# AOS55/exorl

Hardware: AMD Instinct MI355X
Metric: gradient-steps/sec TD3+BC walker_walk batch=1024 (higher is better)
Workload: dtype bf16x3

## Files before the change

exorl_amd/_lib.py:

```python
import ctypes as C
from pathlib import Path

HERE = Path(__file__).resolve().parent
LIB_PATH = HERE / 'libexorl_hip.so'

c_void_p, c_int32, c_int64, c_float, c_size_t, c_uint64, c_uint32 = (
    C.c_void_p, C.c_int32, C.c_int64, C.c_float, C.c_size_t, C.c_uint64, C.c_uint32)
P = C.POINTER

SAMPLER_MT19937, SAMPLER_PHILOX, SAMPLER_GIVEN = 0, 1, 2
WEIGHT_EPISODES, WEIGHT_TRANSITIONS = 0, 1
AGENT_TD3_BC, AGENT_TD3, AGENT_BC, AGENT_DDPG, AGENT_CRR, AGENT_CQL, AGENT_APS = 0, 1, 2, 3, 4, 5, 6
M_CRITIC_CQL, M_CRITIC_CQL_LOGSUM, M_ACTOR_ALPHA, M_ACTOR_ALPHA_LOSS, M_ACTOR_ENT = 10, 11, 12, 13, 14
CRR_WEIGHT = {'identity': 0, 'indicator': 1, 'exp': 2}
PREC_F32, PREC_BF16, PREC_BF16X3, PREC_BF16X6 = 0, 1, 2, 3
NET_ACTOR, NET_CRITIC, NET_CRITIC_TARGET = 0, 1, 2
T_PARAM, T_GRAD, T_ADAM_M, T_ADAM_V = 0, 1, 2, 3
M_BATCH_REWARD, M_CRITIC_TARGET_Q, M_CRITIC_Q1, M_CRITIC_Q2, M_CRITIC_LOSS, M_ACTOR_LOSS, M_ACTOR_LOGPROB = range(7)
N_METRICS = 16
INTR_RND, INTR_ICM, INTR_ICM_APT, INTR_DISAGREEMENT, INTR_DIAYN, INTR_PROTO, INTR_APS, INTR_SMM = 0, 1, 2, 3, 4, 5, 6, 7
IM_LOSS, IM_INTR_REWARD, IM_EXTR_REWARD, IM_RMS_MEAN, IM_RMS_STD, IM_ACC, IM_ENT_REWARD, IM_SF_REWARD = range(8)
N_INTR_METRICS = 8
INTR_XCHG_GRAD, INTR_XCHG_REP, INTR_XCHG_MOMENTS, INTR_XCHG_BN = 0, 1, 2, 3
XCHG_F32, XCHG_F64 = 0, 1
# ... 67 lines not shown
    'exorl_pixel_agent_state': (C.c_int, [c_void_p, c_void_p, c_void_p]),
    'exorl_pixel_agent_set_state': (C.c_int, [c_void_p, c_void_p, c_void_p]),
    'exorl_pixel_agent_encoder_opt2': (C.c_int, [c_void_p, c_void_p, c_void_p, c_void_p]),
    'exorl_pixel_agent_update_phase': (C.c_int, [c_void_p, c_int32, c_float, c_void_p, c_void_p, c_void_p, c_void_p, c_void_p]),
    'exorl_pixel_agent_grad_buffer': (C.c_int, [c_void_p, c_int32, P(c_void_p), P(c_int64)]),
    'exorl_pixel_agent_set_comm': (C.c_int, [c_void_p, c_void_p]),
    'exorl_pixel_agent_encoder_step_phase': (C.c_int, [c_void_p, c_int32, c_void_p, c_int32, c_int32, c_void_p]),
    'exorl_pixel_agent_rnd_features_phase': (C.c_int, [c_void_p, c_int32, c_void_p, c_float, c_void_p, c_void_p, c_void_p]),
    'exorl_pixel_agent_bn_partials': (C.c_int, [c_void_p, P(c_void_p), P(c_int64)]),
    'exorl_pixel_agent_metrics': (C.c_int, [c_void_p, c_void_p, c_void_p]),
    'exorl_pixel_agent_act': (C.c_int, [c_void_p, c_void_p, c_void_p, c_float, c_int32, c_void_p, c_void_p, c_void_p]),
    'exorl_aug_shift': (C.c_int, [c_void_p, c_int32, c_int32, c_int32, c_int32, c_void_p, c_uint64, c_uint64, c_void_p, c_void_p]),
    'exorl_encoder_param_floats': (c_int64, [c_int32, c_int32]),
    'exorl_encoder_out_dim': (c_int64, [c_int32]),
    'exorl_encoder_workspace_floats': (c_int64, [c_int32, c_int32, c_int32]),
    'exorl_encoder_forward': (C.c_int, [c_void_p, c_int32, c_int32, c_void_p, c_int32, c_void_p, P(c_void_p), c_void_p]),
    'exorl_encoder_backward': (C.c_int, [c_void_p, c_int32, c_int32, c_void_p, c_int32, c_void_p, c_void_p, c_void_p, c_void_p]),
    'exorl_encoder_forward_prec': (C.c_int, [c_void_p, c_int32, c_int32, c_void_p, c_int32, c_void_p, P(c_void_p), c_int32, c_void_p]),
    'exorl_encoder_backward_prec': (C.c_int, [c_void_p, c_int32, c_int32, c_void_p, c_int32, c_void_p, c_void_p, c_void_p, c_int32, c_void_p]),
    'exorl_intr_workspace_bytes': (c_size_t, [P(IntrCfg)]),
    'exorl_intr_create': (C.c_int, [P(IntrCfg), c_void_p, c_size_t, P(c_void_p)]),
    'exorl_intr_destroy': (C.c_int, [c_void_p]),
    'exorl_intr_num_tensors': (C.c_int, [c_void_p, P(c_int32)]),
    'exorl_intr_tensor': (C.c_int, [c_void_p, c_int32, c_int32, P(c_void_p), P(c_int64), P(c_int64)]),
    'exorl_intr_flat': (C.c_int, [c_void_p, c_int32, P(c_void_p), P(c_int64)]),
    'exorl_intr_state': (C.c_int, [c_void_p, P(c_void_p), P(c_void_p), P(c_int64)]),
    'exorl_intr_queue': (C.c_int, [c_void_p, P(c_void_p), P(c_int64), P(c_int64), P(c_int64), c_int32]),
    'exorl_intr_update': (C.c_int, [c_void_p, P(IntrBatch), c_int32, c_void_p]),
    'exorl_intr_update_phase': (C.c_int, [c_void_p, P(IntrBatch), c_int32, c_int32, P(c_int32), c_void_p]),
    'exorl_intr_exchange': (C.c_int, [c_void_p, c_int32, P(c_void_p), P(c_int64), P(c_int32), P(c_int32)]),
    'exorl_intr_metrics': (C.c_int, [c_void_p, c_void_p, c_void_p]),
    'exorl_intr_opt_steps': (C.c_int, [c_void_p, P(c_int64), c_int32]),
    'exorl_intr_counter': (C.c_int, [c_void_p, c_void_p, c_int32]),
    'exorl_last_error': (C.c_char_p, []),
    'exorl_abi_version': (C.c_int, []),
    'exorl_device_info': (C.c_int, [C.c_char_p, C.c_int, P(C.c_int), P(c_int64)]),
    'exorl_replay_create': (C.c_int, [P(ReplayCfg), P(c_void_p)]),
    'exorl_replay_destroy': (C.c_int, [c_void_p]),
    'exorl_replay_append_episode': (C.c_int, [c_void_p, c_void_p, c_void_p, c_void_p, c_void_p, c_void_p, c_int32, P(c_int32)]),
    'exorl_replay_evict': (C.c_int, [c_void_p, c_int32]),
    'exorl_replay_set_order': (C.c_int, [c_void_p, c_void_p, c_int32]),
    'exorl_replay_set_weights': (C.c_int, [c_void_p, c_int32, c_void_p, c_int32]),
    'exorl_replay_num_rows': (C.c_int, [c_void_p, P(c_int64), P(c_int64)]),
    'exorl_replay_seed_mt': (C.c_int, [c_void_p, c_void_p, c_int32, c_void_p, c_int32]),
    'exorl_replay_seed_mt_ints': (C.c_int, [c_void_p, c_uint64, c_uint32]),
    'exorl_replay_get_mt': (C.c_int, [c_void_p, c_void_p, P(c_int32), c_void_p, P(c_int32)]),
    'exorl_replay_seed_philox': (C.c_int, [c_void_p, c_uint64]),
    'exorl_replay_sample': (C.c_int, [c_void_p, c_int32, c_int32, c_float, c_int32, c_void_p, P(BatchOut), c_void_p, c_void_p]),
    'exorl_replay_last_pairs': (C.c_int, [c_void_p, c_int32, c_void_p, c_void_p]),
    'exorl_comm_unique_id': (C.c_int, [c_void_p]),
    'exorl_comm_init': (C.c_int, [c_int32, c_int32, c_void_p, P(c_void_p)]),
    'exorl_comm_destroy': (C.c_int, [c_void_p]),
    'exorl_comm_allreduce': (C.c_int, [c_void_p, c_void_p, c_int64, c_void_p]),
    'exorl_agent_set_comm': (C.c_int, [c_void_p, c_void_p]),
    'exorl_agent_workspace_bytes': (c_size_t, [P(AgentCfg)]),
    'exorl_agent_create': (C.c_int, [P(AgentCfg), c_void_p, c_size_t, P(c_void_p)]),
    'exorl_agent_destroy': (C.c_int, [c_void_p]),
    'exorl_agent_num_tensors': (C.c_int, [c_void_p, c_int32, P(c_int32)]),
    'exorl_agent_tensor': (C.c_int, [c_void_p, c_int32, c_int32, c_int32, P(c_void_p), P(c_int64), P(c_int64)]),
    'exorl_agent_flat': (C.c_int, [c_void_p, c_int32, c_int32, P(c_void_p), P(c_int64)]),
    'exorl_agent_params_changed': (C.c_int, [c_void_p, c_int32, c_void_p]),
    'exorl_agent_batch_slots': (C.c_int, [c_void_p, P(BatchOut)]),
    'exorl_agent_set_batch': (C.c_int, [c_void_p, c_void_p, c_void_p, c_void_p, c_void_p, c_void_p, c_void_p]),
    'exorl_agent_update': (C.c_int, [c_void_p, c_float, c_void_p, c_void_p, c_void_p]),
    'exorl_agent_update_phase': (C.c_int, [c_void_p, c_int32, c_float, c_void_p, c_void_p, c_void_p]),
    'exorl_agent_stats_buffer': (C.c_int, [c_void_p, P(c_void_p), P(c_int64)]),
    'exorl_agent_cql_alpha': (C.c_int, [c_void_p, c_void_p, c_int32]),
    'exorl_agent_act': (C.c_int, [c_void_p, c_void_p, c_int32, c_float, c_int32, c_void_p, c_void_p, c_void_p]),
    'exorl_agent_act_host': (C.c_int, [c_void_p, c_void_p, c_int32, c_float, c_int32, c_void_p, c_void_p, c_void_p]),
    'exorl_agent_metrics': (C.c_int, [c_void_p, c_void_p, c_void_p]),
    'exorl_agent_set_metrics': (C.c_int, [c_void_p, c_int32]),
    'exorl_agent_metric_window_bytes': (c_size_t, [P(AgentCfg)]),
    'exorl_agent_set_metric_window': (C.c_int, [c_void_p, c_void_p, c_size_t]),
    'exorl_agent_metric_window_read': (C.c_int, [c_void_p, c_void_p, c_void_p, c_int32, c_void_p]),
    'exorl_agent_set_parallel_branches': (C.c_int, [c_void_p, c_int32]),
    'exorl_agent_opt_steps': (C.c_int, [c_void_p, P(c_int64), P(c_int64)]),
    'exorl_agent_set_opt_steps': (C.c_int, [c_void_p, c_int64, c_int64]),
    'exorl_agent_enable_graph': (C.c_int, [c_void_p, c_void_p, c_int32, c_float, c_float, c_void_p]),
    'exorl_agent_enable_graph_intr': (C.c_int, [c_void_p, c_void_p, P(IntrBatch), c_int32, c_void_p, c_int32, c_float, c_float, c_void_p]),
    'exorl_agent_step_graph': (C.c_int, [c_void_p, c_float, c_void_p]),
    'exorl_agent_noise_counter': (C.c_int, [c_void_p, P(c_uint64), c_void_p]),
    'exorl_debug_philox_normal': (C.c_int, [c_uint64, c_uint64, c_int64, c_void_p, c_void_p]),
    'exorl_debug_agent_poison_scratch': (C.c_int, [c_void_p, c_void_p]),
    'exorl_debug_agent_weight_images': (C.c_int, [c_void_p, c_int32, P(WeightImages)]),
    'exorl_agent_disable_graph': (C.c_int, [c_void_p]),
    'exorl_gemm': (C.c_int, [c_int32, c_int32, c_int32, c_int32, c_int32, c_int32, c_void_p, c_int64, c_void_p, c_int64,
                             c_void_p, c_int64, c_void_p, c_int32, c_int32, c_void_p]),
    'exorl_gemm_bf16': (C.c_int, [c_int32, c_int32, c_int32, c_int32, c_int32, c_void_p, c_int64, c_void_p, c_int64, c_void_p, c_int64,
                                  c_void_p, c_int32, c_int32, c_void_p]),
    'exorl_gemm_planes': (C.c_int, [c_int32, c_void_p, c_int32, c_int32, c_int32, c_int32, c_void_p, c_void_p, c_int64, c_void_p, c_void_p, c_int64,
                                    c_void_p, c_int64, c_int32, c_void_p]),
    'exorl_gemm_planes3': (C.c_int, [c_int32, c_void_p, c_int32, c_int32, c_int32, c_int32, c_void_p, c_void_p, c_void_p, c_int64, c_void_p, c_void_p, c_void_p,
                                     c_int64, c_void_p, c_int64, c_int32, c_void_p]),
    'exorl_gemm_tune': (C.c_int, [c_int32]),
    'exorl_debug_precision_override': (C.c_int, [c_int32]),
    'exorl_profile_gemm': (C.c_int, [c_int32]),
    'exorl_profile_gemm_read': (C.c_int, [c_void_p, c_void_p, c_int32, P(c_int32)]),
    'exorl_profile_event_overhead': (C.c_int, [c_void_p, c_void_p]),
    'exorl_adam_step': (C.c_int, [c_void_p, c_void_p, c_void_p, c_void_p, c_int64, c_float, c_float, c_float, c_float,
                                  c_int64, c_void_p, c_float, c_void_p]),
    'exorl_soft_update': (C.c_int, [c_void_p, c_void_p, c_int64, c_float, c_void_p]),
    'exorl_ln_tanh_fwd': (C.c_int, [c_void_p, c_void_p, c_void_p, c_void_p, c_void_p, c_void_p, c_int32, c_int32, c_void_p]),
    'exorl_knn_topk': (C.c_int, [c_void_p, c_int32, c_void_p, c_int32, c_int32, c_int32, c_void_p, c_void_p]),
}


class ExorlError(RuntimeError):
    pass


_lib = None


def load():
    global _lib
    if _lib is not None:
        return _lib
    if not LIB_PATH.exists():
        raise ExorlError(f'{LIB_PATH} is missing: build it with `python exorl_amd/build.py` '
                         '(hipcc --offload-arch=gfx950). There is no CPU fallback.')
    lib = C.CDLL(str(LIB_PATH))
    for name, (res, args) in PROTOTYPES.items():
        fn = getattr(lib, name)
        fn.restype = res
        fn.argtypes = args
    _lib = lib
    return lib


def check(rc):
    if rc != 0:
        raise ExorlError(load().exorl_last_error().decode())


def ptr(t):
    if t is None:
        return None
    if hasattr(t, 'data_ptr'):
        return t.data_ptr()
    return t.ctypes.data


def current_stream():
    import torch
    return torch.cuda.current_stream().cuda_stream
```

exorl_amd/csrc/agent.hip:

```cpp
#include <cmath>
#include <vector>

#include "kernels.h"

namespace exorl {

struct NetDesc {
    int in_dim = 0, out_dim = 0, H = 0, n_trunks = 0, n_heads = 0;
    int64_t W0 = 0, b0 = 0, g = 0, beta = 0, trunk_stride = 0;
    int64_t W1 = 0, b1 = 0, W2 = 0, b2 = 0, head_stride = 0;
    int64_t total = 0;
    std::vector<TensorDesc> tensors;
};

static int64_t pad4(int64_t n) { return round_up(n, 4); }

static NetDesc make_net(int in_dim, int out_dim, int H, int n_trunks, int n_heads) {
    NetDesc d;
    d.in_dim = in_dim; d.out_dim = out_dim; d.H = H; d.n_trunks = n_trunks; d.n_heads = n_heads;
    int64_t off = 0;
    auto add = [&](int64_t rows, int64_t cols) { const int64_t o = off; d.tensors.push_back({o, rows, cols}); off += pad4(rows * cols); return o; };
    auto add_trunk = [&](bool first) {
        const int64_t w = add(H, in_dim), b = add(H, 1), gg = add(H, 1), be = add(H, 1);
        if (first) { d.W0 = w; d.b0 = b; d.g = gg; d.beta = be; }
// ... 29 lines not shown
    hipStream_t aux = nullptr;
    hipEvent_t ev_fork = nullptr, ev_join = nullptr;
    bool on = false;
    int fork(hipStream_t s) const {
        if (!on) return 0;
        EXORL_CHECK_HIP(hipEventRecord(ev_fork, s));
        EXORL_CHECK_HIP(hipStreamWaitEvent(aux, ev_fork, 0));
        return 0;
    }
    int join(hipStream_t s) const {
        if (!on) return 0;
        EXORL_CHECK_HIP(hipEventRecord(ev_join, aux));
        EXORL_CHECK_HIP(hipStreamWaitEvent(s, ev_join, 0));
        return 0;
    }
    hipStream_t side(hipStream_t s) const { return on ? aux : s; }
};

struct FwdBufs {
    float *h1, *xhat, *rstd, *h2, *out;
    Planes h1q, xhatq;
    FwdBufs rows_from(int64_t row0, int64_t H, int64_t out_cols) const {
        return FwdBufs{h1 + row0 * H, xhat + row0 * H, rstd + row0, h2 + row0 * H, out + row0 * out_cols, h1q.at(row0 * H), xhatq.at(row0 * H)};
    }
};
struct BwdBufs { float *dz2, *dh1; Planes dz2q; };
struct NetShadow { float* w0t; Planes w1q, w0q; };

enum class Route {
    F32,
    Planes,
    Planes3,
};
static Route route_of(int prec, const Planes& act, const Planes& w1, int rows) {
    if (prec == EXORL_PREC_BF16 || (prec == EXORL_PREC_BF16X3 && w1.lo)) return Route::Planes;
    if (prec == EXORL_PREC_BF16X6 && act && w1 && rows % 128 == 0) return Route::Planes3;
    return Route::F32;
}
struct Operand {
    const float* f; Planes q;
    Operand() : f(nullptr) {}
    Operand(const float* f32, int64_t foff, const Planes& planes, int64_t qoff) : f(f32 ? f32 + foff : nullptr), q(planes.at(qoff)) {}
};
struct Product { Operand A, B; float* C; const float* bias; int M, N, K; };
static Gemm16Problem g16(const Planes& A, const Planes& B, float* C, const float* bias, int M, int N, int K, int64_t ld) {
    Gemm16Problem p{A.hi, B.hi, C, bias, M, N, K, ld, ld, ld};
    if (A.mid && B.mid) { p.A_mid = A.mid; p.B_mid = B.mid; }
    if (A.lo && B.lo) { p.A_lo = A.lo; p.B_lo = B.lo; }
    return p;
}
static Gemm16Problem g16(const Product& p, int64_t ld) { return g16(p.A.q, p.B.q, p.C, p.bias, p.M, p.N, p.K, ld); }
static int products(Route rt, int prec, int a_layout, int b_layout, const Product* p, int count, int64_t ld, bool relu, bool accumulate, hipStream_t s) {
    if (rt == Route::F32) {
        GemmProblem g[4];
        for (int i = 0; i < count; ++i) g[i] = GemmProblem{p[i].A.f, p[i].B.f, p[i].C, p[i].bias, p[i].M, p[i].N, p[i].K, ld, ld, ld};
        return gemm_grouped(prec, a_layout, b_layout, g, count, relu, accumulate, s);
    }
    Gemm16Problem q[4];
    for (int i = 0; i < count; ++i) q[i] = g16(p[i], ld);
    return gemm16_grouped(a_layout, b_layout, q, count, relu, accumulate, s);
}
static int refresh_w1_planes(const NetDesc& d, const float* P, const NetShadow& sh, hipStream_t s) {
    if (!sh.w1q.mid) return 0;
    return to_planes3(P + d.W1, d.H, d.H, d.H, sh.w1q.hi, sh.w1q.mid, sh.w1q.lo, d.H, d.H, d.n_heads, d.head_stride, (int64_t)d.H * d.H, s);
}
struct Partials { float *Ph, *Pt, *Pw; };

static ShadowSpec shadow_spec(const NetDesc& d, const NetShadow& sh, const NetShadow* target) {
    ShadowSpec s{};
    s.n_trunks = d.n_trunks; s.n_heads = d.n_heads; s.in_dim = d.in_dim; s.H = d.H;
    for (int t = 0; t < d.n_trunks; ++t) s.w0_off[t] = d.W0 + t * d.trunk_stride;
    for (int i = 0; i < d.n_heads; ++i) s.w1_off[i] = d.W1 + i * d.head_stride;
    const NetShadow none{};
    const NetShadow& t = target ? *target : none;
    const bool own = !sh.w1q.mid;
    s.w0t = sh.w0t; s.t_w0t = t.w0t;
    if (own) { s.w1b = sh.w1q.hi; s.w1l = sh.w1q.lo; s.t_w1b = t.w1q.hi; s.t_w1l = t.w1q.lo; }
    s.w0b = sh.w0q.hi; s.w0l = sh.w0q.lo; s.t_w0b = t.w0q.hi; s.t_w0l = t.w0q.lo;
    return s;
}

static int net_forward(const NetDesc& d, const float* P, const NetShadow& sh, const float* x, int64_t ldx, int rows,
                       const FwdBufs& f, bool save, bool tanh_out, int prec, hipStream_t s, const SampleSpec* sample = nullptr,
                       bool no_head = false) {
    const int H = d.H;
    const int64_t act = (int64_t)rows * H;
    const Route rt = route_of(prec, f.h1q, sh.w1q, rows);
    const bool bf = rt == Route::Planes;
    if (bf && sh.w0q && trunk_fwd16_supported(H))
        EXORL_TRY(trunk_fwd16(x, ldx, sh.w0q, P + d.b0, P + d.g, P + d.beta, save ? f.rstd : nullptr, f.h1q, save ? f.xhatq : Planes{}, rows,
                              d.in_dim, H, d.n_trunks, act, d.trunk_stride, s));
    else
        EXORL_TRY(trunk_fwd(x, ldx, sh.w0t, P + d.b0, P + d.g, P + d.beta, bf ? nullptr : f.h1, (save && !bf) ? f.xhat : nullptr,
                            save ? f.rstd : nullptr, bf ? f.h1q.hi : nullptr, (bf && save) ? f.xhatq.hi : nullptr, rows, d.in_dim, H,
                            d.n_trunks, act, d.trunk_stride, (int64_t)d.in_dim * H, s));
    if (rt == Route::Planes3) EXORL_TRY(to_planes3(f.h1, H, d.n_trunks * rows, H, f.h1q.hi, f.h1q.mid, f.h1q.lo, d.n_trunks * rows, H, 1, 0, 0, s));
    Product p[2];
    for (int i = 0; i < d.n_heads; ++i) {
        const int64_t t = (d.n_trunks == d.n_heads ? i : 0) * act;
        p[i] = Product{Operand(f.h1, t, f.h1q, t), Operand(P + d.W1, i * d.head_stride, sh.w1q, (int64_t)i * H * H), f.h2 + i * act,
                       P + d.b1 + i * d.head_stride, rows, H, H};
    }
    EXORL_TRY(products(rt, prec, 0, 0, p, d.n_heads, H, true, false, s));
    if (no_head) return 0;
    if (H % 4 == 0)
        EXORL_TRY(head_fwd4(f.h2, P + d.W2, P + d.b2, f.out, rows, H, d.out_dim, tanh_out ? 1 : 0, d.n_heads, act, d.head_stride,
                            (int64_t)rows * d.out_dim, s, sample));
    else
        EXORL_TRY(head_fwd(f.h2, P + d.W2, P + d.b2, f.out, rows, H, d.out_dim, tanh_out ? 1 : 0, d.n_heads, act, d.head_stride,
                           (int64_t)rows * d.out_dim, s));
    return 0;
}

static bool forward2_supported(const NetDesc& d, int prec, const NetShadow& sa, const FwdBufs& fa, const NetShadow& sb, const FwdBufs& fb, int rows) {
    const bool planes = route_of(prec, fa.h1q, sa.w1q, rows) == Route::Planes && route_of(prec, fb.h1q, sb.w1q, rows) == Route::Planes;
    return planes && sa.w0q && sb.w0q && trunk_fwd16_supported(d.H) && d.out_dim == 1 && d.n_heads == 2 && d.H % 4 == 0;
}
static int net_forward2(const NetDesc& d, const float* Pa, const NetShadow& sa, const float* xa, const FwdBufs& fa, bool save_a,
                        const float* Pb, const NetShadow& sb, const float* xb, const FwdBufs& fb, bool save_b, int64_t ldx, int rows,
                        hipStream_t s, bool no_head = false, bool fold_a = false, int* slots_a = nullptr) {
    const int H = d.H;
    const int64_t act = (int64_t)rows * H, wst = (int64_t)H * round_up(d.in_dim, 32);
    const float* P[2] = {Pa, Pb};
    const NetShadow* sh[2] = {&sa, &sb};
    const float* x[2] = {xa, xb};
    const FwdBufs* f[2] = {&fa, &fb};
    const bool save[2] = {save_a, save_b};
    TrunkBatch tb{};
    int nt = 0;
    for (int k = 0; k < 2; ++k)
        for (int t = 0; t < d.n_trunks; ++t) {
            const Planes w = sh[k]->w0q.at(t * wst), h = f[k]->h1q.at(t * act), xh = save[k] ? f[k]->xhatq.at(t * act) : Planes{};
            tb.it[nt++] = TrunkItem{x[k], w.hi, P[k] + d.b0 + t * d.trunk_stride, P[k] + d.g + t * d.trunk_stride, P[k] + d.beta + t * d.trunk_stride,
                                    save[k] ? f[k]->rstd + (int64_t)t * rows : nullptr, h.hi, xh.hi, w.lo, h.lo, xh.lo};
        }
    EXORL_TRY(trunk_fwd16_batch(tb, nt, ldx, rows, d.in_dim, H, s));
    Gemm16Problem q[4];
    HeadBatch hb{};
    int nq = 0;
    for (int k = 0; k < 2; ++k)
        for (int i = 0; i < d.n_heads; ++i) {
            q[nq] = g16(f[k]->h1q.at((d.n_trunks == d.n_heads ? i : 0) * act), sh[k]->w1q.at((int64_t)i * H * H), f[k]->h2 + i * act,
                        P[k] + d.b1 + i * d.head_stride, rows, H, H, H);
            hb.it[nq] = HeadItem{f[k]->h2 + i * act, P[k] + d.W2 + i * d.head_stride, P[k] + d.b2 + i * d.head_stride, f[k]->out + (int64_t)i * rows};
            ++nq;
        }
    if (slots_a) *slots_a = 0;
    if (no_head && fold_a && slots_a) {
        const int slots = gemm16_head_slots(q, nq);
        if (slots > 0 && (int64_t)slots <= H) {
            for (int i = 0; i < d.n_heads; ++i) {
                q[i].head_w = P[0] + d.W2 + i * d.head_stride;
                q[i].head_part = f[0]->h2 + i * act;
            }
            *slots_a = slots;
        }
    }
    EXORL_TRY(gemm16_grouped(0, 0, q, nq, true, false, s));
    if (no_head) return 0;
    return head_fwd1_batch(hb, nq, rows, H, s);
}

static int net_backward(const NetDesc& d, const float* P, const NetShadow& sh, float* G, const Partials& pt, const float* x,
                        int64_t ldx, int rows, const FwdBufs& f, const DoutSpec& dout, const BwdBufs& b, float* dx, int dx_col0,
                        int dx_cols, int prec, hipStream_t s, const Fork& fk, FinalizeArgs* defer = nullptr, bool have_dz2 = false) {
    const int H = d.H;
    const int64_t act = (int64_t)rows * H;
    const bool paired = d.n_trunks == d.n_heads;
    Route rt = route_of(prec, f.h1q, sh.w1q, rows);
    if (rt == Route::Planes3 && !b.dz2q) rt = Route::F32;
    const bool bf = rt == Route::Planes;
    const Planes none{};
    const Planes &dz2q = bf ? b.dz2q : none, &h1q = bf ? f.h1q : none, &xhatq = bf ? f.xhatq : none;
    if (have_dz2) {
    } else if (d.out_dim > 16) {
        EXORL_REQUIRE(d.n_heads == 1, "net_backward: wide heads are single-net only");
        EXORL_TRY(head_bwd_wide(dout, P + d.W2, f.h2, bf ? nullptr : b.dz2, dz2q, G ? pt.Ph : nullptr, rows, H, d.out_dim, act, d.head_stride,
                                G ? 1 : 0, s));
    } else {
        EXORL_TRY(head_bwd(dout, P + d.W2, f.h2, bf ? nullptr : b.dz2, dz2q, G ? pt.Ph : nullptr, rows, H, d.out_dim, d.n_heads, act,
                           d.head_stride, G ? 1 : 0, s, dout.mode == EXORL_DOUT_ACTOR_MU && dout.bc_part));
    }
    if (rt == Route::Planes3) EXORL_TRY(to_planes3(b.dz2, H, d.n_heads * rows, H, b.dz2q.hi, b.dz2q.mid, b.dz2q.lo, d.n_heads * rows, H, 1, 0, 0, s));
    auto trunk_of = [&](int i) { return (paired ? i : 0) * act; };
    auto wgrad = [&](int i, int r0, int kr) {
        const int64_t o = (int64_t)r0 * H;
        return Product{Operand(b.dz2, i * act + o, b.dz2q, i * act + o), Operand(f.h1, trunk_of(i) + o, f.h1q, trunk_of(i) + o),
                       G + d.W1 + i * d.head_stride, nullptr, H, H, kr};
    };
    auto dgrad = [&](int i) {
        return Product{Operand(b.dz2, i * act, b.dz2q, i * act), Operand(P + d.W1, i * d.head_stride, sh.w1q, (int64_t)i * H * H),
                       b.dh1 + trunk_of(i), nullptr, rows, H, H};
    };
    Product p[2];
    int dgrads_done = 0;
    if (bf && G && !fk.on) {
        Gemm16Problem q[4];
        int at[4], nq = 0;
        for (int i = 0; i < d.n_heads; ++i) { at[nq] = 1; q[nq++] = g16(wgrad(i, 0, rows), H); }
        dgrads_done = paired ? d.n_heads : 1;
        for (int i = 0; i < dgrads_done; ++i) { at[nq] = 0; q[nq++] = g16(dgrad(i), H); }
        EXORL_TRY(gemm16_grouped_mixed(at, q, nq, s));
    } else if (G) {
        EXORL_TRY(fk.fork(s));
        const int slab = (!bf && rows >= 8192) ? 1024 : rows;
        for (int r0 = 0; r0 < rows; r0 += slab) {
            for (int i = 0; i < d.n_heads; ++i) p[i] = wgrad(i, r0, rows - r0 < slab ? rows - r0 : slab);
            EXORL_TRY(products(rt, prec, 1, 1, p, d.n_heads, H, false, r0 > 0, fk.side(s)));
        }
    }
    for (int i = 0; i < d.n_heads; ++i) p[i] = dgrad(i);
    if (!paired) {
        for (int i = dgrads_done; i < d.n_heads; ++i) EXORL_TRY(products(rt, prec, 0, 1, p + i, 1, H, false, i > 0, s));
    } else if (dgrads_done == 0) {
        EXORL_TRY(products(rt, prec, 0, 1, p, d.n_heads, H, false, false, s));
    }
    const bool dx_fused = dx && !G;
    EXORL_TRY(ln_bwd(b.dh1, f.h1, f.xhat, h1q, xhatq, f.rstd, P + d.g, pt.Pt, rows, H, d.n_trunks, act, d.trunk_stride, G ? 1 : 0, s,
                     dx_fused ? sh.w0t + (int64_t)dx_col0 * H : nullptr, (int64_t)d.in_dim * H, dx_fused ? dx : nullptr, dx_cols,
                     (bf && trunk_fwd16_supported(H)) ? P + d.beta : nullptr));
    if (dx && !dx_fused)
        EXORL_TRY(head_fwd4(b.dh1, sh.w0t + (int64_t)dx_col0 * H, nullptr, dx, rows, H, dx_cols, 0, d.n_trunks, act,
                            (int64_t)d.in_dim * H, (int64_t)rows * dx_cols, s));
    if (G) {
        EXORL_TRY(outer_reduce(x, ldx, d.in_dim, b.dh1, pt.Pw, rows, H, d.n_trunks, act, s));
        EXORL_TRY(fk.join(s));
        FinalizeArgs fa{};
        fa.Ph = pt.Ph; fa.head_chunks = have_dz2 ? qhead_chunks(rows) : head_chunks(rows); fa.n_heads = d.n_heads; fa.head_stride = d.head_stride;
        fa.gW2 = d.W2; fa.gb1 = d.b1; fa.gb2 = d.b2;
        fa.Pt = pt.Pt; fa.trunk_chunks = trunk_chunks(rows); fa.n_trunks = d.n_trunks; fa.trunk_stride = d.trunk_stride;
        fa.Pw = pt.Pw; fa.w_chunks = outer_chunks(rows);
        fa.gW0 = d.W0; fa.gb0 = d.b0; fa.gg = d.g; fa.gbeta = d.beta;
        fa.H = H; fa.nout = d.out_dim; fa.in_dim = d.in_dim; fa.G = G;
        if (defer) *defer = fa;
        else EXORL_TRY(finalize_grads(fa, s));
    }
    return 0;
}

struct Carver : SimpleCarver {
    bool scratch = false;
    std::vector<std::pair<int64_t, int64_t>>* fill = nullptr;
    using SimpleCarver::SimpleCarver;
    float* take(int64_t n) {
        if (fill) {
            const int64_t padded = round_up(n, 64), o = scratch ? off : off + n, len = scratch ? padded : padded - n;
            if (len > 0) {
                if (!fill->empty() && fill->back().first + fill->back().second == o) fill->back().second += len;
                else fill->push_back({o, len});
            }
        }
        return SimpleCarver::take(n);
    }
};

constexpr int ACT_ROWS = 64;

}

using namespace exorl;

struct exorl_agent {
    exorl_agent_cfg cfg;
    NetDesc actor, critic;
    bool has_critic = false;
    bool owns_ws = false;
    float* ws = nullptr;
    size_t ws_bytes = 0;
    float* flat[3][4] = {{nullptr}};
    float *obs = nullptr, *action = nullptr, *reward = nullptr, *discount = nullptr, *next_obs = nullptr;
    float *xa = nullptr, *xc_cur = nullptr, *xc_next = nullptr, *xc_pi = nullptr;
    FwdBufs fa{}, ft{}, fc{};
    BwdBufs bc{}, ba{};
    float *dq = nullptr, *da = nullptr, *dpre = nullptr, *abs_part = nullptr;
    float *sfq = nullptr, *sftq = nullptr;
    float *x_all = nullptr, *dq_all = nullptr;
    CqlScalars* cql = nullptr;
    float *xc_rep = nullptr, *crr_w = nullptr;
    FwdBufs fr{};
    NetShadow sh_actor{}, sh_critic{}, sh_target{};
    ShadowSpec spec_actor{}, spec_critic{};
    Partials pa{}, pc{};
    float *stats = nullptr, *metrics = nullptr;
    float *act_x = nullptr, *act_noise = nullptr;
    float* act_part = nullptr; unsigned int* act_ticket = nullptr;
    FwdBufs fact{};
    StepState* state = nullptr;
    const float *noise_c = nullptr, *noise_a = nullptr;
    int64_t actor_t = 0, critic_t = 0;
    uint64_t act_noise_counter = 0;
    float inv_bg = 0.f;
    float dev_stddev = -1.f;
    hipGraphExec_t graph_exec = nullptr;
    hipGraph_t graph = nullptr;
    hipStream_t capture_stream = nullptr;
    exorl_replay* graph_replay = nullptr;
    uint64_t graph_weights_epoch = 0;
    uint64_t graph_replay_ctr = 0;
    exorl_intr* graph_intr = nullptr;
    bool capturing = false;
    Fork fk{};
    bool parallel_branches = false;
    bool fuse_opt = false;
    bool whole_step = false;
    exorl_comm* comm = nullptr;
    hipStream_t comm_stream = nullptr;
    hipEvent_t ev_stats_ready = nullptr, ev_stats_done = nullptr;
    FinalizeArgs pend_c{}, pend_a{};
    bool staged_by_sampler = false;
    bool want_metrics = true;
    int tq_slots = 0;
    double* win_sums = nullptr; long long* win_steps = nullptr;
    float *win_crit = nullptr, *win_bc = nullptr;
};

namespace exorl {

static bool planes_ok(const exorl_agent_cfg& cfg) {
    return cfg.precision == EXORL_PREC_BF16X3 && cfg.hidden_dim % 64 == 0 && cfg.batch % 64 == 0 && trunk_fwd16_supported(cfg.hidden_dim);
}

static bool planes3_ok(const exorl_agent_cfg& cfg) {
    return cfg.precision == EXORL_PREC_BF16X6 && cfg.hidden_dim % 128 == 0 && cfg.batch % 128 == 0;
}

static void carve(exorl_agent* a, Carver& c) {
    const auto& cfg = a->cfg;
    const int64_t B = cfg.batch, O = cfg.obs_dim, A = cfg.act_dim, H = cfg.hidden_dim, W = O + A;
    const int64_t AO = a->actor.out_dim;
    const int64_t RC = cfg.kind == EXORL_AGENT_CQL ? (3 * cfg.n_samples + 1) * B : B;
    for (int w = 0; w < 4; ++w) a->flat[EXORL_NET_ACTOR][w] = c.take(a->actor.total);
    if (a->has_critic) {
        for (int w = 0; w < 4; ++w) a->flat[EXORL_NET_CRITIC][w] = c.take(a->critic.total);
        a->flat[EXORL_NET_CRITIC_TARGET][EXORL_T_PARAM] = c.take(a->critic.total);
    }
    a->obs = c.take(B * O); a->action = c.take(B * A); a->reward = c.take(B); a->discount = c.take(B); a->next_obs = c.take(B * O);
    const int np = cfg.precision == EXORL_PREC_BF16 ? 1 : planes_ok(cfg) ? 2 : planes3_ok(cfg) ? 3 : 0;
    const int nb = np == 3 ? 0 : np;
    auto take_u16 = [&](int64_t n) { return reinterpret_cast<unsigned short*>(c.take((n + 1) / 2)); };
    auto take_hi_lo = [&](Planes& x, int64_t nx, Planes* y, int64_t ny, int planes) {
        if (planes >= 1) { x.hi = take_u16(nx); if (y) y->hi = take_u16(ny); }
        if (planes >= 2) { x.lo = take_u16(nx); if (y) y->lo = take_u16(ny); }
    };
    auto three_planes = [&](Planes& x, int64_t n) { if (np == 3) { x.hi = take_u16(n); x.mid = take_u16(n); x.lo = take_u16(n); } };
    auto take_fwd = [&](int64_t trunk_rows, int64_t head_rows, int64_t out_cols, bool saved, bool f32_h1, int planes) {
        FwdBufs f{};
        if (f32_h1) f.h1 = c.take(trunk_rows * H);
        if (saved) { f.xhat = c.take(trunk_rows * H); f.rstd = c.take(trunk_rows); }
        f.h2 = c.take(head_rows * H); f.out = c.take(head_rows * out_cols);
        take_hi_lo(f.h1q, trunk_rows * H, saved ? &f.xhatq : nullptr, trunk_rows * H, planes);
        return f;
    };
    auto take_bwd = [&](int64_t head_rows, int64_t trunk_rows) {
        BwdBufs b{c.take(head_rows * H), c.take(trunk_rows * H), {}};
        take_hi_lo(b.dz2q, head_rows * H, nullptr, 0, nb);
        return b;
    };
    auto take_shadow = [&](int64_t n_trunks, int64_t n_heads, int64_t in_dim) {
        NetShadow sh{c.take(n_trunks * in_dim * H), {}, {}};
        take_hi_lo(sh.w1q, n_heads * H * H, &sh.w0q, n_trunks * H * round_up(in_dim, 32), nb);
        return sh;
    };
    c.scratch = true;
    a->xa = c.take(2 * B * O);
    a->fa = take_fwd(2 * B, 2 * B, AO, true, true, nb);
    a->ba = take_bwd(B, B);
    three_planes(a->fa.h1q, 2 * B * H);
    three_planes(a->ba.dz2q, B * H);
    c.scratch = false;
    a->sh_actor = take_shadow(1, 1, O);
    three_planes(a->sh_actor.w1q, H * H);
    c.scratch = true;
    a->pa = Partials{c.take((int64_t)head_chunks(B) * ((AO + 1) * H + 32)), c.take((int64_t)trunk_chunks(B) * 3 * H),
                     c.take((int64_t)outer_chunks(B) * O * H)};
    a->dpre = c.take(B * AO);
    c.scratch = false;
    a->stats = c.take(4 + EXORL_N_METRICS);
    a->metrics = a->stats ? a->stats + 4 : nullptr;
    a->state = reinterpret_cast<StepState*>(c.take((sizeof(StepState) + 3) / 4));
    a->act_x = c.take(ACT_ROWS * O);
    a->act_noise = c.take(ACT_ROWS * A);
    a->act_part = c.take((int64_t)cdiv(H, 4) * ACT_FAST_ROWS * 16);
    a->act_ticket = reinterpret_cast<unsigned int*>(c.take(4));
    a->fact = take_fwd(ACT_ROWS, ACT_ROWS, AO, false, true, nb ? 1 : 0);
    if (a->has_critic) {
        const int64_t nt = a->critic.n_trunks;
        c.scratch = true;
        a->xc_cur = c.take(B * W); a->xc_next = c.take(B * W); a->xc_pi = c.take(B * W);
        const int64_t od = a->critic.out_dim;
        a->ft = take_fwd(nt * B, 2 * B, od, false, true, nb);
        a->fc = take_fwd(nt * RC, 2 * RC, od, true, true, nb);
        a->bc = take_bwd(2 * RC, nt * RC);
        three_planes(a->ft.h1q, nt * B * H);
        three_planes(a->fc.h1q, nt * RC * H);
// ... 32 lines not shown
    EXORL_REQUIRE(cfg, "agent: null cfg");
    EXORL_REQUIRE(cfg->kind >= EXORL_AGENT_TD3_BC && cfg->kind <= EXORL_AGENT_APS, "agent: unknown kind %d", cfg->kind);
    EXORL_REQUIRE(cfg->kind != EXORL_AGENT_APS || (cfg->sf_dim >= 1 && cfg->sf_dim <= 16 && cfg->sf_dim < cfg->obs_dim),
                  "agent: APS needs 1 <= sf_dim <= 16 and obs_dim = observation + sf_dim (got sf_dim=%d obs_dim=%d)", cfg->sf_dim, cfg->obs_dim);
    EXORL_REQUIRE(cfg->kind != EXORL_AGENT_CQL || (cfg->n_samples >= 1 && cfg->n_samples <= 16 && cfg->act_dim <= 16),
                  "agent: CQL needs 1 <= n_samples <= 16 and action_dim <= 16 (got %d, %d)", cfg->n_samples, cfg->act_dim);
    EXORL_REQUIRE(!cfg->use_critic_lagrange || cfg->kind == EXORL_AGENT_CQL, "agent: use_critic_lagrange is a CQL option");
    EXORL_REQUIRE(cfg->kind != EXORL_AGENT_CRR || (cfg->num_value_samples >= 1 && cfg->num_value_samples <= 64 &&
                  cfg->weight_func >= EXORL_CRR_IDENTITY && cfg->weight_func <= EXORL_CRR_EXP),
                  "agent: CRR needs 1 <= num_value_samples <= 64 and a valid weight_func (got %d, %d)", cfg->num_value_samples, cfg->weight_func);
    EXORL_REQUIRE(cfg->obs_dim > 0 && cfg->act_dim > 0 && cfg->act_dim <= 16 && cfg->hidden_dim >= 4 && cfg->hidden_dim <= 1024 && cfg->hidden_dim % 4 == 0 &&
                  cfg->obs_dim + cfg->act_dim <= 256 &&
                  cfg->batch > 0, "agent: unsupported dims O=%d A=%d (<=16) H=%d (multiple of 4, <=1024) B=%d; O+A <= 256", cfg->obs_dim, cfg->act_dim,
                  cfg->hidden_dim, cfg->batch);
    EXORL_REQUIRE(cfg->precision == EXORL_PREC_F32 || cfg->precision == EXORL_PREC_BF16 || cfg->precision == EXORL_PREC_BF16X3 ||
                  cfg->precision == EXORL_PREC_BF16X6, "agent: unknown precision %d", cfg->precision);
    EXORL_REQUIRE(cfg->world_size >= 1, "agent: world_size must be >= 1");
    EXORL_REQUIRE(cfg->precision != EXORL_PREC_BF16 || (cfg->hidden_dim % 8 == 0 && cfg->batch % 8 == 0),
                  "agent: bf16 precision needs hidden_dim and batch to be multiples of 8 (got H=%d B=%d)", cfg->hidden_dim, cfg->batch);
    a->cfg = *cfg;
    a->has_critic = cfg->kind != EXORL_AGENT_BC;
    a->actor = make_net(cfg->obs_dim, cfg->kind == EXORL_AGENT_CQL ? 2 * cfg->act_dim : cfg->act_dim, cfg->hidden_dim, 1, 1);
    if (a->has_critic)
        a->critic = make_net(cfg->obs_dim + cfg->act_dim, cfg->kind == EXORL_AGENT_APS ? cfg->sf_dim : 1, cfg->hidden_dim,
                             (cfg->kind == EXORL_AGENT_DDPG || cfg->kind == EXORL_AGENT_APS) ? 1 : 2, 2);
    a->inv_bg = 1.0f / ((float)cfg->batch * (float)cfg->world_size);
    return 0;
}

static NoiseSpec noise_spec(exorl_agent* a, const float* buf, int which) {
    return NoiseSpec{buf, a->cfg.seed, (uint64_t)which, buf ? nullptr : &a->state->noise_counter};
}
static NoiseSpec act_noise_spec(exorl_agent* a, const float* buf) {
    NoiseSpec n{buf, a->cfg.seed, 0, nullptr};
    if (!buf) n.counter = (1ull << 63) | a->act_noise_counter++;
    return n;
}

static int push_opt_steps(exorl_agent* a) {
    long long t[2] = {a->actor_t, a->critic_t};
    EXORL_CHECK_HIP(hipMemcpy(&a->state->t_actor, t, sizeof(t), hipMemcpyHostToDevice));
    auto prod = [](double b, long long t) { double r = 1.0; for (long long i = 0; i < t; ++i) r *= b; return r; };
    const double p[4] = {prod(0.9, a->actor_t), 0.0, prod(0.9, a->critic_t), prod(0.999, a->critic_t)};
    const double p2 = prod(0.999, a->actor_t);
    EXORL_CHECK_HIP(hipMemcpy(&a->state->b1t, p, sizeof(p), hipMemcpyHostToDevice));
    EXORL_CHECK_HIP(hipMemcpy(&a->state->b2t, &p2, sizeof(p2), hipMemcpyHostToDevice));
    return 0;
}

static FusedAdamArgs fused_adam_args(exorl_agent* a, int net, const NetDesc& d, const AdamConst* c, float* target, uint64_t* bump) {
    float** f = a->flat[net];
    return FusedAdamArgs{f[EXORL_T_PARAM], f[EXORL_T_GRAD], f[EXORL_T_ADAM_M], f[EXORL_T_ADAM_V], target, c, d.n_heads,
                         {d.W1, d.W1 + d.head_stride}, reinterpret_cast<unsigned long long*>(bump)};
}
static int opt_step(exorl_agent* a, int net, const NetDesc& d, const FinalizeArgs& pend, const AdamConst* c, float* target, const ShadowSpec& spec,
                    uint64_t* bump, hipStream_t s) {
    float** f = a->flat[net];
    if (a->fuse_opt) EXORL_TRY(finalize_adam(pend, fused_adam_args(a, net, d, c, target, bump), spec, s));
    else EXORL_TRY(adam_step_dev(f[EXORL_T_PARAM], f[EXORL_T_GRAD], f[EXORL_T_ADAM_M], f[EXORL_T_ADAM_V], d.total, c, target, &spec, s, bump));
    EXORL_TRY(refresh_w1_planes(d, f[EXORL_T_PARAM], net == EXORL_NET_ACTOR ? a->sh_actor : a->sh_critic, s));
    if (target) EXORL_TRY(refresh_w1_planes(d, target, a->sh_target, s));
    return 0;
}
static int opt_step_critic(exorl_agent* a, hipStream_t s) {
    return opt_step(a, EXORL_NET_CRITIC, a->critic, a->pend_c, &a->state->critic, a->flat[EXORL_NET_CRITIC_TARGET][EXORL_T_PARAM], a->spec_critic,
                    nullptr, s);
}

static bool qfuse(const exorl_agent* a) {
    return a->whole_step && !a->fk.on && (!a->want_metrics || a->win_sums) && a->has_critic && a->critic.n_heads == 2 && a->critic.out_dim == 1 && a->cfg.hidden_dim % 4 == 0 &&
           (a->cfg.kind == EXORL_AGENT_TD3_BC || a->cfg.kind == EXORL_AGENT_TD3 || a->cfg.kind == EXORL_AGENT_DDPG);
}
static bool step_metrics(const exorl_agent* a) { return a->win_sums ? !qfuse(a) : a->want_metrics; }
constexpr size_t WIN_HEAD_BYTES = 256;
static_assert(EXORL_N_METRICS * sizeof(double) + sizeof(long long) <= WIN_HEAD_BYTES, "the window's sums and step count fit its head");
static size_t window_bytes(const exorl_agent_cfg& cfg) {
    return WIN_HEAD_BYTES + sizeof(float) * (size_t)round_up(6 * (int64_t)qhead_chunks(cfg.batch) + head_chunks(cfg.batch), 64);
}
static int run_metrics_window(exorl_agent* a, hipStream_t s) {
    const int B = a->cfg.batch;
    MetricsWindowArgs w{};
    w.fused = qfuse(a) ? 1 : 0;
    w.crit_part = a->win_crit; w.abs_part = a->abs_part; w.bc_part = a->win_bc;
    w.q_chunks = qhead_chunks(B); w.bc_chunks = a->cfg.kind == EXORL_AGENT_TD3_BC ? head_chunks(B) : 0;
    w.kind = a->cfg.kind; w.act_dim = a->cfg.act_dim; w.ent_from_std = a->cfg.kind != EXORL_AGENT_CQL;
    w.inv_bg = a->inv_bg; w.alpha = a->cfg.alpha; w.stddev = &a->state->stddev;
    w.metrics = a->metrics; w.sums = a->win_sums; w.steps = a->win_steps;
    return metrics_window(w, s);
}
static int run_qhead(exorl_agent* a, int mode, hipStream_t s) {
    const NetDesc& d = a->critic;
    const int B = a->cfg.batch, H = d.H;
    const int64_t act = (int64_t)B * H;
    const float* Pc = a->flat[EXORL_NET_CRITIC][EXORL_T_PARAM];
    const float* Pt = a->flat[EXORL_NET_CRITIC_TARGET][EXORL_T_PARAM];
    const bool bf = route_of(a->cfg.precision, a->fc.h1q, a->sh_critic.w1q, B) == Route::Planes;
    QHeadArgs q{};
    for (int i = 0; i < 2; ++i) {
        q.a[i] = a->fc.h2 + i * act; q.W[i] = Pc + d.W2 + i * d.head_stride; q.b[i] = Pc + d.b2 + i * d.head_stride;
        q.a[2 + i] = a->ft.h2 + i * act; q.W[2 + i] = Pt + d.W2 + i * d.head_stride; q.b[2 + i] = Pt + d.b2 + i * d.head_stride;
    }
    q.q = a->fc.out; q.tq = a->ft.out; q.reward = a->reward; q.discount = a->discount;
    q.tpart[0] = q.tpart[1] = nullptr; q.tslots = 0;
    if (mode == 0 && a->tq_slots > 0) {
        q.tpart[0] = a->ft.h2; q.tpart[1] = a->ft.h2 + act; q.tslots = a->tq_slots;
    }
    q.dz = bf ? nullptr : a->bc.dz2; q.dzb = bf ? a->bc.dz2q.hi : nullptr; q.dzl = bf ? a->bc.dz2q.lo : nullptr; q.act = act;
    q.P = mode == 0 ? a->pc.Ph : nullptr;
    const bool met = mode == 0 && a->win_sums;
    q.abs_part = met ? a->win_crit : a->abs_part;
    q.rows = B; q.H = H; q.mode = mode; q.inv_bg = a->inv_bg;
    return qhead(q, s, met);
}

static int phase0(exorl_agent* a, float stddev, const float* noise_c, hipStream_t s) {
    const auto& cfg = a->cfg;
    const int B = cfg.batch, O = cfg.obs_dim, A = cfg.act_dim, W = O + A, prec = cfg.precision;
    if (!a->staged_by_sampler)
        EXORL_TRY(prepare_inputs(a->obs, a->action, a->next_obs, a->xa, a->xc_cur, a->xc_next, a->xc_pi, B, O, A, a->has_critic, a->state,
                                 a->capturing ? 1 : 0, s));
    a->actor_t += 1;
    if (a->has_critic) a->critic_t += 1;
    if (!a->has_critic) return 0;
    const float* Pa = a->flat[EXORL_NET_ACTOR][EXORL_T_PARAM];
    const float* Pc = a->flat[EXORL_NET_CRITIC][EXORL_T_PARAM];
    const float* Pt = a->flat[EXORL_NET_CRITIC_TARGET][EXORL_T_PARAM];
    a->noise_c = noise_c;
    const bool fused_sample = cfg.hidden_dim % 4 == 0 && A > 1;
    SampleSpec sp{&a->state->stddev, noise_c, cfg.kind == EXORL_AGENT_CRR ? nullptr : a->noise_a, cfg.seed, &a->state->noise_counter, stddev, cfg.stddev_clip,
                  a->xc_next + O, a->xc_pi + O, W, B};
    EXORL_TRY(net_forward(a->actor, Pa, a->sh_actor, a->xa, O, 2 * B, a->fa, true, true, prec, s, fused_sample ? &sp : nullptr));
    if (!fused_sample)
        EXORL_TRY(sample_actions2(a->fa.out, noise_c, cfg.kind == EXORL_AGENT_CRR ? nullptr : a->noise_a, cfg.seed,
                                  &a->state->noise_counter, stddev, cfg.stddev_clip, a->xc_next + O, a->xc_pi + O, W, B, A, s, &a->state->stddev));
    const bool qf = qfuse(a);
    a->tq_slots = 0;
    if (!a->fk.on && forward2_supported(a->critic, prec, a->sh_target, a->ft, a->sh_critic, a->fc, B)) {
        EXORL_TRY(net_forward2(a->critic, Pt, a->sh_target, a->xc_next, a->ft, false, Pc, a->sh_critic, a->xc_cur, a->fc, true, W, B, s, qf, qf,
                               &a->tq_slots));
    } else {
        EXORL_TRY(a->fk.fork(s));
        EXORL_TRY(net_forward(a->critic, Pt, a->sh_target, a->xc_next, W, B, a->ft, false, false, prec, a->fk.side(s), nullptr, qf));
        EXORL_TRY(net_forward(a->critic, Pc, a->sh_critic, a->xc_cur, W, B, a->fc, true, false, prec, s, nullptr, qf));
        EXORL_TRY(a->fk.join(s));
    }
    if (qf) EXORL_TRY(run_qhead(a, 0, s));
    const bool aps = cfg.kind == EXORL_AGENT_APS;
    const float* task = aps ? a->obs + (O - cfg.sf_dim) : nullptr;
    const float *qv = a->fc.out, *tqv = a->ft.out;
    if (aps) {
        EXORL_TRY(sf_q(a->ft.out, task, O, a->sftq, B, cfg.sf_dim, 2, s));
        EXORL_TRY(sf_q(a->fc.out, task, O, a->sfq, B, cfg.sf_dim, 2, s));
        qv = a->sfq; tqv = a->sftq;
    }
    if (step_metrics(a))
        EXORL_TRY(critic_loss(qv, tqv, a->reward, a->discount, a->dq, a->metrics, B, a->inv_bg, s));
    DoutSpec td{};
    td.mode = EXORL_DOUT_TD; td.q = qv; td.tq = tqv; td.reward = a->reward; td.discount = a->discount; td.inv_bg = a->inv_bg;
    td.task = task; td.task_ld = O;
    EXORL_TRY(net_backward(a->critic, Pc, a->sh_critic, a->flat[EXORL_NET_CRITIC][EXORL_T_GRAD], a->pc, a->xc_cur, W, B, a->fc, td,
                           a->bc, nullptr, 0, 0, prec, s, a->fk, a->fuse_opt ? &a->pend_c : nullptr, qf));
    return 0;
}

static int phase1(exorl_agent* a, float stddev, const float* noise_a, hipStream_t s) {
    if (!a->has_critic) return 0;
    const auto& cfg = a->cfg;
    const int B = cfg.batch, O = cfg.obs_dim, A = cfg.act_dim, W = O + A, prec = cfg.precision;
    EXORL_TRY(opt_step_critic(a, s));
    if (cfg.kind == EXORL_AGENT_CRR) {
        const int n = cfg.num_value_samples;
        const float* Pc = a->flat[EXORL_NET_CRITIC][EXORL_T_PARAM];
        EXORL_TRY(repeat_sample(a->obs, a->fa.out + (int64_t)B * A, noise_a, cfg.seed, noise_a ? nullptr : &a->state->noise_counter, 1,
                                stddev, cfg.stddev_clip, a->xc_rep, B, O, A, n, s, &a->state->stddev));
        EXORL_TRY(net_forward(a->critic, Pc, a->sh_critic, a->xc_rep, W, B * n, a->fr, false, false, prec, s));
        EXORL_TRY(net_forward(a->critic, Pc, a->sh_critic, a->xc_cur, W, B, a->fc, false, false, prec, s));
        EXORL_TRY(crr_weights(a->fr.out, a->fc.out, a->crr_w, B, n, cfg.weight_func, s));
        return 0;
    }
    if ((cfg.kind == EXORL_AGENT_DDPG || cfg.kind == EXORL_AGENT_APS) && (a->want_metrics || a->win_sums))
        EXORL_TRY(sample_action(a->fa.out + (int64_t)B * A, noise_spec(a, noise_a, 1), stddev, cfg.stddev_clip, 1, a->xc_pi + O, W, B, A,
                                a->metrics + EXORL_M_ACTOR_LOGPROB, s, &a->state->stddev, cfg.world_size));
    const bool qf = qfuse(a);
    EXORL_TRY(net_forward(a->critic, a->flat[EXORL_NET_CRITIC][EXORL_T_PARAM], a->sh_critic, a->xc_pi, W, B, a->fc, true, false, prec, s,
                          nullptr, qf));
    if (cfg.kind == EXORL_AGENT_APS) {
        EXORL_TRY(sf_q(a->fc.out, a->obs + (O - cfg.sf_dim), O, a->sfq, B, cfg.sf_dim, 2, s));
        EXORL_TRY(actor_stats(a->sfq, a->stats, B, s));
    } else if (!qf) {
        EXORL_TRY(actor_stats(a->fc.out, a->stats, B, s));
    }
    return 0;
}

static int phase2(exorl_agent* a, float stddev, hipStream_t s) {
    const auto& cfg = a->cfg;
    const int B = cfg.batch, O = cfg.obs_dim, A = cfg.act_dim, W = O + A, H = cfg.hidden_dim, prec = cfg.precision;
    const float* Pa = a->flat[EXORL_NET_ACTOR][EXORL_T_PARAM];
    if (a->has_critic && cfg.kind != EXORL_AGENT_CRR) {
        DoutSpec dq{};
        dq.mode = EXORL_DOUT_ACTOR_Q; dq.q = a->fc.out; dq.stats = a->stats; dq.inv_bg = a->inv_bg; dq.alpha = cfg.alpha;
        if (cfg.kind == EXORL_AGENT_APS) { dq.q = a->sfq; dq.task = a->obs + (O - cfg.sf_dim); dq.task_ld = O; }
        dq.use_lambda = cfg.kind == EXORL_AGENT_TD3_BC;
        const bool qf = qfuse(a);
        if (qf) EXORL_TRY(run_qhead(a, 1, s));
        if (qf && a->comm && dq.use_lambda) {
            EXORL_TRY(reduce_pairs(a->abs_part, qhead_chunks(B), a->stats, s));
            EXORL_CHECK_HIP(hipEventRecord(a->ev_stats_ready, s));
            EXORL_CHECK_HIP(hipStreamWaitEvent(a->comm_stream, a->ev_stats_ready, 0));
            EXORL_TRY(comm_allreduce_sum(a->comm, a->stats, 4, a->comm_stream));
            EXORL_CHECK_HIP(hipEventRecord(a->ev_stats_done, a->comm_stream));
        }
        EXORL_TRY(net_backward(a->critic, a->flat[EXORL_NET_CRITIC][EXORL_T_PARAM], a->sh_critic, nullptr, a->pc, a->xc_pi, W, B, a->fc,
                               dq, a->bc, a->da, O, A, prec, s, a->fk, nullptr, qf));
    }
    const FwdBufs f = a->fa.rows_from(B, H, A);
    if (!a->has_critic)
        EXORL_TRY(net_forward(a->actor, Pa, a->sh_actor, a->xa + (int64_t)B * O, O, B, f, true, true, prec, s));
    if (step_metrics(a))
        EXORL_TRY(actor_dmu(a->da, A, a->has_critic ? a->critic.n_trunks : 0, (int64_t)B * A, f.out, a->action,
                            a->has_critic ? nullptr : a->reward, a->crr_w, a->dpre, a->stats, a->metrics, B, A, a->inv_bg, cfg.alpha,
                            cfg.kind, stddev, s, &a->state->stddev));
    DoutSpec dm{};
    dm.mode = EXORL_DOUT_ACTOR_MU; dm.da = a->da; dm.da_nets = a->has_critic ? a->critic.n_trunks : 0; dm.mu = f.out; dm.a_data = a->action;
    dm.kind = cfg.kind; dm.inv_bg = a->inv_bg; dm.stddev = stddev; dm.stddev_ptr = &a->state->stddev; dm.w = a->crr_w;
    if (qfuse(a)) {
        dm.lam_parts = a->abs_part; dm.lam_chunks = qhead_chunks(B); dm.use_lambda = cfg.kind == EXORL_AGENT_TD3_BC; dm.alpha = cfg.alpha;
        if (a->comm && dm.use_lambda) {
            EXORL_CHECK_HIP(hipStreamWaitEvent(s, a->ev_stats_done, 0));
            dm.lam_parts = a->stats; dm.lam_chunks = 1;
        }
        if (a->win_sums && cfg.kind == EXORL_AGENT_TD3_BC) dm.bc_part = a->win_bc;
    }
    EXORL_TRY(net_backward(a->actor, Pa, a->sh_actor, a->flat[EXORL_NET_ACTOR][EXORL_T_GRAD], a->pa, a->xa + (int64_t)B * O, O, B, f,
                           dm, a->ba, nullptr, 0, 0, prec, s, a->fk, a->fuse_opt ? &a->pend_a : nullptr));
    return 0;
}

static int phase3(exorl_agent* a, hipStream_t s) {
    return opt_step(a, EXORL_NET_ACTOR, a->actor, a->pend_a, &a->state->actor, nullptr, a->spec_actor,
                    a->staged_by_sampler ? &a->state->replay_counter : nullptr, s);
}

static CqlNoise cql_noise(exorl_agent* a) {
    const int64_t BA = (int64_t)a->cfg.batch * a->cfg.act_dim, n = a->cfg.n_samples;
    const float* nc = a->noise_c;
    CqlNoise z{};
    z.z_next = nc; z.u_rand = nc ? nc + BA : nullptr; z.z_cur = nc ? nc + (1 + n) * BA : nullptr;
    z.z_nxt = nc ? nc + (1 + 2 * n) * BA : nullptr; z.z_actor = a->noise_a;
    z.seed = a->cfg.seed; z.counter_ptr = &a->state->noise_counter;
    return z;
}

static int cql_phase0a(exorl_agent* a, hipStream_t s, bool split) {
    const auto& cfg = a->cfg;
    const int B = cfg.batch, O = cfg.obs_dim, A = cfg.act_dim, W = O + A, n = cfg.n_samples, prec = cfg.precision;
    const int R = (3 * n + 1) * B;
    if (!a->staged_by_sampler)
        EXORL_TRY(prepare_inputs(a->obs, a->action, a->next_obs, a->xa, a->xc_cur, a->xc_next, a->xc_pi, B, O, A, 1, a->state,
                                 a->capturing ? 1 : 0, s));
    a->actor_t += 1;
    a->critic_t += 1;
    const float* Pa = a->flat[EXORL_NET_ACTOR][EXORL_T_PARAM];
    const float* Pc = a->flat[EXORL_NET_CRITIC][EXORL_T_PARAM];
    EXORL_TRY(net_forward(a->actor, Pa, a->sh_actor, a->xa, O, 2 * B, a->fa, true, false, prec, s));
    EXORL_TRY(cql_build_inputs(a->obs, a->action, a->fa.out, cql_noise(a), a->xc_next, a->x_all, B, O, A, n, s));
    EXORL_TRY(net_forward(a->critic, a->flat[EXORL_NET_CRITIC_TARGET][EXORL_T_PARAM], a->sh_target, a->xc_next, W, B, a->ft, false, false,
                          prec, s));
    EXORL_TRY(net_forward(a->critic, Pc, a->sh_critic, a->x_all, W, R, a->fc, true, false, prec, s));
    if (split)
        EXORL_TRY(cql_critic_dq(a->fc.out, a->ft.out, a->reward, a->discount, a->dq_all, a->metrics, B, n, cfg.alpha, a->inv_bg, s,
                                a->cql + 1, &a->state->critic, cfg.target_cql_penalty, 1, a->stats + 2));
    return 0;
}

static int cql_phase0b(exorl_agent* a, hipStream_t s, bool split) {
    const auto& cfg = a->cfg;
    const int B = cfg.batch, O = cfg.obs_dim, A = cfg.act_dim, W = O + A, n = cfg.n_samples, prec = cfg.precision;
    const int R = (3 * n + 1) * B;
    const float* Pc = a->flat[EXORL_NET_CRITIC][EXORL_T_PARAM];
    EXORL_TRY(cql_critic_dq(a->fc.out, a->ft.out, a->reward, a->discount, a->dq_all, a->metrics, B, n, cfg.alpha, a->inv_bg, s,
                            cfg.use_critic_lagrange ? a->cql + 1 : nullptr, &a->state->critic, cfg.target_cql_penalty, split ? 2 : 0, a->stats + 2));
    DoutSpec d{};
    d.mode = EXORL_DOUT_BUFFER; d.buf = a->dq_all;
    EXORL_TRY(net_backward(a->critic, Pc, a->sh_critic, a->flat[EXORL_NET_CRITIC][EXORL_T_GRAD], a->pc, a->x_all, W, R, a->fc, d, a->bc,
                           nullptr, 0, 0, prec, s, a->fk, a->fuse_opt ? &a->pend_c : nullptr));
    return 0;
}

static int cql_phase0(exorl_agent* a, hipStream_t s) {
    EXORL_REQUIRE(!(a->cfg.use_critic_lagrange && a->cfg.world_size > 1), "agent_update_phase: CQL with use_critic_lagrange under data parallelism "
                  "runs phase 0 as phases 4 and 5 with a sum-all-reduce of exorl_agent_stats in between");
    EXORL_TRY(cql_phase0a(a, s, false));
    return cql_phase0b(a, s, false);
}

static int cql_phase1(exorl_agent* a, hipStream_t s) {
    const auto& cfg = a->cfg;
    const int B = cfg.batch, O = cfg.obs_dim, A = cfg.act_dim, W = O + A, prec = cfg.precision;
    EXORL_TRY(opt_step_critic(a, s));
    EXORL_TRY(cql_actor_sample(a->fa.out + (int64_t)B * 2 * A, cql_noise(a), a->xc_pi, W, a->stats, B, O, A, s));
    EXORL_TRY(net_forward(a->critic, a->flat[EXORL_NET_CRITIC][EXORL_T_PARAM], a->sh_critic, a->xc_pi, W, B, a->fc, true, false, prec, s));
    return 0;
}

static int cql_phase2(exorl_agent* a, hipStream_t s) {
    const auto& cfg = a->cfg;
    const int B = cfg.batch, O = cfg.obs_dim, A = cfg.act_dim, W = O + A, H = cfg.hidden_dim, prec = cfg.precision;
    EXORL_TRY(cql_alpha_step(a->cql, a->stats, &a->state->actor, a->metrics, B, A, a->inv_bg, a->fc.out, s));
    DoutSpec dq{};
// ... 319 lines not shown
    EXORL_TRY(release_graph(a));
    if (!a->capture_stream) EXORL_CHECK_HIP(hipStreamCreateWithFlags(&a->capture_stream, hipStreamNonBlocking));
    exorl_batch_out slots;
    EXORL_TRY(exorl_agent_batch_slots(a, &slots));
    const int O_raw = a->cfg.obs_dim - meta_dim;
    if (meta_dim > 0) {
        int r_act = 0, r_meta = 0;
        replay_dims(r, &r_act, &r_meta);
        EXORL_REQUIRE(O_raw > 0 && replay_obs_bytes(r) == O_raw * 4 && r_act == a->cfg.act_dim && r_meta == meta_dim,
                      "agent_enable_graph_intr: the replay's rows (%d obs bytes, %d action, %d meta columns) do not fill [obs | meta] rows of "
                      "%d + %d floats and %d actions", replay_obs_bytes(r), r_act, r_meta, O_raw, meta_dim, a->cfg.act_dim);
        slots.meta = a->obs + O_raw;
        slots.meta_stride = a->cfg.obs_dim;
    }
    if (it) {
        EXORL_REQUIRE(ib && ib->reward_out == a->reward && (!ib->extr_reward || ib->extr_reward == a->reward),
                      "agent_enable_graph_intr: the module writes its reward into the agent's reward slot");
        EXORL_TRY(intr_graph_prepare(it, ib, a->capture_stream));
    }
    EXORL_TRY(replay_prepare(r, a->cfg.batch, nstep, a->capture_stream));
    const uint64_t ctr = replay_philox_counter(r);
    EXORL_CHECK_HIP(hipMemcpyAsync(&a->state->replay_counter, &ctr, sizeof(ctr), hipMemcpyHostToDevice, a->capture_stream));
    EXORL_TRY(set_device_float(&a->state->stddev, stddev, a->capture_stream));
    a->dev_stddev = stddev;
    EXORL_CHECK_HIP(hipStreamSynchronize(a->capture_stream));
    const int64_t t_a = a->actor_t, t_c = a->critic_t;
    if (!a->fk.aux) {
        EXORL_CHECK_HIP(hipStreamCreateWithFlags(&a->fk.aux, hipStreamNonBlocking));
        EXORL_CHECK_HIP(hipEventCreateWithFlags(&a->fk.ev_fork, hipEventDisableTiming));
        EXORL_CHECK_HIP(hipEventCreateWithFlags(&a->fk.ev_join, hipEventDisableTiming));
    }
    EXORL_CHECK_HIP(hipStreamBeginCapture(a->capture_stream, hipStreamCaptureModeThreadLocal));
    a->capturing = true;
    a->fk.on = a->parallel_branches;
    StageOut stage{a->xa, a->xc_cur, a->xc_next, a->xc_pi, a->cfg.obs_dim, a->cfg.act_dim, a->cfg.batch, a->has_critic ? 1 : 0, a->state};
    a->staged_by_sampler = replay_obs_bytes(r) == a->cfg.obs_dim * 4;
    int rc = replay_sample_impl(r, a->cfg.batch, nstep, gamma, EXORL_SAMPLER_PHILOX, nullptr, &slots, nullptr, a->capture_stream,
                                &a->state->replay_counter, a->staged_by_sampler ? &stage : nullptr);
    if (rc == 0 && meta_dim > 0) rc = copy_meta_columns(a->obs, a->next_obs, a->cfg.obs_dim, a->cfg.batch, O_raw, meta_dim, a->capture_stream);
    if (rc == 0 && it) rc = intr_graph_capture(it, ib, a->capture_stream);
    a->fuse_opt = !a->comm && !a->fk.on;
    a->whole_step = true;
    if (rc == 0) rc = whole_step_body(a, stddev, nullptr, nullptr, a->capture_stream);
    a->fuse_opt = false;
    a->whole_step = false;
    a->staged_by_sampler = false;
    a->capturing = false;
    a->fk.on = false;
    hipGraph_t g = nullptr;
    hipError_t e = hipStreamEndCapture(a->capture_stream, &g);
    a->actor_t = t_a; a->critic_t = t_c;
    replay_advance_philox(r, (uint64_t)-1);
    if (rc != 0) { if (g) (void)hipGraphDestroy(g); return rc; }
    if (e != hipSuccess) { set_error("agent_enable_graph: hipStreamEndCapture -> %s", hipGetErrorString(e)); return 1; }
    a->graph = g;
    EXORL_CHECK_HIP(hipGraphInstantiate(&a->graph_exec, g, nullptr, nullptr, 0));
    a->graph_replay = r;
    a->graph_weights_epoch = replay_weights_epoch(r);
    a->graph_replay_ctr = ctr;
    a->graph_intr = it;
    return 0;
}

int exorl_agent_enable_graph(exorl_agent_t* a, exorl_replay_t* r, int32_t nstep, float gamma, float stddev, void* stream) {
    return enable_graph_impl(a, nullptr, nullptr, 0, r, nstep, gamma, stddev, stream);
}

int exorl_agent_enable_graph_intr(exorl_agent_t* a, exorl_intr_t* intr, const exorl_intr_batch* batch, int32_t meta_dim, exorl_replay_t* r,
                                  int32_t nstep, float gamma, float stddev, void* stream) {
    EXORL_REQUIRE(a, "agent_enable_graph_intr: null argument");
    EXORL_REQUIRE(meta_dim >= 0 && meta_dim < a->cfg.obs_dim, "agent_enable_graph_intr: meta_dim=%d out of range", meta_dim);
    EXORL_REQUIRE(!intr || a->cfg.world_size == 1, "agent_enable_graph_intr: the joint graph is the one-process step");
    return enable_graph_impl(a, intr, batch, meta_dim, r, nstep, gamma, stddev, stream);
}

int exorl_agent_noise_counter(exorl_agent_t* a, uint64_t* counter_out, void* stream) {
    EXORL_REQUIRE(a && counter_out, "agent_noise_counter: null argument");
    hipStream_t s = as_stream(stream);
    EXORL_CHECK_HIP(hipMemcpyAsync(counter_out, &a->state->noise_counter, sizeof(uint64_t), hipMemcpyDeviceToHost, s));
    EXORL_CHECK_HIP(hipStreamSynchronize(s));
    return 0;
}

int exorl_debug_agent_poison_scratch(exorl_agent_t* a, void* stream) {
    EXORL_REQUIRE(a, "debug_agent_poison_scratch: null handle");
    hipStream_t s = as_stream(stream);
    exorl_agent layout;
    layout.cfg = a->cfg; layout.actor = a->actor; layout.critic = a->critic; layout.has_critic = a->has_critic;
    std::vector<std::pair<int64_t, int64_t>> runs;
    Carver c(nullptr);
    c.fill = &runs;
    carve(&layout, c);
    EXORL_REQUIRE((size_t)c.off * sizeof(float) == a->ws_bytes, "debug_agent_poison_scratch: layout mismatch");
    for (const auto& r : runs) EXORL_CHECK_HIP(hipMemsetAsync(a->ws + r.first, 0xFF, (size_t)r.second * sizeof(float), s));
    return 0;
}

int exorl_debug_agent_weight_images(exorl_agent_t* a, int32_t net, exorl_weight_images* out) {
    EXORL_REQUIRE(a && out, "debug_agent_weight_images: null argument");
    const NetDesc* d = net_of(a, net);
    EXORL_REQUIRE(d, "debug_agent_weight_images: agent has no net %d", net);
    const NetShadow& sh = net == EXORL_NET_ACTOR ? a->sh_actor : net == EXORL_NET_CRITIC ? a->sh_critic : a->sh_target;
    *out = exorl_weight_images{d->n_trunks, d->n_heads, d->in_dim, d->H, sh.w0t, sh.w0q.hi, sh.w0q.lo, sh.w1q.hi, sh.w1q.mid, sh.w1q.lo};
    return 0;
}

int exorl_agent_cql_alpha(exorl_agent_t* a, float* host, int32_t set) {
    EXORL_REQUIRE(a && host && a->cql, "agent_cql_alpha: not a CQL agent / null argument");
    const int nsc = a->cfg.use_critic_lagrange ? 2 : 1;
    for (int i = 0; i < nsc; ++i) {
        float* h = host + 3 * i;
        if (set) {
            CqlScalars sc{h[0], h[1], h[2], expf(h[0])};
            EXORL_CHECK_HIP(hipMemcpy(a->cql + i, &sc, sizeof(sc), hipMemcpyHostToDevice));
        } else {
            CqlScalars sc;
            EXORL_CHECK_HIP(hipMemcpy(&sc, a->cql + i, sizeof(sc), hipMemcpyDeviceToHost));
            h[0] = sc.log_alpha; h[1] = sc.m; h[2] = sc.v;
        }
    }
    return 0;
}

int exorl_agent_set_parallel_branches(exorl_agent_t* a, int32_t enable) {
    EXORL_REQUIRE(a, "agent_set_parallel_branches: null handle");
    EXORL_REQUIRE(!a->graph_exec, "agent_set_parallel_branches: disable the captured graph first");
    a->parallel_branches = enable != 0;
    return 0;
}

int exorl_agent_set_metrics(exorl_agent_t* a, int32_t enable) {
    EXORL_REQUIRE(a, "agent_set_metrics: null handle");
    EXORL_REQUIRE(!a->graph_exec, "agent_set_metrics: disable the captured graph first");
    a->want_metrics = enable != 0;
    return 0;
}

size_t exorl_agent_metric_window_bytes(const exorl_agent_cfg* cfg) {
    exorl_agent tmp;
    if (describe(&tmp, cfg) != 0) return 0;
    return window_bytes(*cfg);
}

int exorl_agent_set_metric_window(exorl_agent_t* a, void* buf_dev, size_t bytes) {
    EXORL_REQUIRE(a, "agent_set_metric_window: null handle");
    EXORL_REQUIRE(!a->graph_exec, "agent_set_metric_window: disable the captured graph first");
    if (!buf_dev) {
        a->win_sums = nullptr; a->win_steps = nullptr; a->win_crit = a->win_bc = nullptr;
        return 0;
    }
    EXORL_REQUIRE(a->cfg.world_size == 1, "agent_set_metric_window: the metric window belongs to the one-process step; this agent was built for "
                  "world_size=%d (its metrics are partial means that the caller all-reduces)", a->cfg.world_size);
    const size_t need = window_bytes(a->cfg);
    EXORL_REQUIRE(bytes >= need && (uintptr_t)buf_dev % 256 == 0, "agent_set_metric_window: buffer %zu B (need %zu B, 256-byte aligned)", bytes, need);
    EXORL_CHECK_HIP(hipMemset(buf_dev, 0, WIN_HEAD_BYTES));
    a->win_sums = static_cast<double*>(buf_dev);
    a->win_steps = reinterpret_cast<long long*>(a->win_sums + EXORL_N_METRICS);
    a->win_crit = reinterpret_cast<float*>(static_cast<char*>(buf_dev) + WIN_HEAD_BYTES);
    a->win_bc = a->win_crit + 6 * (int64_t)qhead_chunks(a->cfg.batch);
    return 0;
}

int exorl_agent_metric_window_read(exorl_agent_t* a, double* sums_host, int64_t* steps_host, int32_t reset, void* stream) {
    EXORL_REQUIRE(a && sums_host && steps_host, "agent_metric_window_read: null argument");
    EXORL_REQUIRE(a->win_sums, "agent_metric_window_read: no metric window (exorl_agent_set_metric_window)");
    hipStream_t s = as_stream(stream);
// ... 38 lines not shown
```

exorl_amd/csrc/fused.hip:

```cpp
#include "kernels.h"

namespace exorl {

constexpr int MAX_IN = 256;
constexpr float LN_EPS2 = 1e-5f;
typedef __bf16 bf16_t;

__device__ __forceinline__ unsigned short f2bf(float x) {
    bf16_t b = (bf16_t)x;
    return __builtin_bit_cast(unsigned short, b);
}
__device__ __forceinline__ unsigned short f2bf_lo(float x) { return f2bf(x - __uint_as_float((unsigned)f2bf(x) << 16)); }
__device__ __forceinline__ ushort4 f4_to_bf4(const float4& v) { ushort4 q; q.x = f2bf(v.x); q.y = f2bf(v.y); q.z = f2bf(v.z); q.w = f2bf(v.w); return q; }
__device__ __forceinline__ ushort4 f4_to_bf4_lo(const float4& v) { ushort4 q; q.x = f2bf_lo(v.x); q.y = f2bf_lo(v.y); q.z = f2bf_lo(v.z); q.w = f2bf_lo(v.w); return q; }

constexpr int TF_ROWS = 8;
constexpr int TF_LDS_FLOATS = 35 * 1024;

__device__ __forceinline__ float tanh_fast(float x) {
    const float e = __expf(2.0f * x);
    return 1.0f - 2.0f * __frcp_rn(1.0f + e);
}

template <bool FAST>
// ... 410 lines not shown
        return 0;
    }
#define EXORL_TF16(T) do { if (x3) hipLaunchKernelGGL((trunk_fwd16_kernel<T, true>), grid, dim3(512), 0, s, tb, ldx, rows, in_dim, Kp); \
                           else hipLaunchKernelGGL((trunk_fwd16_kernel<T, false>), grid, dim3(512), 0, s, tb, ldx, rows, in_dim, Kp); } while (0)
    switch (H / 128) {
        case 1: EXORL_TF16(1); break;
        case 2: EXORL_TF16(2); break;
        case 3: EXORL_TF16(3); break;
        case 4: EXORL_TF16(4); break;
        case 5: EXORL_TF16(5); break;
        case 6: EXORL_TF16(6); break;
        case 7: EXORL_TF16(7); break;
        default: EXORL_TF16(8); break;
    }
#undef EXORL_TF16
    EXORL_LAUNCH_CHECK();
    return 0;
}

int trunk_fwd16(const float* x, int64_t ldx, const Planes& W0q, const float* b0, const float* gain, const float* beta, float* rstd,
                const Planes& hq, const Planes& xhatq, int rows, int in_dim, int H, int nets, int64_t astride, int64_t pstride, hipStream_t s) {
    EXORL_REQUIRE(W0q && hq && nets >= 1 && nets <= 4, "trunk_fwd16: bad arguments");
    TrunkBatch tb{};
    const int64_t wstride = (int64_t)H * round_up(in_dim, 32);
    for (int n = 0; n < nets; ++n) {
        const Planes w = W0q.at(n * wstride), h = hq.at(n * astride), xh = xhatq.at(n * astride);
        tb.it[n] = TrunkItem{x, w.hi, b0 + n * pstride, gain + n * pstride, beta + n * pstride, rstd ? rstd + (int64_t)n * rows : nullptr,
                             h.hi, xh.hi, w.lo, h.lo, xh.lo};
    }
    return trunk_fwd16_batch(tb, nets, ldx, rows, in_dim, H, s);
}

int trunk_fwd(const float* x, int64_t ldx, const float* W0T, const float* b0, const float* gain, const float* beta,
              float* h, float* xhat, float* rstd, unsigned short* h_bf16, unsigned short* xhat_bf16, int rows, int in_dim,
              int H, int nets, int64_t astride, int64_t pstride, int64_t tstride, hipStream_t s) {
    EXORL_REQUIRE(H >= 4 && H <= 1024 && H % 4 == 0 && in_dim >= 1 && in_dim <= MAX_IN, "trunk_fwd: unsupported H=%d in=%d", H, in_dim);
    int kc = TF_LDS_FLOATS / H;
    if (kc > in_dim) kc = in_dim;
    const size_t lds = ((size_t)kc * H + TF_ROWS * MAX_IN) * sizeof(float);
    const dim3 grid(cdiv(rows, TF_ROWS), nets);
    static bool attr_set = false;
    if (!attr_set) {
        EXORL_CHECK_HIP(hipFuncSetAttribute((const void*)trunk_fwd_kernel<true>, hipFuncAttributeMaxDynamicSharedMemorySize, 160 * 1024));
        EXORL_CHECK_HIP(hipFuncSetAttribute((const void*)trunk_fwd_kernel<false>, hipFuncAttributeMaxDynamicSharedMemorySize, 160 * 1024));
        attr_set = true;
    }
    if (h_bf16) hipLaunchKernelGGL((trunk_fwd_kernel<true>), grid, dim3(512), lds, s, x, ldx, W0T, b0, gain, beta, h, xhat, rstd, h_bf16,
                                   xhat_bf16, rows, in_dim, H, astride, pstride, tstride, kc);
    else        hipLaunchKernelGGL((trunk_fwd_kernel<false>), grid, dim3(512), lds, s, x, ldx, W0T, b0, gain, beta, h, xhat, rstd, h_bf16,
                                   xhat_bf16, rows, in_dim, H, astride, pstride, tstride, kc);
    EXORL_LAUNCH_CHECK();
    return 0;
}

constexpr int TB_ROWS = 8;
static int tb_iters(int rows) { return rows >= 8192 ? 4 : 1; }
static int or_iters(int rows) { return rows >= 8192 ? 4 : 1; }
__device__ __forceinline__ float4 bf4_to_f4(ushort4 q) {
    return make_float4(__uint_as_float((unsigned)q.x << 16), __uint_as_float((unsigned)q.y << 16),
                       __uint_as_float((unsigned)q.z << 16), __uint_as_float((unsigned)q.w << 16));
}

__device__ __forceinline__ float wave_sum8(const float (&v)[8], int lane) {
    float a[4], b[2];
#pragma unroll
    for (int j = 0; j < 4; ++j) {
        const float keep = (lane & 1) ? v[2 * j + 1] : v[2 * j];
        const float send = (lane & 1) ? v[2 * j] : v[2 * j + 1];
        a[j] = keep + __shfl_xor(send, 1, 64);
    }
#pragma unroll
    for (int j = 0; j < 2; ++j) {
        const float keep = (lane & 2) ? a[2 * j + 1] : a[2 * j];
        const float send = (lane & 2) ? a[2 * j] : a[2 * j + 1];
        b[j] = keep + __shfl_xor(send, 2, 64);
    }
    float r = ((lane & 4) ? b[1] : b[0]) + __shfl_xor((lane & 4) ? b[0] : b[1], 4, 64);
    r += __shfl_xor(r, 8, 64);
    r += __shfl_xor(r, 16, 64);
    r += __shfl_xor(r, 32, 64);
    return r;
}

template <bool PARAMS, bool B16, bool LO, bool RECOMP>
__global__ __launch_bounds__(512) void ln_bwd_kernel(float* dh, const float* __restrict__ h, const float* __restrict__ xhat,
                                                     const unsigned short* __restrict__ hb, const unsigned short* __restrict__ xhb,
                                                     const float* __restrict__ rstd, const float* __restrict__ gain,
                                                     float* __restrict__ P, int rows, int H, int64_t astride,
                                                     int64_t pstride, const float* __restrict__ w0t, int64_t tstride,
                                                     float* __restrict__ dx, int dx_cols, const unsigned short* __restrict__ hl,
                                                     const unsigned short* __restrict__ xhl, int iters, const float* __restrict__ beta) {
    __shared__ __attribute__((aligned(16))) float red[PARAMS ? 3 * 8 * 1024 : 4];
    const int net = blockIdx.y;
    const int tid = threadIdx.x, lane = tid & 63, wave = tid >> 6;
    const int H4 = H >> 2;
    float4 g[4], be[4], pg[4], pb[4], pb0[4];
#pragma unroll
    for (int i = 0; i < 4; ++i) {
        const int c4 = lane + 64 * i;
        g[i] = c4 < H4 ? reinterpret_cast<const float4*>(gain + net * pstride)[c4] : make_float4(0.f, 0.f, 0.f, 0.f);
        be[i] = (RECOMP && c4 < H4) ? reinterpret_cast<const float4*>(beta + net * pstride)[c4] : make_float4(0.f, 0.f, 0.f, 0.f);
        pg[i] = pb[i] = pb0[i] = make_float4(0.f, 0.f, 0.f, 0.f);
    }
    for (int it = 0; it < iters; ++it) {
        const int row = blockIdx.x * TB_ROWS * iters + it * 8 + wave;
        if (row >= rows) continue;
        const int64_t o = net * astride + (int64_t)row * H;
        float4 d[4], xh[4];
        float s1 = 0.f, s2 = 0.f;
        float4 dvs[4], hvs[4];
        ushort4 xb[4], xl[4], hbv[4], hlv[4];
#pragma unroll
        for (int i = 0; i < 4; ++i) {
            const int cc = lane + 64 * i < H4 ? lane + 64 * i : 0;
            dvs[i] = reinterpret_cast<const float4*>(dh + o)[cc];
            if constexpr (B16) {
                xb[i] = reinterpret_cast<const ushort4*>(xhb + o)[cc];
                if constexpr (LO) xl[i] = reinterpret_cast<const ushort4*>(xhl + o)[cc];
                if constexpr (!RECOMP) {
                    hbv[i] = reinterpret_cast<const ushort4*>(hb + o)[cc];
                    if constexpr (LO) hlv[i] = reinterpret_cast<const ushort4*>(hl + o)[cc];
                }
            } else {
                hvs[i] = reinterpret_cast<const float4*>(h + o)[cc];
                xh[i] = reinterpret_cast<const float4*>(xhat + o)[cc];
            }
        }
#pragma unroll
        for (int i = 0; i < 4; ++i) {
            const int c4 = lane + 64 * i;
            d[i] = make_float4(0.f, 0.f, 0.f, 0.f);
            if (c4 >= H4) { xh[i] = make_float4(0.f, 0.f, 0.f, 0.f); }
            if (c4 < H4) {
                float4 hv;
                if constexpr (B16) {
                    xh[i] = bf4_to_f4(xb[i]);
                    if constexpr (LO) {
                        const float4 l2 = bf4_to_f4(xl[i]);
                        xh[i].x += l2.x; xh[i].y += l2.y; xh[i].z += l2.z; xh[i].w += l2.w;
                    }
                    if constexpr (RECOMP) {
                        hv.x = tanh_fast(xh[i].x * g[i].x + be[i].x); hv.y = tanh_fast(xh[i].y * g[i].y + be[i].y);
                        hv.z = tanh_fast(xh[i].z * g[i].z + be[i].z); hv.w = tanh_fast(xh[i].w * g[i].w + be[i].w);
                    } else {
                        hv = bf4_to_f4(hbv[i]);
                        if constexpr (LO) {
                            const float4 l1 = bf4_to_f4(hlv[i]);
                            hv.x += l1.x; hv.y += l1.y; hv.z += l1.z; hv.w += l1.w;
                        }
                    }
                } else {
                    hv = hvs[i];
                }
                const float4 dv = dvs[i];
                float4 dy;
                dy.x = dv.x * (1.0f - hv.x * hv.x); dy.y = dv.y * (1.0f - hv.y * hv.y);
                dy.z = dv.z * (1.0f - hv.z * hv.z); dy.w = dv.w * (1.0f - hv.w * hv.w);
                if constexpr (PARAMS) {
                    pg[i].x += dy.x * xh[i].x; pg[i].y += dy.y * xh[i].y; pg[i].z += dy.z * xh[i].z; pg[i].w += dy.w * xh[i].w;
                    pb[i].x += dy.x; pb[i].y += dy.y; pb[i].z += dy.z; pb[i].w += dy.w;
                }
                d[i].x = dy.x * g[i].x; d[i].y = dy.y * g[i].y; d[i].z = dy.z * g[i].z; d[i].w = dy.w * g[i].w;
                s1 += (d[i].x + d[i].y) + (d[i].z + d[i].w);
                s2 += (d[i].x * xh[i].x + d[i].y * xh[i].y) + (d[i].z * xh[i].z + d[i].w * xh[i].w);
            }
        }
        const float m1 = wave_sum(s1) / (float)H, m2 = wave_sum(s2) / (float)H;
        const float rs = rstd[net * (int64_t)rows + row];
        float4 dzv[4];
#pragma unroll
        for (int i = 0; i < 4; ++i) {
            const int c4 = lane + 64 * i;
            dzv[i] = make_float4(0.f, 0.f, 0.f, 0.f);
            if (c4 < H4) {
                float4 v;
                v.x = rs * (d[i].x - m1 - xh[i].x * m2); v.y = rs * (d[i].y - m1 - xh[i].y * m2);
                v.z = rs * (d[i].z - m1 - xh[i].z * m2); v.w = rs * (d[i].w - m1 - xh[i].w * m2);
                if (PARAMS || !dx) reinterpret_cast<float4*>(dh + o)[c4] = v;
                dzv[i] = v;
                if constexpr (PARAMS) { pb0[i].x += v.x; pb0[i].y += v.y; pb0[i].z += v.z; pb0[i].w += v.w; }
            }
        }
        if constexpr (!PARAMS) {
            if (dx) {
                for (int j0 = 0; j0 < dx_cols; j0 += 8) {
                    float part[8];
#pragma unroll
                    for (int j = 0; j < 8; ++j) part[j] = 0.f;
#pragma unroll
                    for (int i = 0; i < 4; ++i) {
                        const int cc = lane + 64 * i < H4 ? lane + 64 * i : 0;
                        float4 wv[8];
#pragma unroll
                        for (int j = 0; j < 8; ++j)
                            wv[j] = reinterpret_cast<const float4*>(w0t + net * tstride + (int64_t)(j0 + j < dx_cols ? j0 + j : 0) * H)[cc];
#pragma unroll
                        for (int j = 0; j < 8; ++j) part[j] += dzv[i].x * wv[j].x + dzv[i].y * wv[j].y + dzv[i].z * wv[j].z + dzv[i].w * wv[j].w;
                    }
                    const float tot = wave_sum8(part, lane);
                    const int j = j0 + (lane & 7);
                    if (lane < 8 && j < dx_cols) dx[((int64_t)net * rows + row) * dx_cols + j] = tot;
                }
            }
        }
    }
    if constexpr (PARAMS) {
        float* Pn = P + ((int64_t)net * gridDim.x + blockIdx.x) * 3 * H;
#pragma unroll
        for (int i = 0; i < 4; ++i) {
            const int c4 = lane + 64 * i;
            if (c4 < H4) {
                reinterpret_cast<float4*>(red + wave * 1024)[c4] = pg[i];
                reinterpret_cast<float4*>(red + (8 + wave) * 1024)[c4] = pb[i];
                reinterpret_cast<float4*>(red + (16 + wave) * 1024)[c4] = pb0[i];
            }
        }
        __syncthreads();
        for (int c = tid; c < H; c += 512) {
#pragma unroll
            for (int q = 0; q < 3; ++q) {
                float sacc = 0.f;
#pragma unroll
                for (int w = 0; w < 8; ++w) sacc += red[(q * 8 + w) * 1024 + c];
                Pn[q * H + c] = sacc;
            }
        }
    }
}

int ln_bwd(float* dh, const float* h, const float* xhat, const Planes& hq, const Planes& xhatq, const float* rstd, const float* gain, float* P,
           int rows, int H, int nets, int64_t astride, int64_t pstride, int want_params, hipStream_t s, const float* w0t, int64_t tstride,
           float* dx, int dx_cols, const float* beta) {
    const unsigned short *h_bf16 = hq.hi, *xhat_bf16 = xhatq.hi, *h_lo = hq.lo, *xhat_lo = xhatq.lo;
    EXORL_REQUIRE(H >= 4 && H <= 1024 && H % 4 == 0, "ln_bwd: unsupported H=%d", H);
    EXORL_REQUIRE(!dx || (!want_params && w0t && dx_cols >= 1), "ln_bwd: the dx epilogue belongs to the dgrad-only pass");
    const dim3 grid(trunk_chunks(rows), nets);
    const bool b16 = h_bf16 && xhat_bf16;
    const int iters = tb_iters(rows);
    EXORL_REQUIRE((h_lo != nullptr) == (xhat_lo != nullptr) && (!h_lo || b16), "ln_bwd: lo planes come in pairs, with the bf16 hi planes");
    const bool lo = h_lo != nullptr, rc = b16 && beta != nullptr;
#define EXORL_LNB(PA, BB, LL, RR) hipLaunchKernelGGL((ln_bwd_kernel<PA, BB, LL, RR>), grid, dim3(512), 0, s, dh, h, xhat, h_bf16, xhat_bf16, rstd, gain, P, rows, H, astride, pstride, w0t, tstride, dx, dx_cols, h_lo, xhat_lo, iters, beta)
#define EXORL_LNB2(PA) do { if (!b16) EXORL_LNB(PA, false, false, false); \
                             else if (lo && rc) EXORL_LNB(PA, true, true, true); else if (lo) EXORL_LNB(PA, true, true, false); \
                             else if (rc) EXORL_LNB(PA, true, false, true); else EXORL_LNB(PA, true, false, false); } while (0)
    if (want_params) EXORL_LNB2(true); else EXORL_LNB2(false);
#undef EXORL_LNB2
#undef EXORL_LNB
    EXORL_LAUNCH_CHECK();
    return 0;
}
int trunk_chunks(int rows) { return cdiv(rows, TB_ROWS * tb_iters(rows)); }

constexpr int OR_ROWS = 32;
__global__ __launch_bounds__(256) void outer_reduce_kernel(const float* __restrict__ u, int64_t ldu, int J,
                                                           const float* __restrict__ v, float* __restrict__ P, int rows,
                                                           int H, int64_t vstride, int iters) {
    __shared__ __attribute__((aligned(16))) float us[OR_ROWS][32];
    const int net = blockIdx.z;
    const int c = blockIdx.x * 256 + threadIdx.x;
    float* Pn = P + ((int64_t)net * gridDim.y + blockIdx.y) * (int64_t)J * H;
    for (int j0 = 0; j0 < J; j0 += 32) {
        float acc[32];
#pragma unroll
        for (int j = 0; j < 32; ++j) acc[j] = 0.f;
        for (int sub = 0; sub < iters; ++sub) {
            const int row0 = (blockIdx.y * iters + sub) * OR_ROWS;
            const int nr = rows - row0 < OR_ROWS ? rows - row0 : OR_ROWS;
            const int rclamp = nr > 0 ? row0 : rows - 1;
            float vall[OR_ROWS];
            const int cc = c < H ? c : 0;
#pragma unroll
            for (int r = 0; r < OR_ROWS; ++r) vall[r] = v[net * vstride + (int64_t)(r < nr ? row0 + r : rclamp) * H + cc];
            float ust[OR_ROWS * 32 / 256];
#pragma unroll
            for (int q = 0; q < OR_ROWS * 32 / 256; ++q) {
                const int i = threadIdx.x + 256 * q, r = i >> 5, j = i & 31;
                ust[q] = u[(int64_t)(r < nr ? row0 + r : rclamp) * ldu + (j0 + j < J ? j0 + j : 0)];
            }
            __syncthreads();
#pragma unroll
            for (int q = 0; q < OR_ROWS * 32 / 256; ++q) {
                const int i = threadIdx.x + 256 * q, r = i >> 5, j = i & 31;
                us[r][j] = (r < nr && j0 + j < J) ? ust[q] : 0.f;
            }
            __syncthreads();
            if (c < H) {
#pragma unroll 1
                for (int rb = 0; rb < OR_ROWS; rb += 8) {
#pragma unroll
                    for (int r = 0; r < 8; ++r) {
                        const float vr = vall[rb + r];
#pragma unroll
                        for (int j4 = 0; j4 < 8; ++j4) {
                            const float4 uu = *reinterpret_cast<const float4*>(&us[rb + r][4 * j4]);
                            acc[4 * j4] += uu.x * vr; acc[4 * j4 + 1] += uu.y * vr; acc[4 * j4 + 2] += uu.z * vr; acc[4 * j4 + 3] += uu.w * vr;
                        }
                        __builtin_amdgcn_sched_barrier(0);
                    }
                }
            }
        }
        if (c < H) {
#pragma unroll
            for (int j = 0; j < 32; ++j)
                if (j0 + j < J) Pn[(int64_t)(j0 + j) * H + c] = acc[j];
        }
    }
}

int outer_reduce(const float* u, int64_t ldu, int J, const float* v, float* P, int rows, int H, int nets, int64_t vstride,
                 hipStream_t s) {
    hipLaunchKernelGGL(outer_reduce_kernel, dim3(cdiv(H, 256), outer_chunks(rows), nets), dim3(256), 0, s, u, ldu, J, v, P, rows,
                       H, vstride, or_iters(rows));
    EXORL_LAUNCH_CHECK();
    return 0;
}
int outer_chunks(int rows) { return cdiv(rows, OR_ROWS * or_iters(rows)); }

__device__ __forceinline__ float philox_normal_f(uint64_t seed, uint64_t counter, uint32_t elem) {
    uint32_t c[4] = {elem, 0u, (uint32_t)counter, (uint32_t)(counter >> 32)};
    Philox::gen(c, seed);
    const float u1 = ((float)c[0] + 1.0f) * 2.3283064365386963e-10f;
    const float u2 = (float)c[1] * 2.3283064365386963e-10f;
    return sqrtf(-2.0f * __logf(u1)) * __cosf(6.283185307179586f * u2);
// ... 99 lines not shown
    return 0;
}

constexpr int HB_ROWS = 8;
__device__ __forceinline__ float dout_value(const DoutSpec& d, int net, int m, int j, int rows, int nout, float lam = 1.0f) {
    if (d.mode == EXORL_DOUT_BUFFER) return d.buf[((int64_t)net * rows + m) * nout + j];
    if (d.mode == EXORL_DOUT_CQL_ACTOR) {
        const int A = nout >> 1, jj = j < A ? j : j - A;
        const float* rr = d.raw + (int64_t)m * nout;
        const float mu = tanhf(rr[jj]);
        const float ls = rr[A + jj];
        const float sd = expf(fminf(fmaxf(ls, -10.0f), 2.0f));
        const int e = m * A + jj;
        const float z = d.z ? d.z[e] : philox_normal_f(d.seed, (d.counter_ptr ? *d.counter_ptr : 0ull) * 8 + d.counter, (uint32_t)e);
        const float y = tanhf(mu + sd * z);
        float dy = 0.f;
        for (int t = 0; t < d.da_nets; ++t) dy += d.da[((int64_t)t * rows + m) * A + jj];
        const float g = dy * (1.0f - y * y);
        const float c = *d.alpha_ptr * d.inv_bg / (float)A;
        if (j < A) return (g + 2.0f * c * y) * (1.0f - mu * mu);
        const float inside = (ls >= -10.0f && ls <= 2.0f) ? 1.0f : 0.0f;
        return (g * z + c * (-1.0f / sd + 2.0f * y * z)) * sd * inside;
    }
    if (d.mode == EXORL_DOUT_TD) {
        const float y = d.reward[m] + d.discount[m] * fminf(d.tq[m], d.tq[rows + m]);
        const float g = 2.0f * (d.q[net * rows + m] - y) * d.inv_bg;
        return d.task ? g * d.task[(int64_t)m * d.task_ld + j] : g;
    }
    if (d.mode == EXORL_DOUT_ACTOR_Q) {
        const float lambda = d.use_lambda ? d.alpha / (d.stats[0] * d.inv_bg) : 1.0f;
        const float q1 = d.q[m], q2 = d.q[rows + m];
        const float w1 = q1 < q2 ? 1.0f : (q1 == q2 ? 0.5f : 0.0f);
        const float g = -lambda * d.inv_bg * (net == 0 ? w1 : 1.0f - w1);
        return d.task ? g * d.task[(int64_t)m * d.task_ld + j] : g;
    }
    const int i = m * nout + j;
    const float mv = d.mu[i];
    float dmu;
    if (d.kind == EXORL_AGENT_BC) {
        const float sd = d.stddev_ptr ? *d.stddev_ptr : d.stddev;
        dmu = -(d.a_data[i] - mv) / (sd * sd) * d.inv_bg;
    } else if (d.kind == EXORL_AGENT_CRR) {
        const float sd = d.stddev_ptr ? *d.stddev_ptr : d.stddev;
        dmu = -d.w[m] * (d.a_data[i] - mv) / (sd * sd) * d.inv_bg;
    } else {
        dmu = 0.f;
        for (int t = 0; t < d.da_nets; ++t) dmu += d.da[((int64_t)t * rows + m) * nout + j];
        dmu *= lam;
        if (d.kind == EXORL_AGENT_TD3_BC) dmu += 2.0f * d.inv_bg / (float)nout * (mv - d.a_data[i]);
    }
    return dmu * (1.0f - mv * mv);
}

template <int NO, bool MET = false>
__global__ __launch_bounds__(256) void head_bwd_kernel(const DoutSpec dspec, const float* __restrict__ W,
                                                       const float* __restrict__ a, float* __restrict__ dz,
                                                       unsigned short* __restrict__ dzb, float* __restrict__ P, int rows,
                                                       int H, int nout, int64_t astride, int64_t pstride, int want_params,
                                                       unsigned short* __restrict__ dzl) {
    __shared__ float ds[HB_ROWS * 16];
    __shared__ float lam_s[5];
    const int net = blockIdx.y;
    const int row0 = blockIdx.x * HB_ROWS;
    const int c4 = threadIdx.x;
    const int H4 = H >> 2;
    const int c4c = c4 < H4 ? c4 : 0;
    const int nr = rows - row0 < HB_ROWS ? rows - row0 : HB_ROWS;
    float4 w[NO], pw[NO], avs[HB_ROWS];
#pragma unroll
    for (int j = 0; j < NO; ++j) {
        w[j] = reinterpret_cast<const float4*>(W + net * pstride + (int64_t)(j < nout ? j : 0) * H)[c4c];
        pw[j] = make_float4(0.f, 0.f, 0.f, 0.f);
    }
#pragma unroll
    for (int r = 0; r < HB_ROWS; ++r)
        avs[r] = reinterpret_cast<const float4*>(a + net * astride + (int64_t)(row0 + (r < nr ? r : 0)) * H)[c4c];
    const bool mu_path = dspec.mode == EXORL_DOUT_ACTOR_MU && dspec.kind != EXORL_AGENT_BC && dspec.kind != EXORL_AGENT_CRR;
    const int dr = (threadIdx.x >> 4) & (HB_ROWS - 1), dj = threadIdx.x & 15;
    const bool dlive = threadIdx.x < HB_ROWS * 16 && row0 + dr < rows && dj < nout;
    float mu_v = 0.f, da_v = 0.f, ad_v = 0.f;
    if (mu_path) {
        const int i = (dlive ? row0 + dr : 0) * nout + (dlive ? dj : 0);
        mu_v = dspec.mu[i];
        for (int t = 0; t < dspec.da_nets; ++t) da_v += dspec.da[(int64_t)t * rows * nout + i];
        if (dspec.kind == EXORL_AGENT_TD3_BC) ad_v = dspec.a_data[i];
    }
    float lam = 1.0f;
    if (dspec.mode == EXORL_DOUT_ACTOR_MU && dspec.lam_parts && dspec.use_lambda) {
        float sabs = 0.f;
        for (int i = threadIdx.x; i < dspec.lam_chunks; i += blockDim.x) sabs += dspec.lam_parts[2 * i];
        sabs = wave_sum(sabs);
        if ((threadIdx.x & 63) == 0) lam_s[threadIdx.x >> 6] = sabs;
        __syncthreads();
        if (threadIdx.x == 0) lam_s[4] = dspec.alpha / (((lam_s[0] + lam_s[1]) + (lam_s[2] + lam_s[3])) * dspec.inv_bg);
        __syncthreads();
        lam = lam_s[4];
    }
    if (threadIdx.x < HB_ROWS * 16) {
        float dv = 0.f;
        if (mu_path) {
            float dmu = da_v * lam;
            if (dspec.kind == EXORL_AGENT_TD3_BC) dmu += 2.0f * dspec.inv_bg / (float)nout * (mu_v - ad_v);
            dv = dlive ? dmu * (1.0f - mu_v * mu_v) : 0.f;
        } else if (dlive) {
            dv = dout_value(dspec, net, row0 + dr, dj, rows, nout, lam);
        }
        ds[threadIdx.x] = dv;
    }
    if constexpr (MET) {
        __shared__ float bc_s[2];
        if (threadIdx.x < HB_ROWS * 16) {
            const float d = dlive ? mu_v - ad_v : 0.f;
            const float sq = wave_sum(d * d);
            if ((threadIdx.x & 63) == 0) bc_s[threadIdx.x >> 6] = sq;
        }
        __syncthreads();
        if (threadIdx.x == 0) dspec.bc_part[blockIdx.x] = bc_s[0] + bc_s[1];
    }
    __syncthreads();
    const int64_t nh = (int64_t)(nout + 1) * H + 16;
    float* Pn = P ? P + ((int64_t)net * gridDim.x + blockIdx.x) * nh : nullptr;
    if (want_params && threadIdx.x < nout) {
        float sj = 0.f;
        for (int r = 0; r < HB_ROWS; ++r) sj += ds[r * 16 + threadIdx.x];
        Pn[(int64_t)(nout + 1) * H + threadIdx.x] = sj;
    }
    if (c4 >= H4) return;
    float4 pb = make_float4(0.f, 0.f, 0.f, 0.f);
#pragma unroll
    for (int r = 0; r < HB_ROWS; ++r) {
        if (r >= nr) break;
        const int64_t o = net * astride + (int64_t)(row0 + r) * H;
        const float4 av = avs[r];
        float4 sacc = make_float4(0.f, 0.f, 0.f, 0.f);
#pragma unroll
        for (int j = 0; j < NO; ++j) {
            const float d = ds[r * 16 + j];
            sacc.x += d * w[j].x; sacc.y += d * w[j].y; sacc.z += d * w[j].z; sacc.w += d * w[j].w;
            pw[j].x += d * av.x; pw[j].y += d * av.y; pw[j].z += d * av.z; pw[j].w += d * av.w;
        }
        float4 v;
        v.x = av.x > 0.f ? sacc.x : 0.f; v.y = av.y > 0.f ? sacc.y : 0.f;
        v.z = av.z > 0.f ? sacc.z : 0.f; v.w = av.w > 0.f ? sacc.w : 0.f;
        if (dz) reinterpret_cast<float4*>(dz + o)[c4] = v;
        if (dzb) reinterpret_cast<ushort4*>(dzb + o)[c4] = f4_to_bf4(v);
        if (dzl) reinterpret_cast<ushort4*>(dzl + o)[c4] = f4_to_bf4_lo(v);
        pb.x += v.x; pb.y += v.y; pb.z += v.z; pb.w += v.w;
    }
    if (want_params) {
#pragma unroll
        for (int j = 0; j < NO; ++j)
            if (j < nout) reinterpret_cast<float4*>(Pn + (int64_t)j * H)[c4] = pw[j];
        reinterpret_cast<float4*>(Pn + (int64_t)nout * H)[c4] = pb;
    }
}

int head_bwd(const DoutSpec& dspec, const float* W, const float* a, float* dz, const Planes& dzq, float* P, int rows,
             int H, int nout, int nets, int64_t astride, int64_t pstride, int want_params, hipStream_t s, bool metrics) {
    unsigned short *dz_bf16 = dzq.hi, *dz_lo = dzq.lo;
    EXORL_REQUIRE(nout >= 1 && nout <= 16 && H % 4 == 0 && H <= 1024, "head_bwd: nout=%d H=%d unsupported", nout, H);
    dim3 grid(cdiv(rows, HB_ROWS), nets);
    if (metrics) {
        EXORL_REQUIRE(dspec.mode == EXORL_DOUT_ACTOR_MU && dspec.kind == EXORL_AGENT_TD3_BC && nets == 1 && dspec.bc_part,
                      "head_bwd: the metrics variant is TD3+BC's actor gradient on one net");
        if (nout == 1) hipLaunchKernelGGL((head_bwd_kernel<1, true>), grid, dim3(256), 0, s, dspec, W, a, dz, dz_bf16, P, rows, H, nout, astride, pstride, want_params, dz_lo);
        else if (nout <= 8) hipLaunchKernelGGL((head_bwd_kernel<8, true>), grid, dim3(256), 0, s, dspec, W, a, dz, dz_bf16, P, rows, H, nout, astride, pstride, want_params, dz_lo);
        else hipLaunchKernelGGL((head_bwd_kernel<16, true>), grid, dim3(256), 0, s, dspec, W, a, dz, dz_bf16, P, rows, H, nout, astride, pstride, want_params, dz_lo);
// ... 380 lines not shown
```

exorl_amd/csrc/gemm.hip:

```cpp
#include <algorithm>
#include <type_traits>
#include <vector>

#include "kernels.h"

namespace exorl {
static int g_tune_variant = 0;
static int g_prec_override = 0;
int tune_variant() { return g_tune_variant; }
int prec_override_mask() { return g_prec_override; }
}
extern "C" int exorl_gemm_tune(int32_t variant) {
    exorl::g_tune_variant = variant < 0 ? 0 : variant;
    return 0;
}
extern "C" int exorl_debug_precision_override(int32_t mask) {
    exorl::g_prec_override = mask;
    return 0;
}

namespace exorl {

struct GemmProfile {
    bool on = false;
// ... 779 lines not shown
        constexpr int pair = I / TERMS, term = I % TERMS, ua = pair / SB, ub = pair % SB;
        if constexpr (term == 0) acc[pair] = __builtin_amdgcn_mfma_f32_32x32x16_bf16(f.bh[ub].v, f.ah[ua].v, acc[pair], 0, 0, 0);
        else if constexpr (term == 1) accx[pair] = __builtin_amdgcn_mfma_f32_32x32x16_bf16(f.bl[ub].v, f.ah[ua].v, accx[pair], 0, 0, 0);
        else if constexpr (term == 2) accx[pair] = __builtin_amdgcn_mfma_f32_32x32x16_bf16(f.bh[ub].v, f.al[ua].v, accx[pair], 0, 0, 0);
        else if constexpr (term == 3) accy[pair] = __builtin_amdgcn_mfma_f32_32x32x16_bf16(f.bt[ub].v, f.ah[ua].v, accy[pair], 0, 0, 0);
        else if constexpr (term == 4) accy[pair] = __builtin_amdgcn_mfma_f32_32x32x16_bf16(f.bh[ub].v, f.at[ua].v, accy[pair], 0, 0, 0);
        else accy[pair] = __builtin_amdgcn_mfma_f32_32x32x16_bf16(f.bl[ub].v, f.al[ua].v, accy[pair], 0, 0, 0);
    };
    auto region = [&](Frags& cur, Frags& nxt, auto has_next, int nst_, auto nq, auto nfill, int fst, auto chunk) {
        constexpr bool HN = decltype(has_next)::value;
        constexpr int NFILL = decltype(nfill)::value;
        constexpr int F0 = decltype(chunk)::value * NP / 2, F1 = (decltype(chunk)::value + 1) * NP / 2;
        g16p_static_for<0, NM>([&](auto ic) {
            constexpr int I = decltype(ic)::value;
            mfma_one(cur, ic);
            __builtin_amdgcn_sched_barrier(0);
            if constexpr (HN) g16p_static_for<I * FPG, ((I + 1) * FPG < NF ? (I + 1) * FPG : NF)>([&](auto jc) { read_one(nxt, nst_, nq, jc); });
            constexpr int PPG = (F1 - F0 + NM - 1) / NM;
            if constexpr (NFILL > 0)
                g16p_static_for<F0 + I * PPG, (F0 + (I + 1) * PPG < F1 ? F0 + (I + 1) * PPG : F1)>([&](auto pc) { fill_one(fst, pc); });
            __builtin_amdgcn_sched_barrier(0);
        });
        if constexpr (HN) fence(nxt);
    };
    auto wait_landed = [&](auto younger) {
        constexpr int y = decltype(younger)::value;
        asm volatile("s_waitcnt vmcnt(%0)" :: "n"(y * NP) : "memory");
    };
    Frags fr[2];
    using T = std::true_type;
    using F = std::false_type;
    using NoFill = std::integral_constant<int, 0>;
    using Fill = std::integral_constant<int, NP>;
    using C0 = std::integral_constant<int, 0>;
    auto group = [&](auto first, auto last) {
        constexpr bool FIRST = decltype(first)::value, LAST = decltype(last)::value;
        g16p_static_for<0, NSTG>([&](auto sc) {
            constexpr int s = decltype(sc)::value;
            constexpr bool PENDING = s > 0 ? !LAST : !FIRST;
            g16p_static_for<0, NQ - 1>([&](auto qc) {
                constexpr int q = decltype(qc)::value;
                if constexpr (PENDING && q == 0)
                    region(fr[q & 1], fr[(q + 1) & 1], T{}, s, std::integral_constant<int, q + 1>{}, Fill{}, (s + NSTG - 1) % NSTG, std::integral_constant<int, 1>{});
                else
                    region(fr[q & 1], fr[(q + 1) & 1], T{}, s, std::integral_constant<int, q + 1>{}, NoFill{}, 0, C0{});
            });
            Frags& cur = fr[(NQ - 1) & 1];
            Frags& nxt = fr[NQ & 1];
            if constexpr (!LAST || s < NSTG - 1) {
                wait_landed(std::integral_constant<int, LAST ? NSTG - 2 - s : NSTG - 2>{});
                asm volatile("s_waitcnt lgkmcnt(0)" ::: "memory");
                __builtin_amdgcn_s_barrier();
                asm volatile("" ::: "memory");
                __builtin_amdgcn_sched_barrier(0);
                if constexpr (!LAST) region(cur, nxt, T{}, (s + 1) % NSTG, std::integral_constant<int, 0>{}, Fill{}, s, C0{});
                else region(cur, nxt, T{}, (s + 1) % NSTG, std::integral_constant<int, 0>{}, NoFill{}, 0, C0{});
            } else {
                region(cur, nxt, F{}, 0, std::integral_constant<int, 0>{}, NoFill{}, 0, C0{});
            }
        });
    };

    g16p_static_for<0, NSTG>([&](auto sc) { fill(decltype(sc)::value); });
    wait_landed(std::integral_constant<int, NSTG - 1>{});
    __builtin_amdgcn_s_barrier();
    asm volatile("" ::: "memory");
    g16p_static_for<0, NF>([&](auto jc) { read_one(fr[0], 0, std::integral_constant<int, 0>{}, jc); });
    fence(fr[0]);
    if (nst == NSTG) {
        group(T{}, T{});
    } else {
        group(T{}, F{});
        for (int t = NSTG; t + NSTG < nst; t += NSTG) group(F{}, F{});
        group(F{}, T{});
    }

    const bool relu = gb.relu != 0;
    auto total = [&](int pair, int i) {
        if constexpr (X6) return (accy[pair][i] + accx[pair][i]) + acc[pair][i];
        else if constexpr (X3) return accx[pair][i] + acc[pair][i];
        else return acc[pair][i];
    };
    if (P.head_part) {
#pragma unroll
        for (int ta = 0; ta < SA; ++ta) {
            float dot = 0.f;
#pragma unroll
            for (int tb = 0; tb < SB; ++tb) {
                const int nb = n0 + wn * WC + tb * 32 + 4 * h;
#pragma unroll
                for (int g4 = 0; g4 < 4; ++g4) {
                    const float4 bias = P.bias ? *reinterpret_cast<const float4*>(P.bias + nb + 8 * g4) : make_float4(0.f, 0.f, 0.f, 0.f);
                    const float4 w = *reinterpret_cast<const float4*>(P.head_w + nb + 8 * g4);
                    float4 v;
                    v.x = total(ta * SB + tb, 4 * g4 + 0) + bias.x;
                    v.y = total(ta * SB + tb, 4 * g4 + 1) + bias.y;
                    v.z = total(ta * SB + tb, 4 * g4 + 2) + bias.z;
                    v.w = total(ta * SB + tb, 4 * g4 + 3) + bias.w;
                    if (relu) { v.x = fmaxf(v.x, 0.f); v.y = fmaxf(v.y, 0.f); v.z = fmaxf(v.z, 0.f); v.w = fmaxf(v.w, 0.f); }
                    dot += (v.x * w.x + v.y * w.y) + (v.z * w.z + v.w * w.w);
                }
            }
            dot += __shfl_xor(dot, 32);
            if (h == 0) P.head_part[(int64_t)(m0 + wm * WR + ta * 32 + (lane & 31)) * (P.N / WC) + (n0 / WC + wn)] = dot;
        }
    } else {
#pragma unroll
    for (int ta = 0; ta < SA; ++ta)
#pragma unroll
        for (int tb = 0; tb < SB; ++tb) {
            const int nb = n0 + wn * WC + tb * 32 + 4 * h;
            float* crow = P.C + (int64_t)(m0 + wm * WR + ta * 32 + (lane & 31)) * P.ldc + nb;
#pragma unroll
            for (int g4 = 0; g4 < 4; ++g4) {
                if (P.n_store && nb + 8 * g4 >= P.n_store) continue;
                float4* dst = reinterpret_cast<float4*>(crow + 8 * g4);
                const float4 bias = P.bias ? *reinterpret_cast<const float4*>(P.bias + nb + 8 * g4) : make_float4(0.f, 0.f, 0.f, 0.f);
                float4 v;
                v.x = total(ta * SB + tb, 4 * g4 + 0) + bias.x;
                v.y = total(ta * SB + tb, 4 * g4 + 1) + bias.y;
                v.z = total(ta * SB + tb, 4 * g4 + 2) + bias.z;
                v.w = total(ta * SB + tb, 4 * g4 + 3) + bias.w;
                if (relu) { v.x = fmaxf(v.x, 0.f); v.y = fmaxf(v.y, 0.f); v.z = fmaxf(v.z, 0.f); v.w = fmaxf(v.w, 0.f); }
                if (gb.accumulate) { const float4 o = *dst; v.x += o.x; v.y += o.y; v.z += o.z; v.w += o.w; }
                *dst = v;
            }
        }
    }
}
template <int TN>
__device__ __forceinline__ bool g16p_tile(const Gemm16Batch& gb, int& pidx, int& m0, int& n0) {
    constexpr int SH = TN == 128 ? 7 : 6;
    if (gb.xcd_map) {
        const XcdTile xt = xcd_tile(blockIdx.x, gb.count, gb.p[0].M >> 7, gb.p[0].N >> SH);
        if (!xt.ok) return false;
        pidx = xt.p; m0 = xt.tm << 7; n0 = xt.tn << SH;
        return true;
    }
    pidx = blockIdx.z;
    const int tiles_n = gb.p[pidx].N >> SH, ntiles = tiles_n * (gb.p[pidx].M >> 7);
    if ((int)blockIdx.x >= ntiles) return false;
    m0 = ((int)blockIdx.x / tiles_n) << 7;
    n0 = ((int)blockIdx.x % tiles_n) << SH;
    return true;
}

template <bool AT, bool BT, int NPL, int TN, int KS = 32, int NSTG = 4>
__global__ __launch_bounds__(256) void gemm16p_kernel(const Gemm16Batch gb) {
    extern __shared__ __attribute__((aligned(16))) unsigned char smem_p[];
    int pidx, m0, n0;
    if (!g16p_tile<TN>(gb, pidx, m0, n0)) return;
    gemm16p_body<AT, BT, NPL, TN, KS, NSTG>(gb, smem_p, pidx, m0, n0);
}

template <int NPL, int TN>
__global__ __launch_bounds__(256) void gemm16p_mixed_kernel(const Gemm16Batch gb) {
    extern __shared__ __attribute__((aligned(16))) unsigned char smem_p[];
    int pidx, m0, n0;
    if (!g16p_tile<TN>(gb, pidx, m0, n0)) return;
    if (gb.a_t[pidx]) gemm16p_body<true, true, NPL, TN, 32, 4>(gb, smem_p, pidx, m0, n0);
    else gemm16p_body<false, true, NPL, TN, 32, 4>(gb, smem_p, pidx, m0, n0);
}
constexpr int g16p_lds(int npl, int tn, int ks = 32, int nstg = 4) { return nstg * npl * (2 + tn / 64) * 64 * 2 * ks; }
static_assert(g16p_lds(3, 64) == 147456, "three planes, 128 x 64 tile, four k32 stages");

static bool g16p_uniform(const Gemm16Batch& gb, int count, int tn) {
    if (!(count == 1 || count == 2 || count == 4)) return false;
    const int X = 8 / count, sm = X == 8 ? 4 : 2, sn = X == 2 ? 1 : 2;
    for (int i = 0; i < count; ++i) {
        if (gb.p[i].M != gb.p[0].M || gb.p[i].N != gb.p[0].N) return false;
        if ((gb.p[i].M / 128) % sm != 0 || (gb.p[i].N / tn) % sn != 0) return false;
    }
    return true;
}
template <typename K>
static int g16p_launch(K kernel, Gemm16Batch& gb, int count, int npl, int tn, hipStream_t s, int ks = 32, int nstg = 4) {
    const int lds = g16p_lds(npl, tn, ks, nstg);
    static std::vector<const void*> enabled;
    if (std::find(enabled.begin(), enabled.end(), (const void*)kernel) == enabled.end()) {
        EXORL_CHECK_HIP(hipFuncSetAttribute((const void*)kernel, hipFuncAttributeMaxDynamicSharedMemorySize, lds));
        enabled.push_back((const void*)kernel);
    }
    gb.count = count;
    gb.xcd_map = g16p_uniform(gb, count, tn) ? 1 : 0;
    int tmax = 0, ttot = 0;
    for (int i = 0; i < count; ++i) { const int t = (gb.p[i].M >> 7) * (gb.p[i].N / tn); tmax = t > tmax ? t : tmax; ttot += t; }
    hipLaunchKernelGGL(kernel, gb.xcd_map ? dim3(ttot, 1, 1) : dim3(tmax, 1, count), dim3(256), lds, s, gb);
// ... 80 lines not shown
    if constexpr (NPL == 3 && (F == Form::mixed || TN != 64)) { set_error("gemm16: no three-plane kernel of this form"); return 2; }
    else if constexpr (F == Form::mixed) return g16p_launch(gemm16p_mixed_kernel<NPL, TN>, gb, count, NPL, TN, s);
    else if constexpr (F == Form::row_row && X3) return g16p_launch(gemm16p_kernel<false, false, 2, TN, 64, 2>, gb, count, 2, TN, s, 64, 2);
    else return g16p_launch(gemm16p_kernel<F == Form::k_k, F != Form::row_row, NPL, TN>, gb, count, NPL, TN, s);
}

template <Form F>
static int launch16(Gemm16Batch& gb, int count, const Facts16& f, Pick16 pk, hipStream_t s) {
    constexpr bool MIXED = F == Form::mixed;
    constexpr int AL = F == Form::k_k, BL = F != Form::row_row;
    gb.swizzle = 1;
    const dim3 grid64(f.t64, 1, count), grid128(f.t128x64, 1, count), block(256);
    ProfBracket prof;
    EXORL_TRY(prof.begin(s, f.flops));
    switch (pk.family) {
    case Family::p:
        if (f.has_mid) EXORL_TRY((launch16p<F, 3, 64>(gb, count, s)));
        else if (f.has_lo) EXORL_TRY((pk.tn == 128 ? launch16p<F, 2, 128>(gb, count, s) : launch16p<F, 2, 64>(gb, count, s)));
        else EXORL_TRY((pk.tn == 128 ? launch16p<F, 1, 128>(gb, count, s) : launch16p<F, 1, 64>(gb, count, s)));
        break;
    case Family::x3:
        if constexpr (MIXED) hipLaunchKernelGGL(gemm16x3_mixed_kernel, grid64, block, 0, s, gb);
        else hipLaunchKernelGGL((gemm16x3_kernel<AL != 0, BL != 0>), grid64, block, 0, s, gb);
        break;
    case Family::g:
        if constexpr (MIXED) hipLaunchKernelGGL(gemm16g_mixed_kernel, grid64, block, 0, s, gb);
        else hipLaunchKernelGGL((gemm16g_kernel<AL != 0, BL != 0>), grid64, block, 0, s, gb);
        break;
    case Family::reg:
        if constexpr (!MIXED) {
            const bool exact = f.m_div >= 128 && f.n_div >= 64 && f.k_div >= 64, big = f.t128x64 * count >= 256;
            if (exact && big) hipLaunchKernelGGL((gemm16_kernel<AL, BL, 128, 3, false>), grid128, block, 0, s, gb);
            else if (exact) hipLaunchKernelGGL((gemm16_kernel<AL, BL, 64, 3, false>), grid64, block, 0, s, gb);
            else if (big) hipLaunchKernelGGL((gemm16_kernel<AL, BL, 128, 2, true>), grid128, block, 0, s, gb);
            else hipLaunchKernelGGL((gemm16_kernel<AL, BL, 64, 2, true>), grid64, block, 0, s, gb);
        }
        break;
    case Family::none: break;
    }
    EXORL_LAUNCH_CHECK();
    return prof.end(s);
}

static bool pk3_has_mid(const Gemm16Problem* probs, int count) {
    for (int i = 0; i < count; ++i)
        if (probs[i].A_mid || probs[i].B_mid) return true;
    return false;
}
int gemm16_head_slots(const Gemm16Problem* probs, int count) {
    if (count < 1 || count > 4) return 0;
    Gemm16Batch gb;
    memset(&gb, 0, sizeof(gb));
    const Pick16 pk = pick16(gather16(probs, count, gb));
    if (pk.family != Family::p || pk3_has_mid(probs, count)) return 0;
    for (int i = 0; i < count; ++i)
        if (probs[i].N != probs[0].N) return 0;
    return probs[0].N / (pk.tn / 2);
}

int gemm16_grouped(int a_layout, int b_layout, const Gemm16Problem* probs, int count, bool relu, bool accumulate, hipStream_t s) {
    EXORL_REQUIRE(count >= 1 && count <= 4, "gemm16_grouped: count %d out of range", count);
    for (int i = 0; i < count; ++i) {
        const Gemm16Problem& p = probs[i];
        EXORL_REQUIRE(p.M > 0 && p.N > 0 && p.K > 0, "gemm16_grouped: empty problem %d", i);
        auto ok = [](const unsigned short* ptr, int64_t ld, int R, int K, int layout) {
            const uintptr_t a = reinterpret_cast<uintptr_t>(ptr);
            if (layout == 0) return (a % 16 == 0) && (ld % 8 == 0) && (K % 8 == 0);
            return (a % 4 == 0) && (ld % 2 == 0) && (R % 2 == 0);
        };
        EXORL_REQUIRE(ok(p.A, p.lda, p.M, p.K, a_layout) && ok(p.B, p.ldb, p.N, p.K, b_layout),
                      "gemm16_grouped: problem %d (M=%d N=%d K=%d lda=%lld ldb=%lld) violates the bf16 path's alignment rules "
                      "(hidden_dim and batch must be multiples of 8 in bf16 precision)", i, p.M, p.N, p.K, (long long)p.lda, (long long)p.ldb);
    }
    Gemm16Batch gb;
    memset(&gb, 0, sizeof(gb));
    const Facts16 f = gather16(probs, count, gb);
    const Pick16 pk = pick16(f);
    gb.relu = relu ? 1 : 0;
    gb.accumulate = accumulate ? 1 : 0;
    for (int i = 0; i < count; ++i)
        if (probs[i].head_part)
            EXORL_REQUIRE(probs[i].head_w && a_layout == 0 && b_layout == 0 && !accumulate && gemm16_head_slots(probs, count) > 0,
                          "gemm16_grouped: a folded head needs a forward launch on the 128 x TN kernels (ask gemm16_head_slots first)");
    EXORL_REQUIRE(!f.has_mid || pk.family == Family::p, "gemm16_grouped: three-plane operands need M %% 128 = 0, N %% 64 = 0, K %% 128 = 0 (K >= 128), 16-byte aligned "
                  "hi/mid/lo planes with pitches that are multiples of 8, 16-byte aligned C and bias, ldc %% 4 = 0 (problem 0: M=%d N=%d K=%d)",
                  probs[0].M, probs[0].N, probs[0].K);
    for (int i = 0; i < count; ++i)
        EXORL_REQUIRE(!f.has_mid || !probs[i].head_part, "gemm16_grouped: no folded head on three-plane operands");
    EXORL_REQUIRE(pk.family != Family::none, "gemm16_grouped: split-bf16 operands need M, N, K multiples of 64 and 16-byte aligned hi/lo planes");
    if (a_layout == 0 && b_layout == 0) return launch16<Form::row_row>(gb, count, f, pk, s);
    if (a_layout == 0 && b_layout == 1) return launch16<Form::row_k>(gb, count, f, pk, s);
    if (a_layout == 1 && b_layout == 1) return launch16<Form::k_k>(gb, count, f, pk, s);
    set_error("gemm16_grouped: unsupported layout combination %d %d", a_layout, b_layout);
    return 2;
}

int gemm16_grouped_mixed(const int* a_layouts, const Gemm16Problem* probs, int count, hipStream_t s) {
    EXORL_REQUIRE(count >= 1 && count <= 4, "gemm16_grouped_mixed: count %d out of range", count);
    Gemm16Batch gb;
    memset(&gb, 0, sizeof(gb));
    const Facts16 f = gather16(probs, count, gb);
    EXORL_REQUIRE(!f.has_mid, "gemm16_grouped_mixed: three-plane operands have no mixed wgrad + dgrad form");
    const Pick16 pk = pick16(f);
    bool ok = f.ab16 && f.m_div >= 64 && f.n_div >= 64 && f.k_div >= 256 && pk.family != Family::none;
    for (int i = 0; i < count; ++i) {
        gb.a_t[i] = a_layouts[i] != 0;
        ok = ok && probs[i].M > 0 && !probs[i].bias;
    }
    if (!ok) {
        for (int i = 0; i < count; ++i) EXORL_TRY(gemm16_grouped(a_layouts[i], 1, probs + i, 1, false, false, s));
        return 0;
    }
    EXORL_REQUIRE(pk.family != Family::reg, "gemm16_grouped_mixed: the register-staged kernel has no mixed form");
    return launch16<Form::mixed>(gb, count, f, pk, s);
}

template <int PREC, int AL, int BL>
static int launch_layout(const GemmBatch& gb, int count, int max_tiles, bool vec, hipStream_t s) {
    dim3 grid(max_tiles, 1, count), block(256);
    double flops = 0;
    for (int i = 0; i < count; ++i) flops += 2.0 * gb.p[i].M * (double)gb.p[i].N * gb.p[i].K;
    ProfBracket prof;
    EXORL_TRY(prof.begin(s, flops));
    constexpr size_t dyn = PREC == EXORL_PREC_BF16X6 ? 6 * TILEB : 0;
    if constexpr (PREC == EXORL_PREC_BF16X6) {
        static bool attr = false;
        if (!attr) {
            EXORL_CHECK_HIP(hipFuncSetAttribute((const void*)gemm_kernel<PREC, AL, BL, true>, hipFuncAttributeMaxDynamicSharedMemorySize, (int)dyn));
            EXORL_CHECK_HIP(hipFuncSetAttribute((const void*)gemm_kernel<PREC, AL, BL, false>, hipFuncAttributeMaxDynamicSharedMemorySize, (int)dyn));
            attr = true;
        }
    }
    if (vec) hipLaunchKernelGGL((gemm_kernel<PREC, AL, BL, true>), grid, block, dyn, s, gb);
    else     hipLaunchKernelGGL((gemm_kernel<PREC, AL, BL, false>), grid, block, dyn, s, gb);
    EXORL_LAUNCH_CHECK();
    return prof.end(s);
}

template <int PREC>
static int launch_prec(const GemmBatch& gb, int count, int al, int bl, int max_tiles, bool vec, hipStream_t s) {
    if (al == 0 && bl == 0) return launch_layout<PREC, 0, 0>(gb, count, max_tiles, vec, s);
    if (al == 0 && bl == 1) return launch_layout<PREC, 0, 1>(gb, count, max_tiles, vec, s);
    if (al == 1 && bl == 1) return launch_layout<PREC, 1, 1>(gb, count, max_tiles, vec, s);
    if (al == 1 && bl == 0) return launch_layout<PREC, 1, 0>(gb, count, max_tiles, vec, s);
    set_error("gemm: bad layout %d %d", al, bl);
    return 2;
}

static bool aligned_for_vec(const GemmProblem& p, int al, int bl) {
    auto ok = [](const float* ptr, int64_t ld, int R, int K, int layout) {
        const uintptr_t a = reinterpret_cast<uintptr_t>(ptr);
        if (layout == 0) return (a % 16 == 0) && (ld % 4 == 0) && (K % 4 == 0);
        return (a % 8 == 0) && (ld % 2 == 0) && (R % 2 == 0);
    };
    return ok(p.A, p.lda, p.M, p.K, al) && ok(p.B, p.ldb, p.N, p.K, bl);
}

struct PlaneArena { unsigned char* buf = nullptr; size_t bytes = 0; };
static PlaneArena g_plane_arena;
static bool g_plane_capture_ok = false, g_plane_captured = false;
static size_t* g_plane_probe = nullptr;

__global__ __launch_bounds__(256) void to_planes_kernel(const float* __restrict__ src, int64_t ld, int rows, int cols, unsigned short* __restrict__ hi,
                                                        unsigned short* __restrict__ lo, int rows_p, int cols_p) {
    const int64_t groups = (int64_t)rows_p * (cols_p / 8);
    const bool vec = (ld % 4 == 0) && (reinterpret_cast<uintptr_t>(src) % 16 == 0);
// ... 338 lines not shown
```

exorl_amd/csrc/kernels.h:

```cpp
#pragma once
#include <vector>

#include "common.h"

namespace exorl {

struct TensorDesc { int64_t off, rows, cols; };

struct SimpleCarver {
    float* base; int64_t off = 0;
    explicit SimpleCarver(float* b) : base(b) {}
    float* take(int64_t n) { float* p = base ? base + off : nullptr; off += round_up(n, 64); return p; }
};

struct Planes {
    unsigned short *hi = nullptr, *mid = nullptr, *lo = nullptr;
    Planes at(int64_t off) const { return Planes{hi ? hi + off : nullptr, mid ? mid + off : nullptr, lo ? lo + off : nullptr}; }
    explicit operator bool() const { return hi != nullptr; }
};

struct GemmProblem {
    const float* A;
    const float* B;
    float* C;
    const float* bias;
    int M, N, K;
    int64_t lda, ldb, ldc;
};
int gemm_grouped(int precision, int a_layout, int b_layout, const GemmProblem* probs, int count, bool relu,
                 bool accumulate, hipStream_t s);
void gemm_planes_capture(bool allow, size_t* probe);
int gemm_planes_reserve(size_t bytes);

struct Gemm16Problem {
    const unsigned short* A;
    const unsigned short* B;
    float* C;
    const float* bias;
    int M, N, K;
    int64_t lda, ldb, ldc;
    const unsigned short* A_lo = nullptr;
    const unsigned short* B_lo = nullptr;
    const float* head_w = nullptr;
    float* head_part = nullptr;
    int n_store = 0;
    const unsigned short* A_mid = nullptr;
    const unsigned short* B_mid = nullptr;
};
int to_planes3(const float* src, int64_t ld, int rows, int cols, unsigned short* hi, unsigned short* mid, unsigned short* lo, int rows_p, int cols_p,
               int nb, int64_t src_stride, int64_t dst_stride, hipStream_t s);
int gemm16_head_slots(const Gemm16Problem* probs, int count);
int gemm16_grouped(int a_layout, int b_layout, const Gemm16Problem* probs, int count, bool relu, bool accumulate, hipStream_t s);
int gemm16_grouped_mixed(const int* a_layouts, const Gemm16Problem* probs, int count, hipStream_t s);

int ln_tanh_fwd(const float* z, const float* gain, const float* beta, float* h, float* xhat, float* rstd,
                int rows, int H, int nets, int64_t astride, int64_t pstride, hipStream_t s);
int ln_tanh_bwd(const float* dh, const float* h, const float* xhat, const float* rstd, const float* gain, float* dz,
                int rows, int H, int nets, int64_t astride, int64_t pstride, hipStream_t s);
int ln_param_grad(const float* dh, const float* h, const float* xhat, float* dgain, float* dbeta,
                  int rows, int H, int nets, int64_t astride, int64_t pstride, hipStream_t s);
int colsum(const float* x, float* out, int rows, int cols, int nets, int64_t astride, int64_t pstride, hipStream_t s);
int relu_bwd_colsum(float* x, const float* act, float* out, int rows, int cols, hipStream_t s);
int linear_splitk(int prec, const float* x, int64_t ldx, const float* W, const float* b, float* out, int rows, int F, int K, float* scratch,
                  int splits, hipStream_t s);
int head_fwd(const float* a, const float* W, const float* b, float* out, int rows, int H, int nout, int tanh_out,
             int nets, int64_t astride, int64_t pstride, int64_t ostride, hipStream_t s);
int head_bwd_dx(const float* dout, const float* W, const float* a, float* dz, int rows, int H, int nout,
                int nets, int64_t astride, int64_t pstride, int64_t dstride, hipStream_t s);
int head_bwd_params(const float* dout, const float* a, const float* dz, float* dW, float* db_hidden, float* db_out,
                    int rows, int H, int nout, int nets, int64_t astride, int64_t pstride, int64_t dstride, hipStream_t s);

int trunk_fwd(const float* x, int64_t ldx, const float* W0T, const float* b0, const float* gain, const float* beta,
              float* h, float* xhat, float* rstd, unsigned short* h_bf16, unsigned short* xhat_bf16, int rows, int in_dim,
              int H, int nets, int64_t astride, int64_t pstride, int64_t tstride, hipStream_t s);
struct TrunkItem { const float* x; const unsigned short* W0b; const float *b0, *gain, *beta; float* rstd; unsigned short *hb, *xhb;
                   const unsigned short* W0l; unsigned short *hl, *xhl; };
struct TrunkBatch { TrunkItem it[4]; };
int trunk_fwd16_batch(const TrunkBatch& tb, int count, int64_t ldx, int rows, int in_dim, int H, hipStream_t s);
struct HeadItem { const float* a; const float* W; const float* b; float* out; };
struct HeadBatch { HeadItem it[4]; };
int head_fwd1_batch(const HeadBatch& hb, int count, int rows, int H, hipStream_t s);
bool trunk_fwd16_supported(int H);
int trunk_fwd16(const float* x, int64_t ldx, const Planes& W0q, const float* b0, const float* gain, const float* beta, float* rstd,
                const Planes& hq, const Planes& xhatq, int rows, int in_dim, int H, int nets, int64_t astride, int64_t pstride, hipStream_t s);
int ln_bwd(float* dh, const float* h, const float* xhat, const Planes& hq, const Planes& xhatq, const float* rstd, const float* gain, float* P,
           int rows, int H, int nets, int64_t astride, int64_t pstride, int want_params, hipStream_t s, const float* w0t, int64_t tstride,
           float* dx, int dx_cols, const float* beta);
int trunk_chunks(int rows);
int64_t knn_scratch_floats(int n_src, int n_tgt);
int knn_topk(const float* src, int n_src, const float* tgt, int n_tgt, int dim, int k, float* out, float* d2, hipStream_t s);
int outer_reduce(const float* u, int64_t ldu, int J, const float* v, float* P, int rows, int H, int nets, int64_t vstride,
                 hipStream_t s);
int outer_chunks(int rows);
struct SampleSpec {
    const float* stddev_ptr;
    const float *noise_c, *noise_a;
    uint64_t seed;
    const uint64_t* counter_ptr;
    float stddev, clip;
    float *dst_next, *dst_pi;
    int64_t dst_ld;
    int B;
};
int head_fwd4(const float* a, const float* W, const float* b, float* out, int rows, int H, int nout, int tanh_out,
              int nets, int64_t astride, int64_t pstride, int64_t ostride, hipStream_t s, const SampleSpec* sample = nullptr);
#define EXORL_DOUT_BUFFER   0
#define EXORL_DOUT_TD       1
#define EXORL_DOUT_ACTOR_Q  2
#define EXORL_DOUT_CQL_ACTOR 4
#define EXORL_DOUT_ACTOR_MU 3
struct DoutSpec {
    int mode;
    union {
        const float* buf;
        float* bc_part;
    };
    const float *q, *tq, *reward, *discount;
    const float* stats;
    const float *da, *mu, *a_data;
    const float* w;
    const float *raw, *z;
    const float* alpha_ptr;
    uint64_t seed, counter; const uint64_t* counter_ptr;
    const float* task;
    int64_t task_ld;
    const float* lam_parts;
    int lam_chunks;
    int da_nets;
    int kind;
    int use_lambda;
    float inv_bg, alpha, stddev;
    const float* stddev_ptr;
};
int head_bwd(const DoutSpec& dspec, const float* W, const float* a, float* dz, const Planes& dzq, float* P, int rows,
             int H, int nout, int nets, int64_t astride, int64_t pstride, int want_params, hipStream_t s, bool metrics = false);
int head_chunks(int rows);
int tune_variant();
constexpr int TUNE_CONV_WGRAD_TILE = 64;
constexpr int TUNE_ACT_GENERIC = 256;
constexpr int TUNE_CONV_PER_IMAGE = 8388608;
constexpr int TUNE_ADAPTER_PADDED = 134217728;
constexpr int TUNE_CONV_STRIP = 1073741824;
int prec_override_mask();
struct QHeadArgs {
    const float* a[4];
    const float* W[4];
    const float* b[4];
    float *q, *tq;
    const float *reward, *discount;
    float* dz; unsigned short* dzb; unsigned short* dzl; int64_t act;
    float* P;
    float* abs_part;
    const float* tpart[2];
    int tslots;
    int rows, H, mode;
    float inv_bg;
};
int qhead(const QHeadArgs& q, hipStream_t s, bool metrics = false);
int qhead_chunks(int rows);
__device__ __forceinline__ float chunk_sum(const float* __restrict__ p, int n, int64_t stride) {
    float acc = 0.f;
    int ch = 0;
    if (n > 1024) {
        for (; ch + 32 <= n; ch += 32) {
            float t[32], sub = 0.f;
#pragma unroll
            for (int q = 0; q < 32; ++q) t[q] = p[(int64_t)(ch + q) * stride];
#pragma unroll
            for (int q = 0; q < 32; ++q) sub += t[q];
            acc += sub;
        }
    }
    for (; ch + 32 <= n; ch += 32) {
        float t[32];
#pragma unroll
        for (int q = 0; q < 32; ++q) t[q] = p[(int64_t)(ch + q) * stride];
#pragma unroll
        for (int q = 0; q < 32; ++q) acc += t[q];
    }
    for (; ch + 16 <= n; ch += 16) {
        float t[16];
#pragma unroll
        for (int q = 0; q < 16; ++q) t[q] = p[(int64_t)(ch + q) * stride];
#pragma unroll
        for (int q = 0; q < 16; ++q) acc += t[q];
    }
    for (; ch < n; ++ch) acc += p[(int64_t)ch * stride];
    return acc;
}

struct FinalizeArgs {
    const float* Ph; int head_chunks; int n_heads; int64_t head_stride;
    int64_t gW2, gb1, gb2;
    const float* Pt; int trunk_chunks; int n_trunks; int64_t trunk_stride;
    const float* Pw; int w_chunks;
    int64_t gW0, gb0, gg, gbeta;
    int H, nout, in_dim;
    float* G;
};
int finalize_grads(const FinalizeArgs& f, hipStream_t s);

__device__ __forceinline__ float polyak(float p, float t, float tau, float one_minus_tau) {
#pragma clang fp contract(off)
    const float a = tau * p;
    const float b = one_minus_tau * t;
    return a + b;
}
struct AdamConst;
struct FusedAdamArgs {
    float *p, *g, *m, *v, *target;
    const AdamConst* c;
    int n_heads; int64_t w1_off[2];
    unsigned long long* bump;
};
struct ShadowSpec;
int finalize_adam(const FinalizeArgs& f, const FusedAdamArgs& a, const ShadowSpec& sh, hipStream_t s);

struct ShadowSpec {
    int n_trunks, n_heads, in_dim, H;
    int64_t w0_off[2], w1_off[2];
    float* w0t;
    unsigned short* w1b;
    unsigned short* w0b;
    float* t_w0t;
    unsigned short* t_w1b;
    unsigned short* t_w0b;
    unsigned short *w1l, *w0l, *t_w1l, *t_w0l;
};
int refresh_shadows(const float* p, int64_t n, const ShadowSpec& sh, bool target, hipStream_t s);

struct NoiseSpec {
    const float* buf;
    uint64_t seed;
    uint64_t counter;
    const uint64_t* counter_ptr;
};

struct AdamConst {
    float one_minus_b1, b2, one_minus_b2, bc2_sqrt, eps, neg_step_size, tau, one_minus_tau;
};

__device__ __forceinline__ void adam_elem(float& p, float g, float& m, float& v, const AdamConst& c) {
#pragma clang fp contract(off)
    m = m + c.one_minus_b1 * (g - m);
    v = v * c.b2 + (c.one_minus_b2 * g) * g;
    const float denom = sqrtf(v) / c.bc2_sqrt + c.eps;
    p = p + (c.neg_step_size * m) / denom;
}

struct StepState {
    uint64_t replay_counter;
    uint64_t noise_counter;
    long long t_actor, t_critic;
    double b1t, b2t_actor_unused, b1t_c, b2t_c;
    double b2t;
    AdamConst actor, critic;
    double lr, b1, b2, eps, tau;
    int has_critic;
    float stddev;
};
int step_begin(StepState* st, int advance_replay, hipStream_t s);

struct IntrStepState {
    uint64_t counter;
    uint64_t draw_counter;
    long long t;
    long long queue_ptr;
    long long qrow0;
    int queue_size, num_protos;
    int draws;
    double b1t, b2t;
    double b1, b2, eps;
    double lr[3];
    AdamConst c[3];
};
constexpr int ACT_FAST_ROWS = 2;
struct ActFast {
    const float *x_dev, *x_host;
    const float *w0t, *P;
    int64_t b0, g, beta, W1, b1, W2, b2;
    float* part; unsigned int* ticket;
    const float *noise_dev, *noise_host;
    uint64_t seed, counter;
    float* out;
    float stddev;
    int rows, in_dim, H, nout, eval_mode;
    int first_relu = 0; int64_t W0 = 0;
};
bool act_fast_supported(int rows, int in_dim, int H, int nout);
int act_fast(const ActFast& f, hipStream_t s);
int trunk_one(const float* x, const float* meta, const float* W, const float* b, const float* gain, const float* beta, float* part, unsigned int* ticket,
              float* out, int R, int M, int F, hipStream_t s);
int reduce_pairs(const float* parts, int chunks, float* out, hipStream_t s);
struct MetricsWindowArgs {
    const float *crit_part, *abs_part, *bc_part;
    int q_chunks, bc_chunks;
    int fused;
    int kind, act_dim, ent_from_std;
    float inv_bg, alpha;
    const float* stddev;
    float* metrics;
    double* sums; long long* steps;
};
int metrics_window(const MetricsWindowArgs& w, hipStream_t s);
int set_device_float(float* dst, float value, hipStream_t s);
int set_device_u64(uint64_t* dst, uint64_t value, hipStream_t s);

__host__ __device__ inline void fill_adam_const(AdamConst& c, double b1t, double b2t, double lr, double b1, double b2, double eps, double tau) {
    const double bc1 = 1.0 - b1t;
    const double bc2 = 1.0 - b2t;
    c.one_minus_b1 = (float)(1.0 - b1);
    c.b2 = (float)b2;
    c.one_minus_b2 = (float)(1.0 - b2);
    c.bc2_sqrt = (float)sqrt(bc2);
    c.eps = (float)eps;
    c.neg_step_size = (float)(-(lr / bc1));
    c.tau = (float)tau;
    c.one_minus_tau = (float)(1.0 - tau);
}

__device__ inline void step_begin_device(StepState* st, int advance_replay) {
    if (advance_replay) st->replay_counter += 1;
    st->noise_counter += 2;
    st->t_actor += 1;
    st->b1t *= st->b1;
    st->b2t *= st->b2;
    fill_adam_const(st->actor, st->b1t, st->b2t, st->lr, st->b1, st->b2, st->eps, 0.0);
    if (st->has_critic) {
        st->t_critic += 1;
        st->b1t_c *= st->b1;
        st->b2t_c *= st->b2;
        fill_adam_const(st->critic, st->b1t_c, st->b2t_c, st->lr, st->b1, st->b2, st->eps, st->tau);
    }
}


__device__ inline void intr_step_begin_device(IntrStepState* st) {
    st->t += 1;
    st->b1t *= st->b1;
    st->b2t *= st->b2;
    for (int i = 0; i < 3; ++i) fill_adam_const(st->c[i], st->b1t, st->b2t, st->lr[i], st->b1, st->b2, st->eps, 0.0);
    st->draw_counter = st->counter;
    st->counter += (uint64_t)st->draws;
    st->qrow0 = st->queue_ptr;
    if (st->queue_size > 0) st->queue_ptr = (st->queue_ptr + st->num_protos) % st->queue_size;
}

int prepare_inputs(const float* obs, const float* action, const float* next_obs, float* xa, float* xc_cur,
                   float* xc_next, float* xc_pi, int B, int O, int A, int has_critic, StepState* st, int advance_replay,
                   hipStream_t s);
int sample_actions2(const float* mu2, const float* noise_c, const float* noise_a, uint64_t seed, const uint64_t* counter_ptr,
                    float stddev, float clip, float* dst_next, float* dst_pi, int64_t dst_ld, int B, int A, hipStream_t s,
                    const float* stddev_ptr = nullptr);
int sample_action(const float* mu, NoiseSpec noise, float stddev, float clip, int use_clip, float* dst, int64_t dst_ld,
                  int B, int A, float* logprob_sum, hipStream_t s, const float* stddev_ptr = nullptr, int world_size = 1);
struct CqlNoise {
    const float *z_next, *u_rand, *z_cur, *z_nxt, *z_actor;
    uint64_t seed;
    const uint64_t* counter_ptr;
};
struct CqlScalars {
    float log_alpha, m, v, alpha;
};
int cql_build_inputs(const float* obs, const float* action, const float* raw2, CqlNoise nz, float* xc_next, float* x_all, int B,
                     int O, int A, int n, hipStream_t s);
int cql_critic_dq(const float* q_all, const float* tq, const float* reward, const float* discount, float* dq_all, float* metrics,
                  int B, int n, float cql_alpha, float inv_bg, hipStream_t s, CqlScalars* lag = nullptr, const AdamConst* c_dev = nullptr,
                  float target_penalty = 0.f,
                  int mode = 0, float* gsum = nullptr);
int cql_actor_sample(const float* raw_obs, CqlNoise nz, float* xc_pi, int64_t ld, float* stats, int B, int O, int A, hipStream_t s);
int cql_alpha_step(CqlScalars* sc, const float* stats, const AdamConst* c_dev, float* metrics, int B, int A, float inv_bg, const float* q,
                   hipStream_t s);
int cql_act(const float* raw, const float* noise, uint64_t seed, uint64_t counter, int eval_mode, float* out, int rows, int A, hipStream_t s);
int head_bwd_wide(const DoutSpec& dspec, const float* W, const float* a, float* dz, const Planes& dzq, float* P, int rows, int H,
                  int nout, int64_t astride, int64_t pstride, int want_params, hipStream_t s);

int repeat_sample(const float* obs, const float* mu, const float* noise, uint64_t seed, const uint64_t* counter_ptr, uint64_t counter,
                  float stddev, float clip, float* xc_rep, int B, int O, int A, int n, hipStream_t s, const float* stddev_ptr = nullptr);
int crr_weights(const float* q_rep, const float* q_data, float* w, int B, int n, int weight_func, hipStream_t s);
// ... 54 lines not shown
```

exorl_amd/csrc/loss.hip:

```cpp
#include "kernels.h"

namespace exorl {

template <int NV>
__device__ __forceinline__ void block_sum(float (&v)[NV], float (*sm)[16]) {
    const int lane = threadIdx.x & 63, wave = threadIdx.x >> 6;
    const int nw = (blockDim.x + 63) >> 6;
#pragma unroll
    for (int i = 0; i < NV; ++i) {
        const float s = wave_sum(v[i]);
        if (lane == 0) sm[i][wave] = s;
    }
    __syncthreads();
#pragma unroll
    for (int i = 0; i < NV; ++i) {
        float t = 0.f;
        for (int w = 0; w < nw; ++w) t += sm[i][w];
        v[i] = t;
    }
    __syncthreads();
}

__global__ void prepare_inputs_kernel(const float* __restrict__ obs, const float* __restrict__ action,
                                      const float* __restrict__ next_obs, float* __restrict__ xa,
// ... 476 lines not shown
}

int actor_dq(const float* q, const float* stats, float* dq, int B, float inv_bg, float alpha, int use_lambda,
             hipStream_t s) {
    hipLaunchKernelGGL(actor_dq_kernel, dim3(cdiv(B, 256)), dim3(256), 0, s, q, stats, dq, B, inv_bg, alpha, use_lambda);
    EXORL_LAUNCH_CHECK();
    return 0;
}

__global__ __launch_bounds__(1024) void actor_dmu_kernel(const float* __restrict__ da, int64_t da_ld, int da_nets,
                                                         int64_t da_net_stride,
                                                         const float* __restrict__ mu, const float* __restrict__ a_data,
                                                         const float* __restrict__ reward, const float* __restrict__ w,
                                                         float* __restrict__ dpre, const float* __restrict__ stats,
                                                         float* __restrict__ metrics, int B, int A, float inv_bg,
                                                         float alpha, int kind, float stddev_val, const float* stddev_ptr) {
    const float stddev = stddev_ptr ? *stddev_ptr : stddev_val;
    __shared__ float sm[2][16];
    float v[2] = {0.f, 0.f};
    if (reward)
        for (int m = threadIdx.x; m < B; m += blockDim.x) v[1] += reward[m];
    const float bc_coef = 2.0f * inv_bg / (float)A;
    const float inv_var = 1.0f / (stddev * stddev);
    const float log_norm = -__logf(stddev) - 0.9189385332046727f;
    for (int i = threadIdx.x; i < B * A; i += blockDim.x) {
        const int m = i / A, j = i % A;
        const float mv = mu[i];
        float dmu;
        if (kind == EXORL_AGENT_TD3_BC) {
            const float d = mv - a_data[i];
            float dav = 0.f;
            for (int t = 0; t < da_nets; ++t) dav += da[t * da_net_stride + (int64_t)m * da_ld + j];
            dmu = dav + bc_coef * d;
            v[0] += d * d;
        } else if (kind == EXORL_AGENT_BC) {
            const float d = a_data[i] - mv;
            dmu = -d * inv_var * inv_bg;
            v[0] += d * d * 0.5f * inv_var - log_norm;
        } else if (kind == EXORL_AGENT_CRR) {
            const float d = a_data[i] - mv;
            dmu = -w[m] * d * inv_var * inv_bg;
            v[0] += w[m] * (d * d * 0.5f * inv_var - log_norm);
        } else {
            dmu = 0.f;
            for (int t = 0; t < da_nets; ++t) dmu += da[t * da_net_stride + (int64_t)m * da_ld + j];
        }
        dpre[i] = dmu * (1.0f - mv * mv);
    }
    block_sum<2>(v, sm);
    if (threadIdx.x == 0) {
        if (reward) metrics[EXORL_M_BATCH_REWARD] = v[1] * inv_bg;
        float loss;
        if (kind == EXORL_AGENT_TD3_BC) {
            const float lambda = alpha / (stats[0] * inv_bg);
            loss = -lambda * metrics[EXORL_M_Q_SUM] * inv_bg + v[0] * inv_bg / (float)A;
            metrics[EXORL_M_BC_SUM] = v[0];
        } else if (kind == EXORL_AGENT_BC || kind == EXORL_AGENT_CRR) {
            loss = v[0] * inv_bg;
        } else {
            loss = -metrics[EXORL_M_Q_SUM] * inv_bg;
        }
        metrics[EXORL_M_ACTOR_LOSS] = loss;
    }
}

int actor_dmu(const float* da, int64_t da_ld, int da_nets, int64_t da_net_stride, const float* mu, const float* a_data, const float* reward, const float* w, float* dpre, float* stats,
              float* metrics, int B, int A, float inv_bg, float alpha, int kind, float stddev, hipStream_t s, const float* stddev_ptr) {
    hipLaunchKernelGGL(actor_dmu_kernel, dim3(1), dim3(1024), 0, s, da, da_ld, da_nets, da_net_stride, mu, a_data, reward, w, dpre, stats, metrics, B, A,
                       inv_bg, alpha, kind, stddev, stddev_ptr);
    EXORL_LAUNCH_CHECK();
    return 0;
}

static_assert(EXORL_N_METRICS < 64, "metrics_window_kernel: thread EXORL_N_METRICS of the one wave counts the step");
__global__ __launch_bounds__(64) void metrics_window_kernel(const MetricsWindowArgs w) {
    __shared__ float tot[9];
    __shared__ float m[EXORL_N_METRICS];
    const int t = threadIdx.x;
    const float old = w.metrics[t < EXORL_N_METRICS ? t : 0];
    const float sd = *w.stddev;
    if (w.fused) {
        const int k = t < 9 ? t : 8;
        const float* p = k < 6 ? w.crit_part + k : (k < 8 ? w.abs_part + (k - 6) : w.bc_part);
        const float sum = chunk_sum(p, t >= 9 ? 0 : (k < 8 ? w.q_chunks : w.bc_chunks), k < 6 ? 6 : (k < 8 ? 2 : 1));
        if (t < 9) tot[t] = sum;
    }
    if (t < EXORL_N_METRICS) m[t] = old;
    __syncthreads();
    if (t == 0) {
        if (w.fused) {
            m[EXORL_M_BATCH_REWARD] = tot[0] * w.inv_bg;
            m[EXORL_M_CRITIC_TARGET_Q] = tot[1] * w.inv_bg;
            m[EXORL_M_CRITIC_Q1] = tot[2] * w.inv_bg;
            m[EXORL_M_CRITIC_Q2] = tot[3] * w.inv_bg;
            m[EXORL_M_CRITIC_LOSS] = (tot[4] + tot[5]) * w.inv_bg;
            m[EXORL_M_Q_ABS_SUM] = tot[6];
            m[EXORL_M_Q_SUM] = tot[7];
            if (w.kind == EXORL_AGENT_TD3_BC) {
                const float lambda = w.alpha / (tot[6] * w.inv_bg);
                m[EXORL_M_ACTOR_LOSS] = -lambda * tot[7] * w.inv_bg + tot[8] * w.inv_bg / (float)w.act_dim;
                m[EXORL_M_BC_SUM] = tot[8];
            } else {
                m[EXORL_M_ACTOR_LOSS] = -tot[7] * w.inv_bg;
            }
        }
        if (w.ent_from_std) m[EXORL_M_ACTOR_ENT] = (1.4189385332046727f + logf(sd)) * (float)w.act_dim;
    }
    __syncthreads();
    if (t < EXORL_N_METRICS) {
        const float v = m[t];
        w.metrics[t] = v;
        w.sums[t] += (double)v;
    }
    if (t == EXORL_N_METRICS) *w.steps += 1;
}

int metrics_window(const MetricsWindowArgs& w, hipStream_t s) {
    hipLaunchKernelGGL(metrics_window_kernel, dim3(1), dim3(64), 0, s, w);
    EXORL_LAUNCH_CHECK();
    return 0;
}

}

extern "C" int exorl_debug_philox_normal(uint64_t seed, uint64_t counter, int64_t n, float* out_dev, void* stream) {
    using namespace exorl;
    EXORL_REQUIRE(out_dev && n > 0 && n <= (int64_t)1 << 31, "debug_philox_normal: bad arguments");
    hipLaunchKernelGGL(debug_philox_normal_kernel, dim3(cdiv(n, 256) > 4096 ? 4096 : cdiv(n, 256)), dim3(256), 0, as_stream(stream), seed, counter, n, out_dev);
    EXORL_LAUNCH_CHECK();
    return 0;
}
```

exorl_amd/engine.py:

```python
import ctypes as C

import numpy as np
import torch

from . import _lib as L

KIND = {'td3_bc': L.AGENT_TD3_BC, 'td3': L.AGENT_TD3, 'bc': L.AGENT_BC, 'ddpg': L.AGENT_DDPG, 'crr': L.AGENT_CRR, 'cql': L.AGENT_CQL,
        'aps': L.AGENT_APS}
PRECISION = {'fp32': L.PREC_F32, 'f32': L.PREC_F32, 'bf16': L.PREC_BF16, 'bf16x3': L.PREC_BF16X3, 'bf16x6': L.PREC_BF16X6}
METRIC_KEYS = {L.M_BATCH_REWARD: 'batch_reward', L.M_CRITIC_TARGET_Q: 'critic_target_q', L.M_CRITIC_Q1: 'critic_q1',
               L.M_CRITIC_Q2: 'critic_q2', L.M_CRITIC_LOSS: 'critic_loss', L.M_ACTOR_LOSS: 'actor_loss',
               L.M_ACTOR_LOGPROB: 'actor_logprob'}


def _require_gpu(device):
    if not torch.cuda.is_available():
        raise L.ExorlError('exorl_amd needs a HIP device (torch.cuda.is_available() is False); there is no CPU path')
    dev = torch.device(device)
    if dev.type != 'cuda':
        raise L.ExorlError(f"exorl_amd agents run on the GPU only; got device={device!r}")
    return dev


class _Phased:
# ... 103 lines not shown
        na = self._dev(noise_actor) if noise_actor is not None else None
        L.check(self.lib.exorl_agent_update_phase(self.h, phase, stddev, L.ptr(nc), L.ptr(na), L.current_stream()))
        self._keep_noise = (nc, na)

    def update_steps(self, stddev, noise_critic=None, noise_actor=None):
        phase = lambda p: self.update_phase(p, stddev, noise_critic, noise_actor)
        if self.lagrange:
            phase(4)
            yield self.stats(), L.XCHG_SUM
            phase(5)
        else:
            phase(0)
        if self.has_critic:
            yield self.flat(L.NET_CRITIC, L.T_GRAD), L.XCHG_SUM
        phase(1)
        if self.kind in ('td3_bc', 'cql'):
            yield self.stats(), L.XCHG_SUM
        phase(2)
        yield self.flat(L.NET_ACTOR, L.T_GRAD), L.XCHG_SUM
        phase(3)

    def run_update(self, *a, **k):
        if self.comm is not None:
            return self.update(*a, **k)
        self._run(self.update, self.update_steps, *a, **k)

    def act(self, obs, stddev, eval_mode, noise=None):
        o = self._dev(obs).view(-1, self.obs_dim)
        n = o.shape[0]
        out = torch.empty(n, self.act_dim, dtype=torch.float32, device=self.device)
        nz = self._dev(noise) if noise is not None else None
        L.check(self.lib.exorl_agent_act(self.h, o.data_ptr(), n, stddev, int(eval_mode), L.ptr(nz), out.data_ptr(),
                                         L.current_stream()))
        return out

    def act_host(self, obs, stddev, eval_mode, noise=None):
        if self.kind == 'cql' or self.hidden_dim % 4 != 0 or self.obs_dim > 256:
            return None
        slot = getattr(self, '_act_slot', None)
        if slot is None:
            slot = self._act_slot = torch.zeros(64, dtype=torch.float32).pin_memory()
        o = np.ascontiguousarray(np.asarray(obs, np.float32).reshape(-1))
        assert o.size == self.obs_dim, (o.size, self.obs_dim)
        nz = None if noise is None else np.ascontiguousarray(np.asarray(noise, np.float32).reshape(-1))
        stream = L.current_stream()
        L.check(self.lib.exorl_agent_act_host(self.h, o.ctypes.data, 1, float(stddev), int(eval_mode), nz.ctypes.data if nz is not None else None,
                                              slot.data_ptr(), stream))
        torch.cuda.current_stream(self.device).synchronize()
        return slot[:self.act_dim].numpy().copy()

    def set_comm(self, comm):
        L.check(self.lib.exorl_agent_set_comm(self.h, comm.h if comm is not None else None))
        self.comm = comm

    def enable_graph(self, replay_engine, nstep, gamma, stddev):
        L.check(self.lib.exorl_agent_enable_graph(self.h, replay_engine.h, nstep, gamma, stddev, L.current_stream()))
        self.graph_captures = getattr(self, 'graph_captures', 0) + 1

    def enable_graph_intr(self, replay_engine, nstep, gamma, stddev, intr=None, batch=None, meta_dim=0):
        L.check(self.lib.exorl_agent_enable_graph_intr(self.h, intr.h if intr is not None else None, C.byref(batch) if batch is not None else None,
                                                       meta_dim, replay_engine.h, nstep, gamma, stddev, L.current_stream()))
        self._graph_keep = (intr, batch)
        self.graph_captures = getattr(self, 'graph_captures', 0) + 1

    def disable_graph(self):
        L.check(self.lib.exorl_agent_disable_graph(self.h))
        self._graph_keep = None

    def step_graph(self, stddev):
        L.check(self.lib.exorl_agent_step_graph(self.h, stddev, L.current_stream()))

    def noise_counter(self):
        c = C.c_uint64()
        L.check(self.lib.exorl_agent_noise_counter(self.h, C.byref(c), L.current_stream()))
        return int(c.value)

    def philox_normal(self, seed, counter, shape):
        out = torch.empty(tuple(shape), dtype=torch.float32, device=self.device)
        L.check(self.lib.exorl_debug_philox_normal(seed, counter, out.numel(), out.data_ptr(), L.current_stream()))
        return out

    def poison_scratch(self):
        L.check(self.lib.exorl_debug_agent_poison_scratch(self.h, L.current_stream()))

    def weight_images(self, net):
        w = L.WeightImages()
        L.check(self.lib.exorl_debug_agent_weight_images(self.h, net, C.byref(w)))
        H, kp = w.hidden_dim, (w.in_dim + 31) // 32 * 32

        def planes(ptr, shape):
            if not ptr:
                return None
            n = int(np.prod(shape))
            return self._view(ptr, (n + 1) // 2).view(torch.int16)[:n].view(*shape)
        out = {'w0t': self._view(w.w0t, w.n_trunks * w.in_dim * H).view(w.n_trunks, w.in_dim, H)}
        for k in ('w0_hi', 'w0_lo'):
            out[k] = planes(getattr(w, k), (w.n_trunks, H, kp))
        for k in ('w1_hi', 'w1_mid', 'w1_lo'):
            out[k] = planes(getattr(w, k), (w.n_heads, H, H))
        return out

    def set_parallel_branches(self, enable):
        L.check(self.lib.exorl_agent_set_parallel_branches(self.h, int(bool(enable))))

    def set_metrics(self, enable):
        L.check(self.lib.exorl_agent_set_metrics(self.h, int(bool(enable))))

    def metric_window_bytes(self):
        return int(self.lib.exorl_agent_metric_window_bytes(C.byref(self.cfg)))

    def set_metric_window(self, buf=True):
        if buf is None:
            L.check(self.lib.exorl_agent_set_metric_window(self.h, None, 0))
            self._window = None
            return
        if buf is True:
            buf = torch.empty(self.metric_window_bytes(), dtype=torch.uint8, device=self.device)
        torch.cuda.current_stream(self.device).synchronize()
        L.check(self.lib.exorl_agent_set_metric_window(self.h, buf.data_ptr(), buf.numel()))
        self._window = buf

    def metric_window_read(self, reset=True):
        sums, steps = np.zeros(L.N_METRICS, np.float64), C.c_int64()
        L.check(self.lib.exorl_agent_metric_window_read(self.h, sums.ctypes.data, C.byref(steps), int(bool(reset)), L.current_stream()))
        return sums, int(steps.value)

    def cql_alpha_state(self):
        host = np.zeros(6, np.float32)
        L.check(self.lib.exorl_agent_cql_alpha(self.h, host.ctypes.data, 0))
        return host

    def set_cql_alpha_state(self, log_alpha, m=0.0, v=0.0, log_critic_alpha=0.0, cm=0.0, cv=0.0):
        host = np.array([log_alpha, m, v, log_critic_alpha, cm, cv], np.float32)
        L.check(self.lib.exorl_agent_cql_alpha(self.h, host.ctypes.data, 1))

    def metrics_raw(self):
        host = np.zeros(L.N_METRICS, np.float32)
        L.check(self.lib.exorl_agent_metrics(self.h, host.ctypes.data, L.current_stream()))
        return host

    def opt_steps(self):
        a, c = C.c_int64(), C.c_int64()
        L.check(self.lib.exorl_agent_opt_steps(self.h, C.byref(a), C.byref(c)))
        return a.value, c.value

    def set_opt_steps(self, actor_steps, critic_steps):
        L.check(self.lib.exorl_agent_set_opt_steps(self.h, actor_steps, critic_steps))


class IntrEngine(_Phased):
    KINDS = {'rnd': L.INTR_RND, 'icm': L.INTR_ICM, 'icm_apt': L.INTR_ICM_APT, 'disagreement': L.INTR_DISAGREEMENT, 'diayn': L.INTR_DIAYN,
             'proto': L.INTR_PROTO, 'aps': L.INTR_APS, 'smm': L.INTR_SMM}

    def __init__(self, kind, obs_dim, act_dim, hidden_dim, batch, rep_dim=0, lr=1e-4, scale=1.0, knn_k=12, knn_avg=True,
                 knn_rms=True, knn_clip=0.0, clip_val=5.0, n_models=0, num_protos=0, queue_size=0, tau=0.1, target_tau=0.05, sp_lr=1e-3, vae_lr=1e-2,
                 vae_beta=0.5, state_ent_coef=1.0, latent_ent_coef=1.0, latent_cond_ent_coef=1.0, goal=(150.0, 75.0), precision='fp32',
                 device='cuda', encoded=False, world_size=1, rank=0):
        self.device = _require_gpu(device)
        self.kind, self.batch, self.obs_dim, self.act_dim = kind, batch, obs_dim, act_dim
        self.world_size, self.rank = world_size, rank
        cfg = L.IntrCfg(self.KINDS[kind], obs_dim, act_dim, hidden_dim, rep_dim, batch, PRECISION[precision], knn_k, int(bool(knn_avg)),
                             int(bool(knn_rms)), n_models, 1 if encoded else 0, lr, scale, knn_clip, clip_val, num_protos, queue_size, tau, target_tau,
                             sp_lr, vae_lr, vae_beta, state_ent_coef, latent_ent_coef, latent_cond_ent_coef, goal[0], goal[1], world_size, rank)
        self._create('intr', cfg)
        rms, bn, nbn = C.c_void_p(), C.c_void_p(), C.c_int64()
        L.check(self.lib.exorl_intr_state(self.h, C.byref(rms), C.byref(bn), C.byref(nbn)))
# ... 439 lines not shown
```

include/exorl_hip.h:

```cpp
#ifndef EXORL_HIP_H
#define EXORL_HIP_H

#include <stddef.h>
#include <stdint.h>

#ifdef __cplusplus
extern "C" {
#endif

#define EXORL_ABI_VERSION 12

const char* exorl_last_error(void);
int exorl_abi_version(void);
int exorl_device_info(char* name_out, int name_len, int* num_cus, int64_t* hbm_bytes);

typedef struct exorl_replay exorl_replay_t;

typedef struct {
    int32_t obs_bytes;
    int32_t act_dim;
    int32_t meta_dim;
    int32_t max_episodes;
    int64_t capacity_rows;
} exorl_replay_cfg;
// ... 61 lines not shown
#define EXORL_PREC_BF16X6 3

#define EXORL_NET_ACTOR         0
#define EXORL_NET_CRITIC        1
#define EXORL_NET_CRITIC_TARGET 2

#define EXORL_T_PARAM 0
#define EXORL_T_GRAD  1
#define EXORL_T_ADAM_M 2
#define EXORL_T_ADAM_V 3

#define EXORL_M_BATCH_REWARD    0
#define EXORL_M_CRITIC_TARGET_Q 1
#define EXORL_M_CRITIC_Q1       2
#define EXORL_M_CRITIC_Q2       3
#define EXORL_M_CRITIC_LOSS     4
#define EXORL_M_ACTOR_LOSS      5
#define EXORL_M_ACTOR_LOGPROB   6
#define EXORL_M_Q_ABS_SUM       7
#define EXORL_M_Q_SUM           8
#define EXORL_M_BC_SUM          9
#define EXORL_M_CRITIC_CQL        10
#define EXORL_M_CRITIC_CQL_LOGSUM 11
#define EXORL_M_ACTOR_ALPHA       12
#define EXORL_M_ACTOR_ALPHA_LOSS  13
#define EXORL_M_ACTOR_ENT         14
#define EXORL_N_METRICS        16

typedef struct {
    int32_t kind;
    int32_t obs_dim, act_dim, hidden_dim;
    int32_t batch;
    int32_t precision;
    int32_t world_size;
    int32_t sf_dim;
    float   lr, tau, alpha, stddev_clip;
    uint64_t seed;
    int32_t num_value_samples;
    int32_t weight_func;
    int32_t n_samples;
    int32_t use_critic_lagrange;
    float   target_cql_penalty;
    int32_t reserved3;
} exorl_agent_cfg;

size_t exorl_agent_workspace_bytes(const exorl_agent_cfg* cfg);
int exorl_agent_create(const exorl_agent_cfg* cfg, void* workspace_dev, size_t workspace_bytes,
                       exorl_agent_t** out);
int exorl_agent_destroy(exorl_agent_t* a);
int exorl_agent_num_tensors(exorl_agent_t* a, int32_t net, int32_t* n);
int exorl_agent_tensor(exorl_agent_t* a, int32_t net, int32_t index, int32_t what,
                       void** ptr_dev, int64_t* rows, int64_t* cols);
int exorl_agent_flat(exorl_agent_t* a, int32_t net, int32_t what, void** ptr_dev, int64_t* numel);
int exorl_agent_params_changed(exorl_agent_t* a, int32_t sync_target, void* stream);
int exorl_agent_batch_slots(exorl_agent_t* a, exorl_batch_out* out);
int exorl_agent_set_batch(exorl_agent_t* a, const float* obs_dev, const float* action_dev,
                          const float* reward_dev, const float* discount_dev, const float* next_obs_dev,
                          void* stream);
int exorl_agent_update(exorl_agent_t* a, float stddev, const float* noise_critic_dev,
                       const float* noise_actor_dev, void* stream);
int exorl_agent_update_phase(exorl_agent_t* a, int32_t phase, float stddev, const float* noise_critic_dev,
                             const float* noise_actor_dev, void* stream);
int exorl_agent_stats_buffer(exorl_agent_t* a, void** ptr_dev, int64_t* numel);
int exorl_agent_set_comm(exorl_agent_t* a, exorl_comm_t* c);
int exorl_agent_cql_alpha(exorl_agent_t* a, float* log_alpha_host, int32_t set);
int exorl_agent_act(exorl_agent_t* a, const float* obs_dev, int32_t n, float stddev, int32_t eval_mode,
                    const float* noise_dev, float* action_out_dev, void* stream);
int exorl_agent_act_host(exorl_agent_t* a, const float* obs_host, int32_t n, float stddev, int32_t eval_mode,
                         const float* noise_host, float* action_out, void* stream);
int exorl_agent_metrics(exorl_agent_t* a, float* metrics_host, void* stream);
int exorl_agent_set_metrics(exorl_agent_t* a, int32_t enable);
size_t exorl_agent_metric_window_bytes(const exorl_agent_cfg* cfg);
int exorl_agent_set_metric_window(exorl_agent_t* a, void* buf_dev, size_t bytes);
int exorl_agent_metric_window_read(exorl_agent_t* a, double* sums_host, int64_t* steps_host, int32_t reset, void* stream);
int exorl_agent_set_parallel_branches(exorl_agent_t* a, int32_t enable);
int exorl_agent_opt_steps(exorl_agent_t* a, int64_t* actor_steps, int64_t* critic_steps);
int exorl_agent_set_opt_steps(exorl_agent_t* a, int64_t actor_steps, int64_t critic_steps);
int exorl_agent_enable_graph(exorl_agent_t* a, exorl_replay_t* r, int32_t nstep, float gamma, float stddev, void* stream);
int exorl_agent_step_graph(exorl_agent_t* a, float stddev, void* stream);
int exorl_agent_disable_graph(exorl_agent_t* a);
int exorl_agent_noise_counter(exorl_agent_t* a, uint64_t* counter_out, void* stream);
int exorl_debug_philox_normal(uint64_t seed, uint64_t counter, int64_t n, float* out_dev, void* stream);
int exorl_debug_agent_poison_scratch(exorl_agent_t* a, void* stream);
typedef struct {
    int32_t n_trunks, n_heads, in_dim, hidden_dim;
    float* w0t;
    uint16_t *w0_hi, *w0_lo;
    uint16_t *w1_hi, *w1_mid, *w1_lo;
} exorl_weight_images;
int exorl_debug_agent_weight_images(exorl_agent_t* a, int32_t net, exorl_weight_images* out);

int exorl_gemm(int32_t precision, int32_t a_layout, int32_t b_layout, int32_t M, int32_t N, int32_t K,
               const float* A_dev, int64_t lda, const float* B_dev, int64_t ldb, float* C_dev, int64_t ldc,
               const float* bias_dev, int32_t relu, int32_t accumulate, void* stream);
int exorl_gemm_bf16(int32_t a_layout, int32_t b_layout, int32_t M, int32_t N, int32_t K, const uint16_t* A_dev, int64_t lda,
                    const uint16_t* B_dev, int64_t ldb, float* C_dev, int64_t ldc, const float* bias_dev, int32_t relu,
                    int32_t accumulate, void* stream);
int exorl_gemm_planes(int32_t count, const int32_t* a_layouts, int32_t b_layout, int32_t M, int32_t N, int32_t K,
                      const uint16_t* const* A_hi_dev, const uint16_t* const* A_lo_dev, int64_t lda,
                      const uint16_t* const* B_hi_dev, const uint16_t* const* B_lo_dev, int64_t ldb,
                      float* const* C_dev, int64_t ldc, int32_t relu, void* stream);
int exorl_gemm_planes3(int32_t count, const int32_t* a_layouts, int32_t b_layout, int32_t M, int32_t N, int32_t K,
                       const uint16_t* const* A_hi_dev, const uint16_t* const* A_mid_dev, const uint16_t* const* A_lo_dev, int64_t lda,
                       const uint16_t* const* B_hi_dev, const uint16_t* const* B_mid_dev, const uint16_t* const* B_lo_dev, int64_t ldb,
                       float* const* C_dev, int64_t ldc, int32_t relu, void* stream);
int exorl_gemm_tune(int32_t variant);
int exorl_debug_precision_override(int32_t mask);
int exorl_profile_gemm(int32_t enable);
int exorl_profile_gemm_read(double* flops_out_host, float* ms_out_host, int32_t cap, int32_t* n_out);
int exorl_profile_event_overhead(float* ms_out_host, void* stream);
int exorl_adam_step(float* p_dev, const float* g_dev, float* m_dev, float* v_dev, int64_t n, float lr,
                    float beta1, float beta2, float eps, int64_t t, float* target_dev, float tau, void* stream);
int exorl_soft_update(const float* p_dev, float* target_dev, int64_t n, float tau, void* stream);
int exorl_ln_tanh_fwd(const float* z_dev, const float* gain_dev, const float* beta_dev, float* h_dev,
                      float* xhat_dev, float* rstd_dev, int32_t rows, int32_t H, void* stream);
int exorl_knn_topk(const float* src_dev, int32_t n_src, const float* tgt_dev, int32_t n_tgt, int32_t dim,
                   int32_t k, float* out_dev, void* stream);

#define EXORL_INTR_RND     0
#define EXORL_INTR_ICM     1
#define EXORL_INTR_ICM_APT 2
#define EXORL_INTR_DISAGREEMENT 3
#define EXORL_INTR_DIAYN   4
#define EXORL_INTR_PROTO   5
#define EXORL_INTR_APS     6
#define EXORL_INTR_SMM     7
#define EXORL_MAX_ENSEMBLE 8
#define EXORL_INTR_ENCODED 1

typedef struct exorl_intr_cfg {
    int32_t kind;
    int32_t obs_dim, act_dim, hidden_dim;
    int32_t rep_dim;
    int32_t batch;
    int32_t precision;
    int32_t knn_k, knn_avg, knn_rms;
    int32_t n_models;
    int32_t flags;
    float lr;
    float scale;
    float knn_clip;
    float clip_val;
    int32_t num_protos, queue_size;
    float tau;
    float target_tau;
    float sp_lr, vae_lr, vae_beta;
    float state_ent_coef, latent_ent_coef, latent_cond_ent_coef;
    float goal_x, goal_y;
    int32_t world_size;
    int32_t rank;
} exorl_intr_cfg;

typedef struct exorl_intr exorl_intr_t;

#define EXORL_IM_LOSS        0
#define EXORL_IM_INTR_REWARD 1
#define EXORL_IM_EXTR_REWARD 2
#define EXORL_IM_RMS_MEAN    3
#define EXORL_IM_RMS_STD     4
#define EXORL_IM_ACC         5
#define EXORL_IM_ENT_REWARD  6
#define EXORL_IM_SF_REWARD   7
#define EXORL_N_INTR_METRICS 8

size_t exorl_intr_workspace_bytes(const exorl_intr_cfg* cfg);
int exorl_intr_create(const exorl_intr_cfg* cfg, void* workspace, size_t workspace_bytes, exorl_intr_t** out);
// ... 105 lines not shown
```

Measured before the change: 3323.

## Fold actor-pass critic Q heads into the hidden GEMM and LN backward

In the actor update, the critic's final scalar Q heads are folded into the epilogue of the second-layer grouped bf16 GEMM. That epilogue also writes a relu-gated negative head weight as the upstream gradient planes, which drops the separate run_qhead launch. The Q values, min(Q1,Q2) and the abs/sum partials are then rebuilt from per-slot partials inside the dgrad-only LN backward kernel. The actor dout routes the twin-critic gradient by which Q is smaller. This adds epilogue work and extra shuffles and shared-memory reductions, and applies only to a twin-net bf16 route with no comm.

```diff
diff --git a/exorl_amd/_lib.py b/exorl_amd/_lib.py
--- a/exorl_amd/_lib.py
+++ b/exorl_amd/_lib.py
@@ -173,6 +173,7 @@
     'exorl_agent_noise_counter': (C.c_int, [c_void_p, P(c_uint64), c_void_p]),
     'exorl_debug_philox_normal': (C.c_int, [c_uint64, c_uint64, c_int64, c_void_p, c_void_p]),
     'exorl_debug_agent_poison_scratch': (C.c_int, [c_void_p, c_void_p]),
+    'exorl_debug_agent_head_fold': (C.c_int, [c_void_p, P(C.c_int32)]),
     'exorl_debug_agent_weight_images': (C.c_int, [c_void_p, c_int32, P(WeightImages)]),
     'exorl_agent_disable_graph': (C.c_int, [c_void_p]),
     'exorl_gemm': (C.c_int, [c_int32, c_int32, c_int32, c_int32, c_int32, c_int32, c_void_p, c_int64, c_void_p, c_int64,
diff --git a/exorl_amd/csrc/agent.hip b/exorl_amd/csrc/agent.hip
--- a/exorl_amd/csrc/agent.hip
+++ b/exorl_amd/csrc/agent.hip
@@ -135,7 +135,7 @@
 
 static int net_forward(const NetDesc& d, const float* P, const NetShadow& sh, const float* x, int64_t ldx, int rows,
                        const FwdBufs& f, bool save, bool tanh_out, int prec, hipStream_t s, const SampleSpec* sample = nullptr,
-                       bool no_head = false) {
+                       bool no_head = false, const Planes* gate = nullptr, int* fold_slots = nullptr) {
     const int H = d.H;
     const int64_t act = (int64_t)rows * H;
     const Route rt = route_of(prec, f.h1q, sh.w1q, rows);
@@ -154,6 +154,22 @@
         p[i] = Product{Operand(f.h1, t, f.h1q, t), Operand(P + d.W1, i * d.head_stride, sh.w1q, (int64_t)i * H * H), f.h2 + i * act,
                        P + d.b1 + i * d.head_stride, rows, H, H};
     }
+    if (fold_slots) *fold_slots = 0;
+    if (no_head && gate && fold_slots && bf && d.n_heads == 2 && d.n_trunks == 2 && d.out_dim == 1) {
+        Gemm16Problem q[2];
+        for (int i = 0; i < 2; ++i) q[i] = g16(p[i], H);
+        const int slots = gemm16_head_slots(q, 2);
+        if (slots > 0 && slots <= 32) {
+            for (int i = 0; i < 2; ++i) {
+                q[i].head_w = P + d.W2 + i * d.head_stride;
+                q[i].head_part = f.h2 + i * act;
+                q[i].gate_hi = gate->hi + i * act;
+                q[i].gate_lo = gate->lo ? gate->lo + i * act : nullptr;
+            }
+            *fold_slots = slots;
+            return gemm16_grouped(0, 0, q, 2, true, false, s);
+        }
+    }
     EXORL_TRY(products(rt, prec, 0, 0, p, d.n_heads, H, true, false, s));
     if (no_head) return 0;
     if (H % 4 == 0)
@@ -216,7 +232,8 @@
 
 static int net_backward(const NetDesc& d, const float* P, const NetShadow& sh, float* G, const Partials& pt, const float* x,
                         int64_t ldx, int rows, const FwdBufs& f, const DoutSpec& dout, const BwdBufs& b, float* dx, int dx_col0,
-                        int dx_cols, int prec, hipStream_t s, const Fork& fk, FinalizeArgs* defer = nullptr, bool have_dz2 = false) {
+                        int dx_cols, int prec, hipStream_t s, const Fork& fk, FinalizeArgs* defer = nullptr, bool have_dz2 = false,
+                        const QSlotArgs* qslots = nullptr) {
     const int H = d.H;
     const int64_t act = (int64_t)rows * H;
     const bool paired = d.n_trunks == d.n_heads;
@@ -271,7 +288,7 @@
     const bool dx_fused = dx && !G;
     EXORL_TRY(ln_bwd(b.dh1, f.h1, f.xhat, h1q, xhatq, f.rstd, P + d.g, pt.Pt, rows, H, d.n_trunks, act, d.trunk_stride, G ? 1 : 0, s,
                      dx_fused ? sh.w0t + (int64_t)dx_col0 * H : nullptr, (int64_t)d.in_dim * H, dx_fused ? dx : nullptr, dx_cols,
-                     (bf && trunk_fwd16_supported(H)) ? P + d.beta : nullptr));
+                     (bf && trunk_fwd16_supported(H)) ? P + d.beta : nullptr, qslots));
     if (dx && !dx_fused)
         EXORL_TRY(head_fwd4(b.dh1, sh.w0t + (int64_t)dx_col0 * H, nullptr, dx, rows, H, dx_cols, 0, d.n_trunks, act,
                             (int64_t)d.in_dim * H, (int64_t)rows * dx_cols, s));
@@ -363,6 +380,7 @@
     bool staged_by_sampler = false;
     bool want_metrics = true;
     int tq_slots = 0;
+    int pi_slots = 0;
     double* win_sums = nullptr; long long* win_steps = nullptr;
     float *win_crit = nullptr, *win_bc = nullptr;
 };
@@ -561,7 +579,7 @@
     MetricsWindowArgs w{};
     w.fused = qfuse(a) ? 1 : 0;
     w.crit_part = a->win_crit; w.abs_part = a->abs_part; w.bc_part = a->win_bc;
-    w.q_chunks = qhead_chunks(B); w.bc_chunks = a->cfg.kind == EXORL_AGENT_TD3_BC ? head_chunks(B) : 0;
+    w.q_chunks = qhead_chunks(B); w.abs_chunks = a->pi_slots > 0 ? trunk_chunks(B) : qhead_chunks(B); w.bc_chunks = a->cfg.kind == EXORL_AGENT_TD3_BC ? head_chunks(B) : 0;
     w.kind = a->cfg.kind; w.act_dim = a->cfg.act_dim; w.ent_from_std = a->cfg.kind != EXORL_AGENT_CQL;
     w.inv_bg = a->inv_bg; w.alpha = a->cfg.alpha; w.stddev = &a->state->stddev;
     w.metrics = a->metrics; w.sums = a->win_sums; w.steps = a->win_steps;
@@ -661,8 +679,9 @@
         EXORL_TRY(sample_action(a->fa.out + (int64_t)B * A, noise_spec(a, noise_a, 1), stddev, cfg.stddev_clip, 1, a->xc_pi + O, W, B, A,
                                 a->metrics + EXORL_M_ACTOR_LOGPROB, s, &a->state->stddev, cfg.world_size));
     const bool qf = qfuse(a);
+    a->pi_slots = 0;
     EXORL_TRY(net_forward(a->critic, a->flat[EXORL_NET_CRITIC][EXORL_T_PARAM], a->sh_critic, a->xc_pi, W, B, a->fc, true, false, prec, s,
-                          nullptr, qf));
+                          nullptr, qf, (qf && !a->comm && !(tune_variant() & TUNE_PI_QHEAD)) ? &a->bc.dz2q : nullptr, &a->pi_slots));
     if (cfg.kind == EXORL_AGENT_APS) {
         EXORL_TRY(sf_q(a->fc.out, a->obs + (O - cfg.sf_dim), O, a->sfq, B, cfg.sf_dim, 2, s));
         EXORL_TRY(actor_stats(a->sfq, a->stats, B, s));
@@ -682,7 +701,8 @@
         if (cfg.kind == EXORL_AGENT_APS) { dq.q = a->sfq; dq.task = a->obs + (O - cfg.sf_dim); dq.task_ld = O; }
         dq.use_lambda = cfg.kind == EXORL_AGENT_TD3_BC;
         const bool qf = qfuse(a);
-        if (qf) EXORL_TRY(run_qhead(a, 1, s));
+        const bool folded = qf && a->pi_slots > 0;
+        if (qf && !folded) EXORL_TRY(run_qhead(a, 1, s));
         if (qf && a->comm && dq.use_lambda) {
             EXORL_TRY(reduce_pairs(a->abs_part, qhead_chunks(B), a->stats, s));
             EXORL_CHECK_HIP(hipEventRecord(a->ev_stats_ready, s));
@@ -690,8 +710,11 @@
             EXORL_TRY(comm_allreduce_sum(a->comm, a->stats, 4, a->comm_stream));
             EXORL_CHECK_HIP(hipEventRecord(a->ev_stats_done, a->comm_stream));
         }
-        EXORL_TRY(net_backward(a->critic, a->flat[EXORL_NET_CRITIC][EXORL_T_PARAM], a->sh_critic, nullptr, a->pc, a->xc_pi, W, B, a->fc,
-                               dq, a->bc, a->da, O, A, prec, s, a->fk, nullptr, qf));
+        const NetDesc& d = a->critic;
+        const float* Pc = a->flat[EXORL_NET_CRITIC][EXORL_T_PARAM];
+        const QSlotArgs qs{{a->fc.h2, a->fc.h2 + (int64_t)B * H}, {Pc + d.b2, Pc + d.b2 + d.head_stride}, a->pi_slots, a->fc.out, a->abs_part};
+        EXORL_TRY(net_backward(a->critic, Pc, a->sh_critic, nullptr, a->pc, a->xc_pi, W, B, a->fc,
+                               dq, a->bc, a->da, O, A, prec, s, a->fk, nullptr, qf, folded ? &qs : nullptr));
     }
     const FwdBufs f = a->fa.rows_from(B, H, A);
     if (!a->has_critic)
@@ -704,7 +727,8 @@
     dm.mode = EXORL_DOUT_ACTOR_MU; dm.da = a->da; dm.da_nets = a->has_critic ? a->critic.n_trunks : 0; dm.mu = f.out; dm.a_data = a->action;
     dm.kind = cfg.kind; dm.inv_bg = a->inv_bg; dm.stddev = stddev; dm.stddev_ptr = &a->state->stddev; dm.w = a->crr_w;
     if (qfuse(a)) {
-        dm.lam_parts = a->abs_part; dm.lam_chunks = qhead_chunks(B); dm.use_lambda = cfg.kind == EXORL_AGENT_TD3_BC; dm.alpha = cfg.alpha;
+        if (a->pi_slots > 0) dm.route_q = a->fc.out;
+        dm.lam_parts = a->abs_part; dm.lam_chunks = a->pi_slots > 0 ? trunk_chunks(B) : qhead_chunks(B); dm.use_lambda = cfg.kind == EXORL_AGENT_TD3_BC; dm.alpha = cfg.alpha;
         if (a->comm && dm.use_lambda) {
             EXORL_CHECK_HIP(hipStreamWaitEvent(s, a->ev_stats_done, 0));
             dm.lam_parts = a->stats; dm.lam_chunks = 1;
@@ -1190,6 +1214,12 @@
     return 0;
 }
 
+int exorl_debug_agent_head_fold(exorl_agent_t* a, int32_t* pi_slots) {
+    EXORL_REQUIRE(a && pi_slots, "debug_agent_head_fold: null argument");
+    *pi_slots = a->pi_slots;
+    return 0;
+}
+
 int exorl_debug_agent_poison_scratch(exorl_agent_t* a, void* stream) {
     EXORL_REQUIRE(a, "debug_agent_poison_scratch: null handle");
     hipStream_t s = as_stream(stream);
diff --git a/exorl_amd/csrc/fused.hip b/exorl_amd/csrc/fused.hip
--- a/exorl_amd/csrc/fused.hip
+++ b/exorl_amd/csrc/fused.hip
@@ -516,15 +516,16 @@
     return r;
 }
 
-template <bool PARAMS, bool B16, bool LO, bool RECOMP>
+template <bool PARAMS, bool B16, bool LO, bool RECOMP, bool QP = false>
 __global__ __launch_bounds__(512) void ln_bwd_kernel(float* dh, const float* __restrict__ h, const float* __restrict__ xhat,
                                                      const unsigned short* __restrict__ hb, const unsigned short* __restrict__ xhb,
                                                      const float* __restrict__ rstd, const float* __restrict__ gain,
                                                      float* __restrict__ P, int rows, int H, int64_t astride,
                                                      int64_t pstride, const float* __restrict__ w0t, int64_t tstride,
                                                      float* __restrict__ dx, int dx_cols, const unsigned short* __restrict__ hl,
-                                                     const unsigned short* __restrict__ xhl, int iters, const float* __restrict__ beta) {
+                                                     const unsigned short* __restrict__ xhl, int iters, const float* __restrict__ beta, const QSlotArgs qs) {
     __shared__ __attribute__((aligned(16))) float red[PARAMS ? 3 * 8 * 1024 : 4];
+    __shared__ float qmin_s[QP ? TB_ROWS * 4 : 1];
     const int net = blockIdx.y;
     const int tid = threadIdx.x, lane = tid & 63, wave = tid >> 6;
     const int H4 = H >> 2;
@@ -544,6 +545,12 @@
         float s1 = 0.f, s2 = 0.f;
         float4 dvs[4], hvs[4];
         ushort4 xb[4], xl[4], hbv[4], hlv[4];
+        float qslot = 0.f, qb2 = 0.f;
+        if constexpr (QP) {
+            const int hn = lane >> 5, j = (lane & 31) < qs.slots ? (lane & 31) : 0;
+            qslot = qs.part[hn][(int64_t)row * qs.slots + j];
+            qb2 = qs.b2[hn][0];
+        }
 #pragma unroll
         for (int i = 0; i < 4; ++i) {
             const int cc = lane + 64 * i < H4 ? lane + 64 * i : 0;
@@ -615,6 +622,19 @@
                 if constexpr (PARAMS) { pb0[i].x += v.x; pb0[i].y += v.y; pb0[i].z += v.z; pb0[i].w += v.w; }
             }
         }
+        if constexpr (QP) {
+            if (net == 0) {
+                float qn = 0.f;
+                for (int j = 0; j < qs.slots; ++j) qn += __shfl(qslot, (lane & 32) + j, 64);
+                qn += qb2;
+                const float q1 = __shfl(qn, 0, 64), q2 = __shfl(qn, 32, 64);
+                if (lane == 0) {
+                    qs.q[row] = q1;
+                    qs.q[rows + row] = q2;
+                    qmin_s[it * 8 + wave] = fminf(q1, q2);
+                }
+            }
+        }
         if constexpr (!PARAMS) {
             if (dx) {
                 for (int j0 = 0; j0 < dx_cols; j0 += 8) {
@@ -638,6 +658,19 @@
             }
         }
     }
+    if constexpr (QP) {
+        if (net == 0) {
+            __syncthreads();
+            if (tid == 0) {
+                const int row0 = blockIdx.x * TB_ROWS * iters;
+                const int nr = rows - row0 < TB_ROWS * iters ? rows - row0 : TB_ROWS * iters;
+                float sa = 0.f, sm = 0.f;
+                for (int r = 0; r < nr; ++r) { const float m = qmin_s[r]; sa += fabsf(m); sm += m; }
+                qs.abs_part[2 * blockIdx.x] = sa;
+                qs.abs_part[2 * blockIdx.x + 1] = sm;
+            }
+        }
+    }
     if constexpr (PARAMS) {
         float* Pn = P + ((int64_t)net * gridDim.x + blockIdx.x) * 3 * H;
 #pragma unroll
@@ -664,7 +697,7 @@
 
 int ln_bwd(float* dh, const float* h, const float* xhat, const Planes& hq, const Planes& xhatq, const float* rstd, const float* gain, float* P,
            int rows, int H, int nets, int64_t astride, int64_t pstride, int want_params, hipStream_t s, const float* w0t, int64_t tstride,
-           float* dx, int dx_cols, const float* beta) {
+           float* dx, int dx_cols, const float* beta, const QSlotArgs* qslots) {
     const unsigned short *h_bf16 = hq.hi, *xhat_bf16 = xhatq.hi, *h_lo = hq.lo, *xhat_lo = xhatq.lo;
     EXORL_REQUIRE(H >= 4 && H <= 1024 && H % 4 == 0, "ln_bwd: unsupported H=%d", H);
     EXORL_REQUIRE(!dx || (!want_params && w0t && dx_cols >= 1), "ln_bwd: the dx epilogue belongs to the dgrad-only pass");
@@ -673,7 +706,17 @@
     const int iters = tb_iters(rows);
     EXORL_REQUIRE((h_lo != nullptr) == (xhat_lo != nullptr) && (!h_lo || b16), "ln_bwd: lo planes come in pairs, with the bf16 hi planes");
     const bool lo = h_lo != nullptr, rc = b16 && beta != nullptr;
-#define EXORL_LNB(PA, BB, LL, RR) hipLaunchKernelGGL((ln_bwd_kernel<PA, BB, LL, RR>), grid, dim3(512), 0, s, dh, h, xhat, h_bf16, xhat_bf16, rstd, gain, P, rows, H, astride, pstride, w0t, tstride, dx, dx_cols, h_lo, xhat_lo, iters, beta)
+    const QSlotArgs qs = qslots ? *qslots : QSlotArgs{};
+    if (qslots) {
+        EXORL_REQUIRE(!want_params && dx && b16 && nets == 2 && iters <= 4 && qs.slots >= 1 && qs.slots <= 32 && qs.part[0] && qs.part[1] && qs.b2[0] &&
+                      qs.b2[1] && qs.q && qs.abs_part, "ln_bwd: the folded heads' Q values ride on the dgrad-only pass of a twin net's bf16 route (slots <= 32)");
+#define EXORL_LNQ(LL, RR) hipLaunchKernelGGL((ln_bwd_kernel<false, true, LL, RR, true>), grid, dim3(512), 0, s, dh, h, xhat, h_bf16, xhat_bf16, rstd, gain, P, rows, H, astride, pstride, w0t, tstride, dx, dx_cols, h_lo, xhat_lo, iters, beta, qs)
+        if (lo && rc) EXORL_LNQ(true, true); else if (lo) EXORL_LNQ(true, false); else if (rc) EXORL_LNQ(false, true); else EXORL_LNQ(false, false);
+#undef EXORL_LNQ
+        EXORL_LAUNCH_CHECK();
+        return 0;
+    }
+#define EXORL_LNB(PA, BB, LL, RR) hipLaunchKernelGGL((ln_bwd_kernel<PA, BB, LL, RR>), grid, dim3(512), 0, s, dh, h, xhat, h_bf16, xhat_bf16, rstd, gain, P, rows, H, astride, pstride, w0t, tstride, dx, dx_cols, h_lo, xhat_lo, iters, beta, qs)
 #define EXORL_LNB2(PA) do { if (!b16) EXORL_LNB(PA, false, false, false); \
                              else if (lo && rc) EXORL_LNB(PA, true, true, true); else if (lo) EXORL_LNB(PA, true, true, false); \
                              else if (rc) EXORL_LNB(PA, true, false, true); else EXORL_LNB(PA, true, false, false); } while (0)
@@ -939,7 +982,14 @@
     if (mu_path) {
         const int i = (dlive ? row0 + dr : 0) * nout + (dlive ? dj : 0);
         mu_v = dspec.mu[i];
-        for (int t = 0; t < dspec.da_nets; ++t) da_v += dspec.da[(int64_t)t * rows * nout + i];
+        if (dspec.route_q) {
+            const int m = dlive ? row0 + dr : 0;
+            const float q1 = dspec.route_q[m], q2 = dspec.route_q[rows + m];
+            const float w1 = q1 < q2 ? 1.0f : (q1 == q2 ? 0.5f : 0.0f);
+            for (int t = 0; t < dspec.da_nets; ++t) da_v += (dspec.inv_bg * (t == 0 ? w1 : 1.0f - w1)) * dspec.da[(int64_t)t * rows * nout + i];
+        } else {
+            for (int t = 0; t < dspec.da_nets; ++t) da_v += dspec.da[(int64_t)t * rows * nout + i];
+        }
         if (dspec.kind == EXORL_AGENT_TD3_BC) ad_v = dspec.a_data[i];
     }
     float lam = 1.0f;
diff --git a/exorl_amd/csrc/gemm.hip b/exorl_amd/csrc/gemm.hip
--- a/exorl_amd/csrc/gemm.hip
+++ b/exorl_amd/csrc/gemm.hip
@@ -885,12 +885,15 @@
         else return acc[pair][i];
     };
     if (P.head_part) {
+        auto head_rows = [&](auto with_gate) {
+        constexpr bool gate = decltype(with_gate)::value;
 #pragma unroll
         for (int ta = 0; ta < SA; ++ta) {
             float dot = 0.f;
 #pragma unroll
             for (int tb = 0; tb < SB; ++tb) {
                 const int nb = n0 + wn * WC + tb * 32 + 4 * h;
+                uint2 gh[4], gl[4];
 #pragma unroll
                 for (int g4 = 0; g4 < 4; ++g4) {
                     const float4 bias = P.bias ? *reinterpret_cast<const float4*>(P.bias + nb + 8 * g4) : make_float4(0.f, 0.f, 0.f, 0.f);
@@ -900,12 +903,38 @@
                     v.y = total(ta * SB + tb, 4 * g4 + 1) + bias.y;
                     v.z = total(ta * SB + tb, 4 * g4 + 2) + bias.z;
                     v.w = total(ta * SB + tb, 4 * g4 + 3) + bias.w;
+                    if constexpr (gate) {
+                        const float4 gw = make_float4(v.x > 0.f ? -w.x : 0.f, v.y > 0.f ? -w.y : 0.f, v.z > 0.f ? -w.z : 0.f, v.w > 0.f ? -w.w : 0.f);
+                        gh[g4] = make_uint2(pack_bf16(gw.x, gw.y), pack_bf16(gw.z, gw.w));
+                        gl[g4] = make_uint2(pack_bf16(bf16_residual(gw.x), bf16_residual(gw.y)), pack_bf16(bf16_residual(gw.z), bf16_residual(gw.w)));
+                    }
                     if (relu) { v.x = fmaxf(v.x, 0.f); v.y = fmaxf(v.y, 0.f); v.z = fmaxf(v.z, 0.f); v.w = fmaxf(v.w, 0.f); }
                     dot += (v.x * w.x + v.y * w.y) + (v.z * w.z + v.w * w.w);
+                }
+                {
+                    if constexpr (gate) {
+                        const int64_t o = (int64_t)(m0 + wm * WR + ta * 32 + (lane & 31)) * P.ldc + (n0 + wn * WC + tb * 32 + 8 * h);
+#pragma unroll
+                        for (int gp = 0; gp < 2; ++gp) {
+                            auto swap = [&](const uint2 (&q)[4]) {
+                                const uint2 keep = h ? q[2 * gp + 1] : q[2 * gp], send = h ? q[2 * gp] : q[2 * gp + 1];
+                                const uint2 got = make_uint2(__shfl_xor(send.x, 32), __shfl_xor(send.y, 32));
+                                return h ? make_uint4(got.x, got.y, keep.x, keep.y) : make_uint4(keep.x, keep.y, got.x, got.y);
+                            };
+                            *reinterpret_cast<uint4*>(P.gate_hi + o + 16 * gp) = swap(gh);
+                            if (P.gate_lo) *reinterpret_cast<uint4*>(P.gate_lo + o + 16 * gp) = swap(gl);
+                        }
+                    }
                 }
             }
             dot += __shfl_xor(dot, 32);
             if (h == 0) P.head_part[(int64_t)(m0 + wm * WR + ta * 32 + (lane & 31)) * (P.N / WC) + (n0 / WC + wn)] = dot;
+        }
+        };
+        if constexpr (!AT && !BT && !X6) {
+            if (P.gate_hi) head_rows(std::true_type{}); else head_rows(std::false_type{});
+        } else {
+            head_rows(std::false_type{});
         }
     } else {
 #pragma unroll
@@ -1152,6 +1181,11 @@
         if (probs[i].head_part)
             EXORL_REQUIRE(probs[i].head_w && a_layout == 0 && b_layout == 0 && !accumulate && gemm16_head_slots(probs, count) > 0,
                           "gemm16_grouped: a folded head needs a forward launch on the 128 x TN kernels (ask gemm16_head_slots first)");
+    for (int i = 0; i < count; ++i)
+        if (probs[i].gate_hi || probs[i].gate_lo)
+            EXORL_REQUIRE(probs[i].head_part && probs[i].gate_hi && relu && probs[i].ldc % 8 == 0 && reinterpret_cast<uintptr_t>(probs[i].gate_hi) % 16 == 0 &&
+                          reinterpret_cast<uintptr_t>(probs[i].gate_lo) % 16 == 0,
+                          "gemm16_grouped: the gated head weight is stored beside a folded head (head_part) with relu, into 16-byte aligned planes of pitch ldc %% 8 = 0");
     EXORL_REQUIRE(!f.has_mid || pk.family == Family::p, "gemm16_grouped: three-plane operands need M %% 128 = 0, N %% 64 = 0, K %% 128 = 0 (K >= 128), 16-byte aligned "
                   "hi/mid/lo planes with pitches that are multiples of 8, 16-byte aligned C and bias, ldc %% 4 = 0 (problem 0: M=%d N=%d K=%d)",
                   probs[0].M, probs[0].N, probs[0].K);
diff --git a/exorl_amd/csrc/kernels.h b/exorl_amd/csrc/kernels.h
--- a/exorl_amd/csrc/kernels.h
+++ b/exorl_amd/csrc/kernels.h
@@ -43,6 +43,8 @@
     const unsigned short* B_lo = nullptr;
     const float* head_w = nullptr;
     float* head_part = nullptr;
+    unsigned short* gate_hi = nullptr;
+    unsigned short* gate_lo = nullptr;
     int n_store = 0;
     const unsigned short* A_mid = nullptr;
     const unsigned short* B_mid = nullptr;
@@ -83,9 +85,10 @@
 bool trunk_fwd16_supported(int H);
 int trunk_fwd16(const float* x, int64_t ldx, const Planes& W0q, const float* b0, const float* gain, const float* beta, float* rstd,
                 const Planes& hq, const Planes& xhatq, int rows, int in_dim, int H, int nets, int64_t astride, int64_t pstride, hipStream_t s);
+struct QSlotArgs { const float* part[2]; const float* b2[2]; int slots; float* q; float* abs_part; };
 int ln_bwd(float* dh, const float* h, const float* xhat, const Planes& hq, const Planes& xhatq, const float* rstd, const float* gain, float* P,
            int rows, int H, int nets, int64_t astride, int64_t pstride, int want_params, hipStream_t s, const float* w0t, int64_t tstride,
-           float* dx, int dx_cols, const float* beta);
+           float* dx, int dx_cols, const float* beta, const QSlotArgs* qslots = nullptr);
 int trunk_chunks(int rows);
 int64_t knn_scratch_floats(int n_src, int n_tgt);
 int knn_topk(const float* src, int n_src, const float* tgt, int n_tgt, int dim, int k, float* out, float* d2, hipStream_t s);
@@ -124,6 +127,7 @@
     uint64_t seed, counter; const uint64_t* counter_ptr;
     const float* task;
     int64_t task_ld;
+    const float* route_q;
     const float* lam_parts;
     int lam_chunks;
     int da_nets;
@@ -138,6 +142,7 @@
 int tune_variant();
 constexpr int TUNE_CONV_WGRAD_TILE = 64;
 constexpr int TUNE_ACT_GENERIC = 256;
+constexpr int TUNE_PI_QHEAD = 1024;
 constexpr int TUNE_CONV_PER_IMAGE = 8388608;
 constexpr int TUNE_ADAPTER_PADDED = 134217728;
 constexpr int TUNE_CONV_STRIP = 1073741824;
@@ -295,6 +300,7 @@
 struct MetricsWindowArgs {
     const float *crit_part, *abs_part, *bc_part;
     int q_chunks, bc_chunks;
+    int abs_chunks;
     int fused;
     int kind, act_dim, ent_from_std;
     float inv_bg, alpha;
diff --git a/exorl_amd/csrc/loss.hip b/exorl_amd/csrc/loss.hip
--- a/exorl_amd/csrc/loss.hip
+++ b/exorl_amd/csrc/loss.hip
@@ -582,7 +582,7 @@
     if (w.fused) {
         const int k = t < 9 ? t : 8;
         const float* p = k < 6 ? w.crit_part + k : (k < 8 ? w.abs_part + (k - 6) : w.bc_part);
-        const float sum = chunk_sum(p, t >= 9 ? 0 : (k < 8 ? w.q_chunks : w.bc_chunks), k < 6 ? 6 : (k < 8 ? 2 : 1));
+        const float sum = chunk_sum(p, t >= 9 ? 0 : (k < 6 ? w.q_chunks : (k < 8 ? w.abs_chunks : w.bc_chunks)), k < 6 ? 6 : (k < 8 ? 2 : 1));
         if (t < 9) tot[t] = sum;
     }
     if (t < EXORL_N_METRICS) m[t] = old;
diff --git a/exorl_amd/engine.py b/exorl_amd/engine.py
--- a/exorl_amd/engine.py
+++ b/exorl_amd/engine.py
@@ -209,6 +209,11 @@
 
     def poison_scratch(self):
         L.check(self.lib.exorl_debug_agent_poison_scratch(self.h, L.current_stream()))
+
+    def head_fold(self):
+        n = C.c_int32()
+        L.check(self.lib.exorl_debug_agent_head_fold(self.h, C.byref(n)))
+        return int(n.value)
 
     def weight_images(self, net):
         w = L.WeightImages()
diff --git a/include/exorl_hip.h b/include/exorl_hip.h
--- a/include/exorl_hip.h
+++ b/include/exorl_hip.h
@@ -167,6 +167,7 @@
 int exorl_agent_noise_counter(exorl_agent_t* a, uint64_t* counter_out, void* stream);
 int exorl_debug_philox_normal(uint64_t seed, uint64_t counter, int64_t n, float* out_dev, void* stream);
 int exorl_debug_agent_poison_scratch(exorl_agent_t* a, void* stream);
+int exorl_debug_agent_head_fold(exorl_agent_t* a, int32_t* pi_slots);
 typedef struct {
     int32_t n_trunks, n_heads, in_dim, hidden_dim;
     float* w0t;
```

After: 3330 (median of 2 runs). About the same (+0.2%).
